# wujinzhong/seamlessCloneOptimization

Hardware: AMD Instinct MI355X
Metric: Mpix/s seamlessClone (ROI 2048^2) (higher is better)
Workload: dtype f32 (arithmetic); storage: 16-bit fixed-point field on the first two level-0 stores of a solve, float16 right-hand side and level 1

## Files before the change

include/seamlessclone_hip_testing.h:

```cpp
#ifndef SEAMLESSCLONE_HIP_TESTING_H
#define SEAMLESSCLONE_HIP_TESTING_H

#include "seamlessclone_hip.h"

#ifdef __cplusplus
extern "C" {
#endif

#define SC_FLAG_LEGACY_PATHS   (1 << 6)
#define SC_LEGACY_SEPARATE_RESTRICT 1
#define SC_LEGACY_BOTTOM_F32   2
#define SC_LEGACY_SEPARATE_TAIL 4
#define SC_LEGACY_UNPACKED_TILES 8
#define SC_LEGACY_SPLICE_LAUNCH 16
#define SC_FORCE_INTERLEAVED_OUT 32
#define SC_FLAG_KEEP_FIELD     (1 << 7)

#define SC_FLAG_POISON_ARENA   (1 << 14)


SC_API int sc_hip_mask_stage(void *instance, const uint8_t *mask, int mask_cols, int mask_rows, int mask_step,
                      int centerX, int centerY, int geo[6], uint8_t *M_out, size_t M_capacity);

SC_API int sc_hip_build_rhs(void *instance,
                     const uint8_t *face, int face_cols, int face_rows, int face_step,
                     const uint8_t *body, int body_cols, int body_rows, int body_step,
                     const uint8_t *mask, int mask_cols, int mask_rows, int mask_step,
                     int centerX, int centerY, int geo[6], float *B_out, float *lap_out, size_t plane_capacity);

SC_API int sc_hip_edit_rhs(void *instance, const sc_edit_params *p, const uint8_t *src, int cols, int rows, int src_step,
                           const uint8_t *mask, int mask_step, uint8_t *M_out, float *lap_out, size_t plane_capacity);
SC_API int sc_hip_canny(void *instance, const uint8_t *src, int cols, int rows, int src_step, float low_threshold,
                        float high_threshold, int kernel_size, uint8_t *classes_out, uint8_t *edges_out, int counts[2]);
SC_API int sc_hip_edit_counts(void *instance, int counts[2]);

SC_API int sc_hip_field_load(void *instance, int W, int H, int C, const float *U, const float *lap);
SC_API int sc_hip_field_sweep(void *instance, int method, int sweeps, float omega, int sweeps_per_launch);
SC_API int sc_hip_field_residual(void *instance, double out[2] );
SC_API int sc_hip_field_solve(void *instance);
SC_API int sc_hip_field_shape(void *instance, int whc[3]);
SC_API int sc_hip_field_store(void *instance, float *U_out, size_t capacity_floats);

SC_API int sc_hip_field_finish(void *instance, uint8_t *body, int body_cols, int body_rows, int body_step, int ltx, int lty);
SC_API int sc_hip_field_lowmode(void *instance);

SC_API int sc_hip_field_time_sweeps(void *instance, int method, int launches, int sweeps_per_launch, float omega,
                             float *ms_per_launch);

SC_API int sc_hip_time_cycle0(void *instance, int launches, float *ms_per_launch);
SC_API int sc_hip_time_cycle0_form(void *instance, int form, int launches, float *ms_per_launch);
SC_API int sc_hip_time_coarse_chain(void *instance, int reps, float *ms_eager, float *ms_graph, int *launches);
SC_API int sc_hip_time_tail_phases(void *instance, unsigned long long *cycles11);

SC_API int sc_hip_selftest_host(void);

SC_API int sc_hip_cycle0_form(const int *facts, int index, int form[3]);

SC_API int sc_hip_bytes_writer(void *instance);

SC_API int sc_hip_coarse_tile_plan(const int *facts, int *plan);

SC_API int sc_hip_pcg_plan(int cols, int rows, int kind, int frames, long long plan[10]);

#define SC_FUSED_ROW 18
SC_API int sc_hip_fused_schedule(const int *facts, const int *verdicts, int nverdicts, int *rows, int capacity);

SC_API int sc_hip_restore_spans(long long step, int rows, int ltx, int lty, int W, int H, long long *spans, int capacity);

#ifdef __cplusplus
}
#endif
#endif
```

seamlesscloneoptimization_amd/capi.py:

```python
from __future__ import annotations

import ctypes as C
import os
import re
import subprocess

import numpy as np

_PKG = os.path.dirname(os.path.abspath(__file__))
_ROOT = os.path.dirname(_PKG)
LIB_PATH = os.path.join(_PKG, "libseamlessclone_hip.so")
HEADER_PATH = os.path.join(_ROOT, "include", "seamlessclone_hip.h")
TESTING_HEADER_PATH = os.path.join(_ROOT, "include", "seamlessclone_hip_testing.h")

SC_OK = 0
SC_ERR_BAD_ARG = -1
SC_ERR_BAD_SIZE = -2
SC_ERR_EMPTY_MASK = -3
SC_ERR_ROI_OOB = -4
SC_ERR_HIP = -5
SC_ERR_NOT_CONVERGED = -6

SC_NORMAL_CLONE = 1
SC_MIXED_CLONE = 2
SC_MONOCHROME_TRANSFER = 3
CLONE_MODES = (SC_NORMAL_CLONE, SC_MIXED_CLONE, SC_MONOCHROME_TRANSFER)

SC_EDIT_COLOR_CHANGE = 1
SC_EDIT_ILLUMINATION_CHANGE = 2
SC_EDIT_TEXTURE_FLATTENING = 3
EDIT_OPS = (SC_EDIT_COLOR_CHANGE, SC_EDIT_ILLUMINATION_CHANGE, SC_EDIT_TEXTURE_FLATTENING)

SC_METHOD_JACOBI = 0
SC_METHOD_RBGS = 1
SC_METHOD_SOR = 2
SC_METHOD_MULTIGRID = 3
SC_METHOD_DST = 4
SC_METHOD_AUTO = 5
SC_METHOD_FFT = 6
SC_AUTO_DIRECT_MAX = 720
SC_AUTO_DIRECT_AREA = 450000
SC_AUTO_NARROW_MAX = 140
SC_AUTO_THIN_MAX = 4
SC_AUTO_THIN_LONG_MAX = 4096

SC_FLAG_NO_SPECULATE = 1 << 0
SC_FLAG_FLOAT_RHS = 1 << 1
SC_FLAG_FLOAT_U0 = 1 << 2
SC_FLAG_NO_COMPOSE_L1 = 1 << 3
SC_FLAG_VCYCLE_BOTTOM = 1 << 4
SC_FLAG_EXACT_TABLES = 1 << 5
SC_FLAG_LEGACY_PATHS = 1 << 6
SC_LEGACY_SEPARATE_RESTRICT, SC_LEGACY_BOTTOM_F32, SC_LEGACY_SEPARATE_TAIL, SC_LEGACY_UNPACKED_TILES = 1, 2, 4, 8
SC_LEGACY_SPLICE_LAUNCH = 16
SC_FORCE_INTERLEAVED_OUT = 32
SC_FLAG_KEEP_FIELD = 1 << 7
SC_FLAG_FFT_FP64 = 1 << 8
SC_FLAG_OPENCV_GREY_MASK = 1 << 9
SC_FLAG_FLOAT_L1 = 1 << 10
SC_FLAG_FLOAT_FIELD = 1 << 11
SC_FLAG_NO_STAGE_MARKS = 1 << 12
SC_FLAG_ROWS_RETURN = 1 << 13
SC_FLAG_POISON_ARENA = 1 << 14

def auto_takes_direct(w: int, h: int) -> bool:
    if w <= SC_AUTO_DIRECT_MAX and h <= SC_AUTO_DIRECT_MAX:
        return True
    if max(w, h) <= SC_AUTO_THIN_LONG_MAX and (w * h <= SC_AUTO_DIRECT_AREA or min(w, h) <= SC_AUTO_NARROW_MAX):
        return True
    return False


ERR_NAMES = {
    SC_ERR_BAD_ARG: "SC_ERR_BAD_ARG", SC_ERR_BAD_SIZE: "SC_ERR_BAD_SIZE", SC_ERR_EMPTY_MASK: "SC_ERR_EMPTY_MASK",
    SC_ERR_ROI_OOB: "SC_ERR_ROI_OOB", SC_ERR_HIP: "SC_ERR_HIP", SC_ERR_NOT_CONVERGED: "SC_ERR_NOT_CONVERGED",
}


class SolverOpts(C.Structure):
    _fields_ = [("method", C.c_int), ("max_sweeps", C.c_int), ("tol", C.c_float), ("check_every", C.c_int),
                ("omega", C.c_float), ("sweeps_per_launch", C.c_int), ("reference_warmup", C.c_int),
                ("mg_pre", C.c_int), ("mg_post", C.c_int), ("update_tol", C.c_float), ("flags", C.c_int), ("jacobi_tile_rows", C.c_int), ("mg_level1_sweeps", C.c_int), ("mg_direct_max", C.c_int), ("legacy_paths", C.c_int)]


class RunInfo(C.Structure):
    _fields_ = [("x0", C.c_int), ("y0", C.c_int), ("W", C.c_int), ("H", C.c_int), ("ltx", C.c_int), ("lty", C.c_int),
                ("sweeps", C.c_int), ("converged", C.c_int), ("rel_residual", C.c_double),
                ("ms_h2d", C.c_float), ("ms_mask", C.c_float), ("ms_pre", C.c_float), ("ms_solve", C.c_float),
                ("ms_post", C.c_float), ("ms_d2h", C.c_float), ("ms_device_total", C.c_float),
                ("sweep_launches", C.c_int), ("last_update", C.c_float), ("device_bytes", C.c_size_t), ("method", C.c_int),
                ("device", C.c_int), ("ms_call", C.c_float), ("field_retry", C.c_int), ("new_size", C.c_int),
                ("group_members", C.c_int), ("group_ragged", C.c_int)]


class BatchJob(C.Structure):
    _fields_ = [("face", C.c_void_p), ("face_cols", C.c_int), ("face_rows", C.c_int), ("face_step", C.c_int),
                ("body", C.c_void_p), ("body_cols", C.c_int), ("body_rows", C.c_int), ("body_step", C.c_int),
                ("mask", C.c_void_p), ("mask_cols", C.c_int), ("mask_rows", C.c_int), ("mask_step", C.c_int),
                ("centerX", C.c_int), ("centerY", C.c_int), ("body_restore", C.c_void_p), ("rc", C.c_int)]


class EditParams(C.Structure):
    _fields_ = [("op", C.c_int), ("red_mul", C.c_float), ("green_mul", C.c_float), ("blue_mul", C.c_float),
                ("alpha", C.c_float), ("beta", C.c_float), ("low_threshold", C.c_float), ("high_threshold", C.c_float),
                ("kernel_size", C.c_int)]


class EditJob(C.Structure):
# ... 204 lines not shown
    L.my_seamlessclone_api_imp_destroy.restype = None
    L.my_seamlessclone_api_imp_sync.argtypes = [C.c_void_p]
    L.my_seamlessclone_api_imp_sync.restype = None
    L.sc_hip_default_opts.argtypes = [C.POINTER(SolverOpts)]
    L.sc_hip_default_opts.restype = None
    L.sc_hip_set_solver.argtypes = [C.c_void_p, C.POINTER(SolverOpts)]
    L.sc_hip_set_solver.restype = C.c_int
    L.sc_hip_get_solver.argtypes = [C.c_void_p, C.POINTER(SolverOpts)]
    L.sc_hip_get_solver.restype = C.c_int
    L.sc_hip_get_info.argtypes = [C.c_void_p, C.POINTER(RunInfo)]
    L.sc_hip_get_info.restype = C.c_int
    L.sc_hip_last_error.argtypes = [C.c_void_p]
    L.sc_hip_last_error.restype = C.c_char_p
    L.sc_hip_set_clone_mode.argtypes = [C.c_void_p, C.c_int]
    L.sc_hip_set_clone_mode.restype = C.c_int
    L.sc_hip_get_clone_mode.argtypes = [C.c_void_p]
    L.sc_hip_get_clone_mode.restype = C.c_int
    L.sc_hip_pool_set_clone_mode.argtypes = [C.c_void_p, C.c_int]
    L.sc_hip_pool_set_clone_mode.restype = C.c_int
    L.sc_hip_run_device.argtypes = [C.c_void_p] + _IMG * 3 + [C.c_int, C.c_int, C.c_bool]
    L.sc_hip_run_device.restype = C.c_int
    L.sc_hip_malloc.argtypes = [C.c_void_p, C.c_size_t]
    L.sc_hip_malloc.restype = C.c_void_p
    L.sc_hip_free.argtypes = [C.c_void_p, C.c_void_p]
    L.sc_hip_free.restype = None
    L.sc_hip_host_alloc.argtypes = [C.c_void_p, C.c_size_t]
    L.sc_hip_host_alloc.restype = C.c_void_p
    L.sc_hip_host_free.argtypes = [C.c_void_p, C.c_void_p]
    L.sc_hip_host_free.restype = None
    L.sc_hip_memcpy_h2d.argtypes = [C.c_void_p, C.c_void_p, C.c_void_p, C.c_size_t]
    L.sc_hip_memcpy_h2d.restype = C.c_int
    L.sc_hip_memcpy_d2h.argtypes = [C.c_void_p, C.c_void_p, C.c_void_p, C.c_size_t]
    L.sc_hip_memcpy_d2h.restype = C.c_int
    L.sc_hip_memcpy_d2d_async.argtypes = [C.c_void_p, C.c_void_p, C.c_void_p, C.c_size_t]
    L.sc_hip_memcpy_d2d_async.restype = C.c_int
    L.sc_hip_device_count.argtypes = []
    L.sc_hip_device_count.restype = C.c_int
    L.sc_hip_device_pci_bus_id.argtypes = [C.c_int, C.c_char_p, C.c_int]
    L.sc_hip_device_pci_bus_id.restype = C.c_int
    L.sc_hip_mask_stage.argtypes = [C.c_void_p] + _IMG + [C.c_int, C.c_int, i32p, u8p, C.c_size_t]
    L.sc_hip_mask_stage.restype = C.c_int
    L.sc_hip_build_rhs.argtypes = [C.c_void_p] + _IMG * 3 + [C.c_int, C.c_int, i32p, f32p, f32p, C.c_size_t]
    L.sc_hip_build_rhs.restype = C.c_int
    L.sc_hip_field_load.argtypes = [C.c_void_p, C.c_int, C.c_int, C.c_int, f32p, f32p]
    L.sc_hip_field_load.restype = C.c_int
    L.sc_hip_field_sweep.argtypes = [C.c_void_p, C.c_int, C.c_int, C.c_float, C.c_int]
    L.sc_hip_field_sweep.restype = C.c_int
    L.sc_hip_field_residual.argtypes = [C.c_void_p, f64p]
    L.sc_hip_field_residual.restype = C.c_int
    L.sc_hip_field_solve.argtypes = [C.c_void_p]
    L.sc_hip_field_solve.restype = C.c_int
    L.sc_hip_bytes_writer.argtypes = [C.c_void_p]
    L.sc_hip_bytes_writer.restype = C.c_int
    L.sc_hip_field_shape.argtypes = [C.c_void_p, i32p]
    L.sc_hip_field_shape.restype = C.c_int
    L.sc_hip_field_store.argtypes = [C.c_void_p, f32p, C.c_size_t]
    L.sc_hip_field_store.restype = C.c_int
    L.sc_hip_field_finish.argtypes = [C.c_void_p, C.c_void_p, C.c_int, C.c_int, C.c_int, C.c_int, C.c_int]
    L.sc_hip_field_finish.restype = C.c_int
    L.sc_hip_field_lowmode.argtypes = [C.c_void_p]
    L.sc_hip_field_lowmode.restype = C.c_int
    L.sc_hip_field_time_sweeps.argtypes = [C.c_void_p, C.c_int, C.c_int, C.c_int, C.c_float, C.POINTER(C.c_float)]
    L.sc_hip_field_time_sweeps.restype = C.c_int
    L.sc_hip_pool_create.argtypes = [C.c_int, C.c_int]
    L.sc_hip_pool_create.restype = C.c_void_p
    L.sc_hip_pool_destroy.argtypes = [C.c_void_p]
    L.sc_hip_pool_destroy.restype = None
    L.sc_hip_pool_size.argtypes = [C.c_void_p]
    L.sc_hip_pool_size.restype = C.c_int
    L.sc_hip_pool_instance.argtypes = [C.c_void_p, C.c_int]
    L.sc_hip_pool_instance.restype = C.c_void_p
    L.sc_hip_pool_set_solver.argtypes = [C.c_void_p, C.POINTER(SolverOpts)]
    L.sc_hip_pool_set_solver.restype = C.c_int
    L.sc_hip_pool_run.argtypes = [C.c_void_p, C.POINTER(BatchJob), C.c_int, C.c_int]
    L.sc_hip_pool_run.restype = C.c_int
    L.sc_hip_pool_set_group.argtypes = [C.c_void_p, C.c_int]
    L.sc_hip_pool_set_group.restype = C.c_int
    L.sc_hip_run_device_batch.argtypes = [C.c_void_p, C.POINTER(BatchJob), C.c_int]
    L.sc_hip_run_device_batch.restype = C.c_int
    L.sc_hip_time_cycle0.argtypes = [C.c_void_p, C.c_int, C.POINTER(C.c_float)]
    L.sc_hip_time_cycle0.restype = C.c_int
    L.sc_hip_time_coarse_chain.argtypes = [C.c_void_p, C.c_int, C.POINTER(C.c_float), C.POINTER(C.c_float), C.POINTER(C.c_int)]
    L.sc_hip_time_coarse_chain.restype = C.c_int
    L.sc_hip_time_tail_phases.argtypes = [C.c_void_p, C.POINTER(C.c_ulonglong)]
    L.sc_hip_time_tail_phases.restype = C.c_int
    L.sc_hip_time_cycle0_form.argtypes = [C.c_void_p, C.c_int, C.c_int, C.POINTER(C.c_float)]
    L.sc_hip_time_cycle0_form.restype = C.c_int
    L.sc_hip_reference_tables_singular.argtypes = [C.c_int, C.c_int]
    L.sc_hip_reference_tables_singular.restype = C.c_int
    L.sc_hip_selftest_host.argtypes = []
    L.sc_hip_selftest_host.restype = C.c_int
    L.sc_hip_cycle0_form.argtypes = [i32p, C.c_int, i32p]
    L.sc_hip_cycle0_form.restype = C.c_int
    L.sc_hip_coarse_tile_plan.argtypes = [i32p, i32p]
    L.sc_hip_coarse_tile_plan.restype = C.c_int
    L.sc_hip_pcg_plan.argtypes = [C.c_int] * 4 + [C.POINTER(C.c_longlong)]
    L.sc_hip_pcg_plan.restype = C.c_int
    L.sc_hip_fused_schedule.argtypes = [i32p, i32p, C.c_int, i32p, C.c_int]
    L.sc_hip_fused_schedule.restype = C.c_int
    L.sc_hip_restore_spans.argtypes = [C.c_longlong] + [C.c_int] * 5 + [C.POINTER(C.c_longlong), C.c_int]
    L.sc_hip_restore_spans.restype = C.c_int
    L.sc_hip_plan_groups.argtypes = [i32p, C.c_int, C.c_int, C.POINTER(SolverOpts), i32p, i32p]
    L.sc_hip_plan_groups.restype = C.c_int
    L.sc_hip_plan_size.argtypes = [C.c_int, C.c_int, C.POINTER(SolverOpts), i32p]
    L.sc_hip_plan_groups_pool.argtypes = [i32p, C.c_int, C.c_int, C.c_int, C.POINTER(SolverOpts), i32p, i32p]
    L.sc_hip_plan_groups_pool.restype = C.c_int
# ... 808 lines not shown
        return p

    def from_device(self, p, shape, dtype=np.uint8):
        out = np.empty(shape, dtype)
        self._check(self.L.sc_hip_memcpy_d2h(self.h, out.ctypes.data, p, out.nbytes))
        return out

    def copy_d2d_async(self, dst, src, nbytes):
        self._check(self.L.sc_hip_memcpy_d2d_async(self.h, dst, src, nbytes))

    def run_device(self, d_face, fshape, d_body, bshape, d_mask, mshape, cx, cy, sync=True,
                   allow_not_converged=False):
        rc = self.L.sc_hip_run_device(self.h, d_face, fshape[1], fshape[0], 3 * fshape[1],
                                      d_body, bshape[1], bshape[0], 3 * bshape[1],
                                      d_mask, mshape[1], mshape[0], mshape[1], int(cx), int(cy), bool(sync))
        return self._check(rc, allow=(SC_ERR_NOT_CONVERGED,) if allow_not_converged else ())

    def run_device_batch(self, jobs, sync=True):
        rc = self.L.sc_hip_run_device_batch(self.h, jobs, len(jobs))
        if sync:
            self.sync()
        return self._check(rc, allow=(SC_ERR_NOT_CONVERGED,))

    def mask_stage(self, mask, cx, cy):
        m = _img(mask)
        geo = np.zeros(6, np.int32)
        M = np.zeros(m[1] * m[2], np.uint8)
        self._check(self.L.sc_hip_mask_stage(self.h, *m, int(cx), int(cy), geo.ctypes.data_as(i32p),
                                             M.ctypes.data_as(u8p), M.size))
        W, H = int(geo[2]), int(geo[3])
        return geo, M[:W * H].reshape(H, W).copy()

    def build_rhs(self, face, body, mask, cx, cy):
        f, b, m = _img(face), _img(body), _img(mask)
        geo = np.zeros(6, np.int32)
        cap = m[1] * m[2]
        B = np.zeros(3 * cap, np.float32)
        lap = np.zeros(3 * cap, np.float32)
        self._check(self.L.sc_hip_build_rhs(self.h, *f, *b, *m, int(cx), int(cy), geo.ctypes.data_as(i32p),
                                            B.ctypes.data_as(f32p), lap.ctypes.data_as(f32p), cap))
        W, H = int(geo[2]), int(geo[3])
        return geo, B[:3 * W * H].reshape(3, H, W).copy(), lap[:3 * W * H].reshape(3, H, W).copy()

    def field_load(self, U, lap):
        U = np.ascontiguousarray(U, np.float32)
        lap = np.ascontiguousarray(lap, np.float32)
        assert U.shape == lap.shape and U.ndim == 3
        Cc, H, W = U.shape
        self._check(self.L.sc_hip_field_load(self.h, W, H, Cc, U.ctypes.data_as(f32p), lap.ctypes.data_as(f32p)))

    def bytes_writer(self):
        return int(self.L.sc_hip_bytes_writer(self.h))

    def field_shape(self):
        whc = np.zeros(3, np.int32)
        self._check(self.L.sc_hip_field_shape(self.h, whc.ctypes.data_as(i32p)))
        return int(whc[2]), int(whc[1]), int(whc[0])

    def field_sweep(self, method, sweeps, omega=1.0, sweeps_per_launch=1):
        self._check(self.L.sc_hip_field_sweep(self.h, int(method), int(sweeps), float(omega), int(sweeps_per_launch)))

    def field_residual(self):
        out = np.zeros(2, np.float64)
        self._check(self.L.sc_hip_field_residual(self.h, out.ctypes.data_as(f64p)))
        return float(out[0]), float(out[1])

    def field_solve(self, allow_not_converged=False):
        rc = self.L.sc_hip_field_solve(self.h)
        return self._check(rc, allow=(SC_ERR_NOT_CONVERGED,) if allow_not_converged else ())

    def field_store(self):
        out = np.zeros(self.field_shape(), np.float32)
        self._check(self.L.sc_hip_field_store(self.h, out.ctypes.data_as(f32p), out.size))
        return out

    def field_finish(self, body, ltx, lty):
        b = _img(body)
        self._check(self.L.sc_hip_field_finish(self.h, *b, int(ltx), int(lty)))

    def field_lowmode(self):
        self._check(self.L.sc_hip_field_lowmode(self.h))

    def field_time_sweeps(self, method, launches, sweeps_per_launch=1, omega=1.0) -> float:
        ms = C.c_float(0)
        self._check(self.L.sc_hip_field_time_sweeps(self.h, int(method), int(launches), int(sweeps_per_launch),
                                                    float(omega), C.byref(ms)))
        return float(ms.value)

    def time_cycle0(self, launches: int = 100) -> float:
        ms = C.c_float(0)
        self._check(self.L.sc_hip_time_cycle0(self.h, int(launches), C.byref(ms)))
        return float(ms.value)

    def time_cycle0_form(self, form: int, launches: int = 100) -> float:
        ms = C.c_float(0)
        self._check(self.L.sc_hip_time_cycle0_form(self.h, int(form), int(launches), C.byref(ms)))
        return float(ms.value)

    def time_coarse_chain(self, reps: int = 50):
        a, b, n = C.c_float(0), C.c_float(0), C.c_int(0)
        self._check(self.L.sc_hip_time_coarse_chain(self.h, int(reps), C.byref(a), C.byref(b), C.byref(n)))
        return float(a.value), float(b.value), int(n.value)

    def time_tail_phases(self):
        buf = (C.c_ulonglong * 11)()
        self._check(self.L.sc_hip_time_tail_phases(self.h, buf))
# ... 93 lines not shown
        try:
            self.close()
        except Exception:
            pass


def plan_size(W: int, H: int, opts: "SolverOpts | None" = None) -> dict:
    out = np.zeros(12, np.int32)
    load().sc_hip_plan_size(int(W), int(H), C.byref(opts) if opts is not None else None, out.ctypes.data_as(i32p))
    keys = ("eligible", "levels", "tail_level", "pad_x", "pad_y", "Kxp", "Kyp", "column_tiles", "row_splits", "direct_nx_ny", "solo_differs", "conditional")
    return dict(zip(keys, out.tolist()))


def plan_groups_pool(sizes, group: int = 0, streams: int = 2, opts: "SolverOpts | None" = None):
    wh = np.ascontiguousarray(np.asarray(sizes, np.int32).reshape(-1, 2))
    n = wh.shape[0]
    g = np.zeros(n, np.int32); k = np.zeros(n, np.int32)
    rc = load().sc_hip_plan_groups_pool(wh.ctypes.data_as(i32p), n, int(group), int(streams), C.byref(opts) if opts is not None else None,
                                        g.ctypes.data_as(i32p), k.ctypes.data_as(i32p))
    if rc < 0:
        raise SeamlessCloneError(rc, "sc_hip_plan_groups_pool")
    return g.tolist(), k.tolist()


SC_POOL_GROUP_AUTO = 0


def plan_edit_groups_pool(sizes, group: int = 0, streams: int = 2):
    wh = np.ascontiguousarray(np.asarray(sizes, np.int32).reshape(-1, 2))
    n = wh.shape[0]
    g = np.zeros(n, np.int32)
    rc = load().sc_hip_plan_edit_groups_pool(wh.ctypes.data_as(i32p), n, int(group), int(streams), g.ctypes.data_as(i32p))
    if rc < 0:
        raise SeamlessCloneError(rc, "sc_hip_plan_edit_groups_pool")
    return g.tolist()


def plan_prepare(sizes, opts: "SolverOpts | None" = None) -> int:
    wh = np.ascontiguousarray(np.asarray(sizes, np.int32).reshape(-1, 2))
    return int(load().sc_hip_plan_prepare(wh.ctypes.data_as(i32p), wh.shape[0], C.byref(opts) if opts is not None else None))


def plan_cache_clear() -> None:
    load().sc_hip_plan_cache_clear()


CYCLE0_FACTS = ("sweeps", "prolong", "f_half", "u_half", "q16_in", "q16_out", "final_cycle", "out_bytes", "composed", "l1_half", "timing",
                "bands", "rag")


def cycle0_form(**facts):
    if facts.pop("out_interleaved", 0):
        facts["out_bytes"] = int(bool(facts.get("out_bytes", 0))) | 2
    f = (C.c_int * len(CYCLE0_FACTS))(*[int(facts.pop(k, 0)) for k in CYCLE0_FACTS])
    if facts:
        raise TypeError("cycle0_form: no such fact: %s" % sorted(facts))
    out = (C.c_int * 3)()
    return tuple(out) if load().sc_hip_cycle0_form(f, 0, out) == 0 else -1


def coarse_tile_plan(W, H, C_, useful, halo, rows, size_class=False, unpacked=False, lanes=False):
    f = (C.c_int * 10)(W, H, C_, useful, halo, rows, int(size_class), int(unpacked), 0, 0)
    head = np.zeros(4, np.int32)
    rc = load().sc_hip_coarse_tile_plan(f, head.ctypes.data_as(i32p))
    if rc != 0:
        raise SeamlessCloneError(rc, "coarse_tile_plan")
    if not lanes:
        return tuple(int(v) for v in head)
    n = int(head[3])
    f[9] = n
    out = np.zeros(4 + 130 * n, np.int32)
    rc = load().sc_hip_coarse_tile_plan(f, out.ctypes.data_as(i32p))
    if rc != 0:
        raise SeamlessCloneError(rc, "coarse_tile_plan")
    t = out[4:].reshape(n, 130)
    return tuple(int(v) for v in head), (t[:, 0], t[:, 1], t[:, 2::2], t[:, 3::2])


PCG_PLAN = ("nx", "ny", "x0", "y0", "cg", "bands", "rows", "eparts", "egroups", "stride")


def pcg_plan(cols, rows, kind, frames=1):
    out = (C.c_longlong * len(PCG_PLAN))()
    rc = load().sc_hip_pcg_plan(int(cols), int(rows), int(kind), int(frames), out)
    if rc != 0:
        raise SeamlessCloneError(rc, "pcg_plan")
    return dict(zip(PCG_PLAN, (int(v) for v in out)))


FUSED_FACTS = ("pre", "post", "budget", "tol", "out_wanted", "q16", "u_half", "composed", "separate_restrict", "early_kind", "bytes_form", "small")
FUSED_ROW = ("kind", "sweeps", "prolong", "final_cycle", "out_bytes", "u_half", "q16_in", "q16_out", "composed", "bands", "lm", "nodes", "judged",
             "coarse_first", "sat", "bands_asked", "early_asked", "cycle")


def fused_schedule(verdicts=(), **facts):
    d = dict(pre=2, post=2, budget=30, tol=0, out_wanted=1, q16=1, u_half=1, composed=1, separate_restrict=0, early_kind=1, bytes_form=1, small=1)
    unknown = sorted(set(facts) - set(d))
    if unknown:
        raise TypeError("fused_schedule: no such fact: %s" % unknown)
    d.update(facts)
    f = (C.c_int * len(FUSED_FACTS))(*[int(d[k]) for k in FUSED_FACTS])
    v = (C.c_int * max(1, len(verdicts)))(*[int(x) for x in verdicts])
    cap = len(FUSED_ROW) * (3 * int(d["budget"]) + 2) + 3
    out = (C.c_int * cap)()
    n = load().sc_hip_fused_schedule(f, v, len(verdicts), out, cap)
    if n < 0:
        raise SeamlessCloneError(n, "fused_schedule")
    k = len(FUSED_ROW)
    return [dict(zip(FUSED_ROW, out[k * i:k * i + k])) for i in range(n)], out[k * n], out[k * n + 1], out[k * n + 2]


# ... 48 lines not shown
```

seamlesscloneoptimization_amd/csrc/sanitize_main.cpp:

```cpp
#include "../../include/seamlessclone_hip_testing.h"
#include "sc_pcg.h"
#include <algorithm>
#include <atomic>
#include <cmath>
#include <cstdio>
#include <cstdlib>
#include <cstring>
#include <thread>
#include <vector>

namespace {
struct StubInst { int gpu; std::atomic<long> calls{ 0 }; sc_solver_opts opts; int clone_mode = SC_NORMAL_CLONE; };
std::atomic<long> g_jobs_run{ 0 };
}
extern "C" {
void *stub_create(int gpu) { StubInst *s = new StubInst(); s->gpu = gpu; sc_hip_default_opts(&s->opts); return s; }
void stub_destroy(void *p) { delete (StubInst *)p; }
void stub_sync(void *) {}
int stub_set_solver(void *p, const sc_solver_opts *o) { ((StubInst *)p)->opts = *o; return SC_OK; }
int stub_get_solver(void *p, sc_solver_opts *o) { *o = ((StubInst *)p)->opts; return SC_OK; }
int stub_set_clone_mode(void *p, int mode)
{
    if (mode < SC_NORMAL_CLONE || mode > SC_MONOCHROME_TRANSFER) return SC_ERR_BAD_ARG;
    ((StubInst *)p)->clone_mode = mode;
    return SC_OK;
}
int stub_memcpy_d2d_async(void *, void *, const void *, size_t) { return SC_OK; }
int stub_run_device(void *p, const uint8_t *, int, int, int, uint8_t *body, int, int, int, const uint8_t *, int, int, int, int, int, bool)
{
    ((StubInst *)p)->calls++;
    g_jobs_run++;
    *(volatile uint8_t *)body += 1;
    return SC_OK;
}
int stub_run(void *p, const uint8_t *f, int fc, int fr, int fs, uint8_t *body, int bc, int br, int bs, const uint8_t *m, int mc, int mr, int ms, int cx, int cy, int, bool)
{
    return stub_run_device(p, f, fc, fr, fs, body, bc, br, bs, m, mc, mr, ms, cx, cy, false);
}
std::atomic<long> g_edit_mixed{ 0 };
int stub_edit_device(void *p, const sc_edit_params *, const uint8_t *, int, int, int, const uint8_t *, int, uint8_t *dst, int, bool)
{
    ((StubInst *)p)->calls++;
    g_jobs_run++;
    *(volatile uint8_t *)dst += 1;
    return SC_OK;
}
int stub_edit(void *p, const sc_edit_params *e, const uint8_t *s, int c, int r, int ss, const uint8_t *m, int ms, uint8_t *dst, int ds)
{
    return stub_edit_device(p, e, s, c, r, ss, m, ms, dst, ds, false);
}
constexpr int FAILING_COLS = 777;
int stub_edit_device_batch(void *p, const sc_edit_params *, sc_edit_job *jobs, int n)
{
    ((StubInst *)p)->calls++;
    for (int i = 0; i < n; ++i) {
        if (jobs[i].cols != jobs[0].cols || jobs[i].rows != jobs[0].rows) g_edit_mixed++;
        g_jobs_run++; *(volatile uint8_t *)jobs[i].dst += 1; jobs[i].rc = SC_OK;
    }
    return jobs[0].cols == FAILING_COLS ? SC_ERR_HIP : SC_OK;
}
// ... 485 lines not shown
                pub[k] = sc_volume_wls_job{ fake(k, 6), fake(k, 9), fake(k, 4), nullptr, fake(k, 8), k == 1 ? nullptr : fake(k, 3), fake(k, 0),
                                            links ? fake(k, 1) : nullptr, links ? fake(k, 2) : nullptr,
                                            !links ? nullptr : k == 3 ? (const float *)((uintptr_t)fake(k, 5) + 2) : fake(k, 5), fake(k, 10),
                                            (float *)fake(k, 7), 12345 };
            }
            Instance inst;
            FloatJobs v;
            const int rc = float_intake(&inst, SC_POISSON_GUIDANCE, carries, pub, 5, arrays_of, v);
            const std::vector<int> stay = links ? std::vector<int>{ 0, 2, 4 } : std::vector<int>{ 0, 2, 3, 4 };
            if (rc != SC_ERR_BAD_ARG || inst.err != "null state pointer") return fail("float_intake: the worst code and the first reason");
            if (v.dj.size() != stay.size() || v.side.size() != stay.size() || v.rcs.size() != stay.size()) return fail("float_intake: how many jobs stay");
            if (pub[1].rc != SC_ERR_BAD_ARG || (links && pub[3].rc != SC_ERR_BAD_ARG)) return fail("float_intake: a refused job's code");
            for (size_t i = 0; i < stay.size(); ++i) {
                const int k = stay[i];
                const SideArrays &a = v.side[i];
                if (v.rcs[i] != &pub[k].rc || pub[k].rc != SC_ERR_HIP) return fail("float_intake: where a job's code goes");
                if (v.dj[i].gx != fake(k, 6) || v.dj[i].gy != fake(k, 9) || v.dj[i].b != fake(k, 10) || v.dj[i].out != (float *)fake(k, 7) || v.dj[i].d != fake(k, 8))
                    return fail("float_intake: a job's own arrays");
                if (a.w != fake(k, 0) || a.st != fake(k, 3) || a.gt != fake(k, 4)) return fail("float_intake: w, st or gt of another job");
                if (links ? (a.sx != fake(k, 1) || a.sy != fake(k, 2) || a.smt != fake(k, 5)) : (a.sx || a.sy || a.smt))
                    return fail("float_intake: sx, sy or smt of another job, or not NULL where the call carries none");
            }
        }
        {
            sc_volume_wls_job one{ fake(0, 6), fake(0, 9), fake(0, 4), nullptr, fake(0, 8), fake(0, 3), fake(0, 0), fake(0, 1), fake(0, 2), fake(0, 5), fake(0, 10),
                                   (float *)fake(0, 7), 0 };
            Instance inst;
            FloatJobs v;
            if (float_intake(&inst, SC_POISSON_GUIDANCE, FLOAT_DATA | FLOAT_STATE, &one, 1, arrays_of, v) != SC_OK || v.side.size() != 1) return fail("float_intake (a plain region call)");
            const SideArrays &a = v.side[0];
            if (a.w || a.sx || a.sy || a.gt || a.smt || a.st != fake(0, 3)) return fail("float_intake: an array the call does not carry must be NULL");
        }
    }
    {
        const int kinds[] = { SC_POISSON_LAPLACIAN, SC_POISSON_LAPLACIAN | SC_POISSON_NEUMANN, SC_POISSON_GUIDANCE | SC_POISSON_FREE_LEFT | SC_POISSON_FREE_TOP,
                              SC_POISSON_GUIDANCE | SC_POISSON_PERIODIC_X, SC_POISSON_LAPLACIAN | SC_POISSON_PERIODIC_X | SC_POISSON_PERIODIC_Y };
        for (int kind : kinds)
            for (int frames : { 1, 2, 17, 64, SC_POISSON_MAX_PLANES })
                for (int cols = 3; cols <= 2105; cols += (cols < 20 ? 1 : 83))
                    for (int rows = 3; rows <= 2205; rows += (rows < 70 ? 1 : 61)) {
                        long long p[10];
                        if (sc_hip_pcg_plan(cols, rows, kind, frames, p) != SC_OK) return fail("pcg_plan");
                        const long long nx = p[0], ny = p[1], cg = p[4], bands = p[5], rows_per = p[6], eparts = p[7], egroups = p[8], stride = p[9];
                        if (nx < 1 || nx > cols || ny < 1 || ny > (long long)rows * frames || ny % frames) return fail("pcg_plan: the unknown block");
                        if (cg != (nx + 255) / 256 || cg * bands > sc::PCG_PARTS || bands * rows_per < ny || (bands - 1) * rows_per >= ny) return fail("pcg_plan: the bands");
                        if (eparts < 1 || eparts > sc::PCG_PARTS || egroups != (nx * ny + 3) / 4 || eparts * ((egroups + eparts - 1) / eparts) < egroups) return fail("pcg_plan: the segments");
                        if (stride % 64 || stride < nx * ny) return fail("pcg_plan: the stride");
                    }
        long long p[10];
        if (sc_hip_pcg_plan(2, 7, SC_POISSON_LAPLACIAN, 1, p) != SC_ERR_BAD_SIZE || sc_hip_pcg_plan(33, 47, SC_POISSON_NEUMANN, 1, p) != SC_ERR_BAD_ARG ||
            sc_hip_pcg_plan(33, 47, SC_POISSON_LAPLACIAN, 0, p) != SC_ERR_BAD_ARG || sc_hip_pcg_plan(33, 47, SC_POISSON_LAPLACIAN, SC_POISSON_MAX_PLANES + 1, p) != SC_ERR_BAD_ARG ||
            sc_hip_pcg_plan(33, 47, SC_POISSON_LAPLACIAN, 1, nullptr) != SC_ERR_BAD_ARG) return fail("pcg_plan (refusals)");
    }
    printf("sanitize_main: clean\n");
    return 0;
}
```

seamlesscloneoptimization_amd/csrc/sc_arena.cpp:

```cpp
#include "sc_instance.h"
#include <algorithm>
#include <cstring>
#include <thread>

namespace sc {

int hip_fail(Instance *I, hipError_t e, const char *what)
{
    if (I) {
        I->err = std::string(what) + ": " + hipGetErrorString(e);
        I->scan_counter_dirty = true;
    }
    return SC_ERR_HIP;
}

int ensure(Instance *I, DevBuf &b, size_t bytes, bool zero)
{
    if (bytes <= b.cap) {
        if (!zero && bytes && (I->opts.flags & SC_FLAG_POISON_ARENA)) {
            SC_HIP(I, hipStreamSynchronize(I->stream));
            if (I->aux) SC_HIP(I, hipStreamSynchronize(I->aux));
            if (I->aux2) SC_HIP(I, hipStreamSynchronize(I->aux2));
            SC_HIP(I, hipMemsetAsync(b.p, 0xFF, bytes, I->stream));
            SC_HIP(I, hipStreamSynchronize(I->stream));
// ... 102 lines not shown
    if (rc) return rc;
    uint8_t *s = (uint8_t *)stage.p;
    size_t piece = (size_t)1 << 20;
    for (int y0 = 0; y0 < rows;) {
        const int n = std::min((int)std::max<size_t>(1, piece / dpitch), rows - y0);
        copy_rows(I, s + (size_t)y0 * dpitch, dpitch, h + (size_t)y0 * hpitch, hpitch, row_bytes, n);
        SC_HIP(I, hipMemcpyAsync((uint8_t *)d + (size_t)y0 * dpitch, s + (size_t)y0 * dpitch, dpitch * (size_t)(n - 1) + row_bytes,
                                 hipMemcpyHostToDevice, I->stream));
        y0 += n;
        piece = std::min(piece * 4, (size_t)8 << 20);
    }
    return SC_OK;
}

int download_rows(Instance *I, DevBuf &stage, uint8_t *h, size_t hpitch, const void *d, size_t dpitch,
                  size_t row_bytes, int rows)
{
    if (rows <= 0 || row_bytes == 0) return SC_OK;
    const size_t total = dpitch * (size_t)(rows - 1) + row_bytes;
    int rc = ensure_pinned(I, stage, total);
    if (rc) return rc;
    SC_HIP(I, hipMemcpyAsync(stage.p, d, total, hipMemcpyDeviceToHost, I->stream));
    SC_HIP(I, hipStreamSynchronize(I->stream));
    copy_rows(I, h, hpitch, (const uint8_t *)stage.p, dpitch, row_bytes, rows);
    return SC_OK;
}

static Field make_field(void *p, int W, int H, int C)
{
    Field f;
    f.p = (float *)p; f.W = W; f.H = H; f.C = C;
    f.pitch = round_up(W, 64);
    f.plane = (size_t)f.pitch * H;
    return f;
}

int setup_fields(Instance *I, int W, int H, int C)
{
    field_moved(I);
    I->out_direct = false;
    Field proto = make_field(nullptr, W, H, C);
    const size_t bytes = proto.bytes() + 4096;
    int rc;
    if ((rc = ensure(I, I->d_U0, bytes, false))) return rc;
    if ((rc = ensure(I, I->d_U1, bytes, false))) return rc;
    if ((rc = ensure(I, I->d_F, bytes, false))) return rc;
    const bool same = I->F.p == I->d_F.p && I->U0.p == I->d_U0.p && I->U1.p == I->d_U1.p && I->F.W == W &&
                      I->F.H == H && I->F.C == C;
    I->U0 = make_field(I->d_U0.p, W, H, C);
    I->U1 = make_field(I->d_U1.p, W, H, C);
    I->F = make_field(I->d_F.p, W, H, C);
    I->result_in_U1 = false;
    I->f_half = false;
    I->u_half = false;
    if (!same) I->mg.clear();
    return SC_OK;
}

}
```

seamlesscloneoptimization_amd/csrc/sc_batch.cpp:

```cpp
#include "sc_instance.h"
#include <algorithm>
#include <cmath>
#include <cstring>
#include <vector>

using namespace sc;

namespace sc {

FrameSpans frame_spans(size_t step, int rows, int ltx, int lty, int W, int H)
{
    FrameSpans f{};
    f.bytes = step * (size_t)rows;
    f.head_end = f.tail_begin = f.bytes;
    if (W < 3 || H < 3) return f;
    const size_t c0 = 3 * (size_t)(ltx + 1), c1 = 3 * (size_t)(ltx + W - 1), top = (size_t)(lty + 1) * step;
    f.head_end = top + c0;
    f.mid_first = top + c1; f.mid_len = step - (c1 - c0); f.stride = step; f.mids = H - 3;
    f.tail_begin = top + (size_t)(H - 3) * step + c1;
    return f;
}

}

namespace {

constexpr int GROUP_RS = 32;

struct RagScope {
    Instance *I;
    ~RagScope() { rag_end(I); }
};

int run_group_members(Instance *I, sc_batch_job *jobs, const std::vector<int> &idx, const std::vector<Geo> &geo, const int *guess, int *d_r,
                      const std::vector<SizePlan> *plans, const std::vector<char> &frame)
{
    const int n = (int)idx.size();
    Geo g0 = geo[idx[0]];
    if (plans) for (int k = 1; k < n; ++k) { g0.W = std::max(g0.W, geo[idx[k]].W); g0.H = std::max(g0.H, geo[idx[k]].H); }
    int rc;
    I->mpitch = round_up(g0.W, 64);
    const size_t mplane = (size_t)I->mpitch * g0.H;
    if ((rc = ensure(I, I->d_M, mplane * n, false))) return rc;
    if ((rc = setup_fields(I, g0.W, g0.H, 3 * n))) return rc;
    RagScope scope{ I };
    CallScope call{ I };
    std::vector<MaskJob> mj(n);
    std::vector<ImageJob> ij(n);
    for (int k = 0; k < n; ++k) {
        const int i = idx[k];
        const sc_batch_job &j = jobs[i];
        mj[k] = MaskJob{};
        mj[k].mask = j.mask; mj[k].mw = j.mask_cols; mj[k].mh = j.mask_rows; mj[k].mstep = j.mask_step;
        mj[k].rect = d_r + GROUP_RS * i;
        mj[k].g = geo[i]; mj[k].M = (uint8_t *)I->d_M.p + mplane * k; mj[k].mpitch = I->mpitch;
        ij[k].face_org = j.face + (size_t)geo[i].y0 * j.face_step + 3 * geo[i].x0; ij[k].fstep = j.face_step;
        const size_t roi = (size_t)geo[i].lty * j.body_step + 3 * geo[i].ltx;
        ij[k].body_org = j.body + roi; ij[k].body_src = frame[i] ? j.body_restore + roi : j.body + roi; ij[k].bstep = j.body_step;
        ij[k].M = (const uint8_t *)I->d_M.p + mplane * k;
        ij[k].d_rect = guess ? d_r + GROUP_RS * i : nullptr;
        if (guess) { ij[k].rx0 = guess[4 * i]; ij[k].rx1 = guess[4 * i + 1]; ij[k].ry0 = guess[4 * i + 2]; ij[k].ry1 = guess[4 * i + 3]; }
        if (plans) { ij[k].W = geo[i].W; ij[k].H = geo[i].H; }
    }
    if (plans && (rc = rag_begin_table(I, *plans))) return rc;
    bool builds_done = false;
    launch_mask_erode3_group(mj.data(), n, I->stream);
    I->erode_done = false;
    I->guard = RectGuard();
    const SolveTarget to{ nullptr, 0, &ij };
    const int solve_rc = solve_step(I, to, [&]() -> int {
        launch_preprocess_group(ij.data(), n, I->mpitch, I->U0, I->F, I->stream, I->f_half, I->u_half, I->clone_mode);
        SC_HIP(I, hipGetLastError());
        if (plans && !builds_done) {
            if ((rc = rag_begin_builds(I))) return rc;
            builds_done = true;
        }
        return SC_OK;
    });
    if (solve_rc != SC_OK && solve_rc != SC_ERR_NOT_CONVERGED) return solve_rc;
    if (!I->spec_post.done && (rc = write_output(I, to))) return rc;
    for (int k = 0; k < n; ++k) jobs[idx[k]].rc = solve_rc;
    SC_HIP(I, hipGetLastError());
    fill_info_geo(I, g0);
    I->info.group_members = n; I->info.group_ragged = plans ? 1 : 0;
    return solve_rc;
}

int report_groups(const std::vector<std::vector<int>> &groups, const std::vector<SizePlan> &plans, const int *order, int *group_of, int *kind_of)
{
    for (size_t g = 0; g < groups.size(); ++g) {
        bool uniform = true;
        for (int i : groups[g]) uniform = uniform && plans[i].W == plans[groups[g][0]].W && plans[i].H == plans[groups[g][0]].H;
        for (int i : groups[g]) {
            const int m = order ? order[i] : i;
            group_of[m] = (int)g;
            if (kind_of) kind_of[m] = groups[g].size() < 2 ? 0 : uniform ? 1 : plans[i].solo_differs ? 3 : 2;
        }
    }
    return (int)groups.size();
}

}

extern "C" {

int sc_hip_run_device_batch(void *p, sc_batch_job *jobs, int n)
{
    if (!jobs || n <= 0) return SC_ERR_BAD_ARG;
    Instance *I;
    int rc = begin_call(p, I);
    if (rc) return rc;
    auto alone = [&](int i) -> int {
        sc_batch_job &j = jobs[i];
        j.rc = sc_hip_run_device(p, j.face, j.face_cols, j.face_rows, j.face_step, j.body, j.body_cols, j.body_rows, j.body_step,
                                 j.mask, j.mask_cols, j.mask_rows, j.mask_step, j.centerX, j.centerY, false);
        return j.rc;
    };
    auto one_by_one = [&]() -> int {
        int worst = SC_OK;
        for (int i = 0; i < n; ++i) worst = worse(worst, alone(i));
        return worst;
    };
    std::vector<char> frame(n, 0);
    std::vector<Geo> geo(n);
// ... 240 lines not shown
```

seamlesscloneoptimization_amd/csrc/sc_common.h:

```cpp
#pragma once
#include <hip/hip_runtime.h>
#include <stdint.h>
#include <stddef.h>
#include <algorithm>
#include <string>
#include <vector>
#include "../../include/seamlessclone_hip_testing.h"

namespace sc {

struct Field {
    float *p = nullptr;
    int W = 0, H = 0, C = 0;
    int pitch = 0;
    size_t plane = 0;
    __host__ __device__ float *at(int c) const { return p + (size_t)c * plane; }
    size_t bytes() const { return plane * (size_t)C * sizeof(float); }
};

static inline int round_up(int v, int m) { return (v + m - 1) / m * m; }

struct Geo { int x0, y0, W, H, ltx, lty; };

struct Img8 {
// ... 69 lines not shown
    return (a - b) + (cc - d);
}
#endif
void launch_poisson_pre(const PoissonGeo &g, bool lap, const PoissonJobDev &j, Field U0, Field F, hipStream_t s, float lam = 0.f);
void launch_poisson_pre_group(const PoissonGeo &g, bool lap, const PoissonJobDev *jobs, int n, Field U0, Field F, hipStream_t s, float lam = 0.f);
void launch_poisson_out(const PoissonGeo &g, const PoissonJobDev &j, Field U, hipStream_t s);
void launch_poisson_out_group(const PoissonGeo &g, const PoissonJobDev *jobs, int n, Field U, hipStream_t s);
int poisson_mean_parts(int H);
void launch_poisson_mean(const PoissonGeo &g, const PoissonJobDev *jobs, int n, double *parts, hipStream_t s);
size_t mask_bbox_group_parts(const MaskJob *jobs, int n);
void launch_mask_bbox_group(const MaskJob *jobs, int n, hipStream_t s, int *parts);
void launch_mask_erode3_group(const MaskJob *jobs, int n, hipStream_t s);
struct BboxTask { const uint8_t *mask = nullptr; int mw = 0, mh = 0, mstep = 0; BboxFold fold; int scan_rows = 0; Geo g{}; size_t mask_bytes = 0; uint8_t *M_out = nullptr; };
void launch_preprocess(const uint8_t *body_org, int bstep, const uint8_t *face_org, int fstep,
                       const uint8_t *M, int mpitch, Field U0, Field U1, Field F, hipStream_t s, bool f_half = false, bool u_half = false, bool grey = false,
                       const BboxTask *scan = nullptr, int mode = SC_NORMAL_CLONE);
struct RectGuard { const int *d_rect = nullptr; int x0 = 0, x1 = 0, y0 = 0, y1 = 0; };
struct AbortFlag { unsigned *p = nullptr; unsigned gen = 0; unsigned *host = nullptr; };
#if defined(__HIPCC__)
__device__ __forceinline__ bool abort_set(const AbortFlag &a) { return a.p && *reinterpret_cast<const volatile unsigned *>(a.p) == a.gen; }
#endif
struct LmNodes { const float *CN = nullptr; int ny = 0, npitch = 0; };
#if defined(__HIPCC__)
__device__ __forceinline__ void lm_add4_nodes(float p00, float p01, float p10, float p11, int x, int y, float4 &v)
{
    const float ty = 0.125f * (float)(y & 7);
    const float l = __builtin_fmaf(ty, p10 - p00, p00), r = __builtin_fmaf(ty, p11 - p01, p01);
    const float dx = 0.125f * (r - l), a0 = __builtin_fmaf((float)(x & 7), dx, l);
    v.x += a0;
    v.y += a0 + dx;
    v.z += __builtin_fmaf(2.0f, dx, a0);
    v.w += __builtin_fmaf(3.0f, dx, a0);
}
__device__ __forceinline__ void lm_add4(const LmNodes &lm, int c, int x, int y, float4 &v)
{
    const float *__restrict__ p = lm.CN + ((size_t)c * lm.ny + (y >> 3)) * lm.npitch + (x >> 3);
    lm_add4_nodes(p[0], p[1], p[lm.npitch], p[lm.npitch + 1], x, y, v);
}
__device__ __forceinline__ unsigned lm_byte(float d)
{
    d = d > 255.0f ? 255.0f : d;
    d = d < 0.0f ? 0.0f : d;
    return (unsigned)(unsigned char)d;
}
__device__ __forceinline__ float lm_bilinear(const LmNodes &lm, int c, int x, int y)
{
    const float *__restrict__ p = lm.CN + ((size_t)c * lm.ny + (y >> 3)) * lm.npitch + (x >> 3);
    const float tx = 0.125f * (float)(x & 7), ty = 0.125f * (float)(y & 7);
    const float top = __builtin_fmaf(tx, p[1] - p[0], p[0]), bot = __builtin_fmaf(tx, p[lm.npitch + 1] - p[lm.npitch], p[lm.npitch]);
    return __builtin_fmaf(ty, bot - top, top);
}
#endif
void launch_postprocess(Field U, uint8_t *body_org, int bstep, hipStream_t s, RectGuard guard = RectGuard(), LmNodes lm = LmNodes(), AbortFlag ab = AbortFlag());
void launch_preprocess_group(const ImageJob *jobs, int n, int mpitch, Field U0, Field F, hipStream_t s, bool f_half, bool u_half, int mode);
void launch_postprocess_group(Field U, const ImageJob *jobs, int n, hipStream_t s, LmNodes lm = LmNodes(), AbortFlag ab = AbortFlag());
void launch_splice_planar(Field Q, uint8_t *body_org, int bstep, hipStream_t s, RectGuard guard = RectGuard(), AbortFlag ab = AbortFlag());
void launch_splice_planar_group(Field Q, const ImageJob *jobs, int n, hipStream_t s, AbortFlag ab = AbortFlag());
void launch_half_to_float(const void *src_half, float *dst, size_t n, hipStream_t s);
struct FrameSpans { size_t bytes, head_end, mid_first, mid_len, stride, tail_begin; int mids; };
FrameSpans frame_spans(size_t step, int rows, int ltx, int lty, int W, int H);
struct CopyJobs { enum { MAX = 16 }; void *dst[MAX]; const void *src[MAX]; size_t bytes[MAX]; FrameSpans frame[MAX]; };
void launch_copy_group(const CopyJobs &t, int n, hipStream_t s);

void launch_jacobi(Field Uin, Field Uout, Field F, hipStream_t s, bool tag = false, int lds_tile_rows = 0);
void launch_rb_half(Field U, Field F, int color, float omega, hipStream_t s, bool tag = false);
bool launch_jacobi_tb(Field Uin, Field Uout, Field F, int sweeps, hipStream_t s, bool tag = false);
bool launch_rb_tb(Field Uin, Field Uout, Field F, int sweeps, float omega, hipStream_t s, bool tag = false);
int  tb_max_depth(int method);
int  tb_hard_max_depth(int method);
long tb_big_side();
struct TilePlan { int nbx, nby, full, lps, lg, K, blocks; };
__host__ __device__ inline TilePlan coarse_tile_plan(int W, int H, int C, int uw, int hx, int rows, bool size_class, bool pack = true)
{
    TilePlan p;
    p.nbx = (W + uw - 1) / uw; p.nby = (H + rows - 1) / rows;
    p.full = p.nbx; p.lps = 64; p.lg = 6; p.K = 1;
    const int need = (W - (p.nbx - 1) * uw + 2 * hx + 3) / 4;
    if (pack && !size_class && need <= 32) {
        p.lg = 32 - __builtin_clz((unsigned)(need - 1));
        p.lps = 1 << p.lg; p.K = 64 >> p.lg; p.full = p.nbx - 1;
    }
    p.blocks = p.nby * (p.full * C + (p.nbx - p.full) * ((C + p.K - 1) >> (6 - p.lg)));
    return p;
}
struct TileLane { int by, c, x, sl, lps; };
__host__ __device__ inline TileLane coarse_tile_lane(const TilePlan &p, int C, int uw, int hx, int tile, int lane)
{
    TileLane t;
    const int nfull = p.full * p.nby * C;
    if (tile < nfull) {
        const int q = tile / p.full;
        t.c = q / p.nby; t.by = q - t.c * p.nby;
        t.x = (tile - q * p.full) * uw - hx + 4 * lane; t.sl = lane; t.lps = 64;
    } else {
        const int k = tile - nfull, g = k / p.nby;
        t.by = k - g * p.nby; t.lps = p.lps; t.sl = lane & (p.lps - 1);
        t.c = (g << (6 - p.lg)) + (lane >> p.lg);
        t.x = p.full * uw - hx + 4 * t.sl;
    }
    return t;
}
int  tb_gen_rows(int W, int H, int C, int hx, int hy, bool pack = false, int pack_rows = 8);
int  tb_gen_rows_deep(int W, int H, int C, int hx, int hy, bool pack = false);
struct MGGeom;
struct ComposeArgs;
struct RagMember;
constexpr int TBM_PLAIN = 0, TBM_PROLONG = 1, TBM_ZEROIN = 4;
bool launch_rb_tb_gen(Field Uin, Field Uout, Field F, int sweeps, const MGGeom &g, int mode, Field E, hipStream_t s, const RagMember *rag = nullptr, int lev = 0,
                      bool pack = true);
int  launch_rb_tb_prolong0(Field Uin, Field Uout, Field F, int sweeps, const MGGeom &g, Field E, float *partial, hipStream_t s);
int  tb_blocks_level0(int W, int H, int C, int sweeps);
void launch_max_final(const float *d_partial, int n, unsigned *d_out, hipStream_t s);
void launch_max_final2(const float *d_a, int na, const float *d_b, int nb, unsigned *d_out2, hipStream_t s, const unsigned *flag = nullptr);
void cycle0_row_geometry(int H, int sweeps, int &nby, int &step, int &hy);
int  cycle0_blocks(int W, int H, int C, int sweeps);
bool launch_cycle_coarse(Field Uout, Field F, Field Fc, const MGGeom &g, int sweeps, hipStream_t s, bool half_io = false,
                         const RagMember *rag = nullptr, int lev = 0, bool pack = true);

int  residual_max_blocks();
void launch_residual(Field U, Field F, double *d_partials, double *d_out, hipStream_t s);

struct MGDim {
    int n, nc;
    float alpha;
    float cw_last;
    float d_last;
    float tw1, tw2;
    float inv_last;
};
struct MGGeom { MGDim x, y; };
struct ComposeArgs { Field E2; MGGeom g1; };

constexpr int C0_TIMING   = 1;
constexpr int C0_F_HALF   = 2;
constexpr int C0_U_HALF   = 4;
constexpr int C0_FINAL    = 8;
constexpr int C0_COMPOSED = 16;
constexpr int C0_OUT      = 32;
constexpr int C0_BANDS    = 64;
constexpr int C0_L1_HALF  = 128;
constexpr int C0_Q16_IN   = 256;
constexpr int C0_Q16_OUT  = 512;
constexpr int C0_PACK_ROWS = 6;
constexpr int C0_PACK     = 2048;
constexpr int C0_OUT3     = 4096;
constexpr int C0_RAG      = 1024;

struct Cycle0Launch {
    Field Uin, Uout, F, Fc, E;
    MGGeom g{};
    int sweeps = 0;
    bool prolong = false;
    bool f_half = false, u_half = false, q16_in = false, q16_out = false;
    bool final_cycle = false, out_bytes = false;
    bool out_interleaved = false;
    const ImageJob *jobs = nullptr; int njobs = 0;
    bool composed = false;
    bool l1_half = false, timing = false;
    ComposeArgs comp{};
    float4 *bands = nullptr;
    float *partial = nullptr;
    LmNodes lm{};
    AbortFlag sat{};
    const RagMember *rag = nullptr;
    hipStream_t s = nullptr;
};
bool cycle0_form(const Cycle0Launch &d, int &T, bool &PRO, int &TAG);
int  cycle0_form_at(int i, int &T, bool &PRO, int &TAG);
int  launch_cycle0(const Cycle0Launch &d);

constexpr int RAG_MAX_LEVELS = 12;
struct RagMember {
    int W, H;
    int lw[RAG_MAX_LEVELS], lh[RAG_MAX_LEVELS];
    MGGeom g[RAG_MAX_LEVELS];
    const unsigned char *mm;
    int npx, npy;
    int lm_nx, lm_ny, lm_cells_y, lm_nxt, lm_nrs, lm_nparts, lm_Kx, lm_Ky;
    const float *lm_Sx, *lm_Sy, *lm_R;
    const int *lm_map[2];
};

void launch_rb_half_gen(Field U, Field F, int color, float omega, MGGeom g, hipStream_t s);
void launch_residual_restrict(Field U, Field F, Field Fc, MGGeom g, hipStream_t s);
int  prolong_blocks(int nx, int ny, int C);
void launch_prolong_add(Field Uc, Field Uf, MGGeom g, float *d_partial, unsigned *d_maxcorr, hipStream_t s);
void launch_fill_zero(Field U, hipStream_t s);

constexpr int MG_BOTTOM_MAX_LEVELS = 12;
constexpr int MG_BOTTOM_LDS_BYTES = 152 * 1024;
struct MGBottomLevel { MGGeom g; float omega; int offU, offF, pitch; };
struct MGBottomArgs {
    int nlevels, pre, post, coarse_sweeps, lds_floats;
    int fd_level, fd_nxp, fd_nyp, fd_off;
    const float *fd_mats;
    Field Ftop, Utop;
    MGBottomLevel lv[MG_BOTTOM_MAX_LEVELS];
};
__host__ __device__ static inline long fd_mat_floats(int nxp, int nyp) { return 2L * nxp * nxp + 2L * nyp * nyp + (long)nxp * nyp; }
__host__ __device__ static inline long fd_lds_floats(int nxp, int nyp) { return fd_mat_floats(nxp, nyp) + 2L * nxp * nyp; }
hipError_t mg_bottom_prepare();
void launch_fd_build(float *mats, const MGGeom &g, int nxp, int nyp, hipStream_t s, unsigned char *mm = nullptr, int NPX = 0, int NPY = 0);
void launch_fd_build_rag(const RagMember *rag, int members, int lev, hipStream_t s);
__host__ __device__ static inline long fd_mm_bytes(int NPX, int NPY) { return 4L * (2L * NPX * NPX + 2L * NPY * NPY + (long)NPX * NPY); }
struct MGBottomMM { const unsigned char *mm; Field Ftop, Utop; int nx, ny; };
bool launch_mg_bottom_mm(const MGBottomMM &a, int NPX, int NPY, int C, hipStream_t s);
struct MGTail { const unsigned char *mm; Field F, U; MGGeom g; int pre, post; unsigned long long *stamps;
                const RagMember *rag; int lev; bool rag_uniform; };
// ... 7 lines not shown
```

seamlesscloneoptimization_amd/csrc/sc_cycle0.hip:

```cpp
#include "sc_common.h"
#include <hip/hip_fp16.h>
#include "sc_wave.h"
#include "sc_mg_device.h"
#include <type_traits>

namespace sc {

constexpr int C0_HXQ = 3;
constexpr int C0_HX = 4 * C0_HXQ;

template <int R>
__device__ __forceinline__ void c0_load(const float *__restrict__ p, int P, int H, int x, int y0, float4 (&v)[R])
{
    const int xc = min(max(x, 0), P - 4);
#pragma unroll
    for (int r = 0; r < R; ++r) {
        const int yc = min(max(y0 + r, 0), H - 1);
        v[r] = *reinterpret_cast<const float4 *>(p + (size_t)yc * P + xc);
    }
}

template <int R>
__device__ __forceinline__ void c0_load_half(const __half *__restrict__ p, int P, int H, int x, int y0, float4 (&v)[R])
{
    const int xc = min(max(x, 0), P - 4);
    uint2 raw[R];
#pragma unroll
    for (int r = 0; r < R; ++r) {
        const int yc = min(max(y0 + r, 0), H - 1);
        raw[r] = *reinterpret_cast<const uint2 *>(p + (size_t)yc * P + xc);
    }
#pragma unroll
    for (int r = 0; r < R; ++r) {
        const __half2 a = *reinterpret_cast<const __half2 *>(&raw[r].x), b = *reinterpret_cast<const __half2 *>(&raw[r].y);
        const float2 fa = __half22float2(a), fb = __half22float2(b);
        v[r] = make_float4(fa.x, fa.y, fb.x, fb.y);
    }
}

template <int R>
__device__ __forceinline__ void c0_load_half_raw(const __half *__restrict__ p, int P, int H, int x, int y0, uint2 (&v)[R])
{
    const int xc = min(max(x, 0), P - 4);
#pragma unroll
    for (int r = 0; r < R; ++r) {
        const int yc = min(max(y0 + r, 0), H - 1);
        v[r] = *reinterpret_cast<const uint2 *>(p + (size_t)yc * P + xc);
    }
}
template <int R>
__device__ __forceinline__ void c0_load_q16(const uint16_t *__restrict__ p, int P, int H, int x, int y0, float4 (&v)[R])
{
    const int xc = min(max(x, 0), P - 4);
    uint2 raw[R];
#pragma unroll
    for (int r = 0; r < R; ++r) {
        const int yc = min(max(y0 + r, 0), H - 1);
        raw[r] = *reinterpret_cast<const uint2 *>(p + (size_t)yc * P + xc);
    }
#pragma unroll
    for (int r = 0; r < R; ++r) {
        v[r].x = __builtin_fmaf((float)(raw[r].x & 0xffffu), 0.015625f, -256.0f);
        v[r].y = __builtin_fmaf((float)(raw[r].x >> 16), 0.015625f, -256.0f);
        v[r].z = __builtin_fmaf((float)(raw[r].y & 0xffffu), 0.015625f, -256.0f);
        v[r].w = __builtin_fmaf((float)(raw[r].y >> 16), 0.015625f, -256.0f);
    }
}
__device__ __forceinline__ unsigned c0_q16_checked(float u, int &seen)
{
    int i;
    asm("v_cvt_i32_f32 %0, %1" : "=v"(i) : "v"(__builtin_fmaf(u, 64.0f, 16384.5f)));
    seen |= i;
    return (unsigned)min(max(i, 0), 65535);
}

__device__ __forceinline__ void c0_scale_q(uint2 &h)
{
    const __half2 k = __float2half2_rn(-0.25f);
    __half2 a = *reinterpret_cast<__half2 *>(&h.x), b = *reinterpret_cast<__half2 *>(&h.y);
    a = __hmul2(a, k); b = __hmul2(b, k);
    h.x = *reinterpret_cast<unsigned *>(&a); h.y = *reinterpret_cast<unsigned *>(&b);
}
template <int K>
__device__ __forceinline__ float c0_gs_q(float s, float quarter, const uint2 &h)
{
    const unsigned raw = (K < 2) ? h.x : h.y;
    float d;
    if (K & 1) asm("v_fma_mix_f32 %0, %1, %2, %3 op_sel:[0,0,1] op_sel_hi:[0,0,1]" : "=v"(d) : "v"(s), "s"(quarter), "v"(raw));
    else asm("v_fma_mix_f32 %0, %1, %2, %3 op_sel_hi:[0,0,1]" : "=v"(d) : "v"(s), "s"(quarter), "v"(raw));
    return d;
}
template <int K>
__device__ __forceinline__ float c0_f_minus(const uint2 &h, float s)
{
    const unsigned raw = (K < 2) ? h.x : h.y;
    float d;
    if (K & 1) asm("v_fma_mix_f32 %0, %1, -4.0, -%2 op_sel:[1,0,0] op_sel_hi:[1,0,0]" : "=v"(d) : "v"(raw), "v"(s));
    else asm("v_fma_mix_f32 %0, %1, -4.0, -%2 op_sel_hi:[1,0,0]" : "=v"(d) : "v"(raw), "v"(s));
    return d;
}
__device__ __forceinline__ float c0_comp(const float4 &v, int k) { return k == 0 ? v.x : k == 1 ? v.y : k == 2 ? v.z : v.w; }


constexpr int C0_OUT3_ROWS = 52, C0_OUT3_WORDS = (256 - 2 * C0_HX) / 4;
__device__ __forceinline__ int c0_lane_again() { int z = 0; asm volatile("" : "+v"(z)); return (int)__builtin_amdgcn_mbcnt_hi(~0u, __builtin_amdgcn_mbcnt_lo(~0u, (unsigned)z)); }
template <bool ON> __device__ __forceinline__ float c0_opaque_s(float v) { if constexpr (ON) asm volatile("" : "+s"(v)); return v; }
template <bool ON> __device__ __forceinline__ int c0_opaque_s(int v) { if constexpr (ON) asm volatile("" : "+s"(v)); return v; }
template <int N> __device__ __forceinline__ unsigned *c0_out3_stage() { __shared__ unsigned stage[N]; return stage; }
__device__ __forceinline__ void c0_out3_write(const unsigned *__restrict__ stage, uint8_t *__restrict__ body, int bstep, int W, int H, int x0t, int y0t,
                                              int wv, int lane, int nw)
{
    const int lo = 3 * (max(x0t, 1) - x0t), hi = 3 * (min(x0t + 4 * C0_OUT3_WORDS, W - 1) - x0t);
    for (int rr = wv; rr < C0_OUT3_ROWS; rr += nw) {
        const int y = y0t + rr;
        if (y < 1 || y > H - 2) continue;
        uint8_t *d = body + (size_t)y * bstep + 3 * (size_t)x0t;
        const int a = (int)((uintptr_t)d & 3);
        const int o0 = 12 * lane - a;
        if (o0 >= hi || o0 + 12 <= lo) continue;
        const int jc = min(lane, C0_OUT3_WORDS - 1), jp = max(min(lane - 1, C0_OUT3_WORDS - 1), 0);
        unsigned pc[3], pp[3];
#pragma unroll
        for (int c = 0; c < 3; ++c) {
            const unsigned *row = stage + (c * C0_OUT3_ROWS + rr) * C0_OUT3_WORDS;
            pc[c] = row[jc]; pp[c] = row[jp];
        }
        unsigned w[4];
        w[0] = ((pp[2] >> 16) & 255u) | ((pp[0] >> 24) << 8) | ((pp[1] >> 24) << 16) | ((pp[2] >> 24) << 24);
        w[1] = (pc[0] & 255u) | ((pc[1] & 255u) << 8) | ((pc[2] & 255u) << 16) | (((pc[0] >> 8) & 255u) << 24);
        w[2] = ((pc[1] >> 8) & 255u) | (((pc[2] >> 8) & 255u) << 8) | (((pc[0] >> 16) & 255u) << 16) | (((pc[1] >> 16) & 255u) << 24);
        w[3] = ((pc[2] >> 16) & 255u) | ((pc[0] >> 24) << 8) | ((pc[1] >> 24) << 16) | ((pc[2] >> 24) << 24);
#pragma unroll
        for (int k = 0; k < 3; ++k) {
            const unsigned v = (unsigned)(((((unsigned long long)w[k + 1]) << 32) | w[k]) >> (8 * (4 - a)));
            const int o = o0 + 4 * k;
            if (o >= lo && o + 4 <= hi) *reinterpret_cast<unsigned *>(d + o) = v;
            else {
#pragma unroll
                for (int b = 0; b < 4; ++b)
                    if (o + b >= lo && o + b < hi) d[o + b] = (uint8_t)(v >> (8 * b));
            }
        }
    }
}

template <int T, int NW, int R, bool PRO, bool GEN, bool ZEROIN, int TAG = 0, class... X3>
__global__ __launch_bounds__(NW * 64) __attribute__((amdgpu_waves_per_eu(4))) void k_cycle0(Field Uin, Field Uout, Field F, Field Fc, Field E, MGGeom g,
                                                    float *__restrict__ partial, ComposeArgs comp, float4 *__restrict__ bands, LmNodes lm, AbortFlag sat,
                                                    const RagMember *__restrict__ rag, int lev, X3... x3)
{
    constexpr int HY = 2 * T + 2, RH = NW * R;
    constexpr bool OUT3 = (TAG & C0_OUT3) != 0;
    static_assert(sizeof...(X3) == (OUT3 ? 1 : 0), "the members' jobs travel with the three-channel bytes form only");
    constexpr bool RAG = (TAG & C0_RAG) != 0;
    constexpr bool COMP = (TAG & C0_COMPOSED) != 0;
    static_assert(!COMP || (PRO && !GEN && R % 2 == 0), "composition of two prolongations exists on level 0 only");
    constexpr bool FINAL = (TAG & C0_FINAL) != 0;
    constexpr bool OUT = (TAG & C0_OUT) != 0, BANDS = ((TAG & C0_BANDS) != 0 || FINAL) && !OUT;
    static_assert(!OUT || (FINAL && !GEN), "bytes leave from the last level-0 launch only");
    static_assert(!OUT3 || (OUT && !RAG && T == 2 && RH - 2 * HY == C0_OUT3_ROWS), "interleaved bytes: the judged two-sweep form of a same-size group");
    static_assert(!(TAG & C0_BANDS) || !GEN, "cell shares exist on level 0 only");
    constexpr bool HF = (TAG & C0_F_HALF) != 0, HU = (TAG & C0_U_HALF) != 0;
    static_assert(!(HF && GEN), "float16 right-hand sides exist on level 0 only");
    constexpr bool L1H = (TAG & C0_L1_HALF) != 0;
    constexpr bool UQI = (TAG & C0_Q16_IN) != 0, UQO = (TAG & C0_Q16_OUT) != 0;
    static_assert(!((UQI || UQO) && (GEN || (HU && UQI) || (OUT && UQO))), "16-bit fields: level 0, between its launches");
    static_assert(!L1H || !GEN || ZEROIN, "float16 level-1 fields: the level-1 launch starts from a zero correction");
    static_assert(!(PRO && GEN), "the in-kernel prolongation relies on level 0's regular last interval");
    static_assert(2 * T + 2 <= C0_HX, "column halo too small");
    static_assert(R % 2 == 0, "bands must hold whole coarse-row pairs");
    __shared__ float4 edge[2][NW][2][64];
    __shared__ float2 hedge[2][NW][64];
    const int lane = threadIdx.x & 63;
    const int wv = __builtin_amdgcn_readfirstlane(threadIdx.x >> 6);
    int W = Uin.W, H = Uin.H;
    const int P = Uin.pitch;
    const int nbx = (W + (256 - 2 * C0_HX) - 1) / (256 - 2 * C0_HX), nby = (H + (RH - 2 * HY) - 1) / (RH - 2 * HY);
    const int tile = xcd_tile(blockIdx.x, gridDim.x);
    constexpr bool PACK = (TAG & C0_PACK) != 0;
    static_assert(!PACK || (GEN && ZEROIN && !PRO && !RAG), "packed column tiles: the coarse forms of one size");
    TileLane tl{};
    if constexpr (PACK) tl = coarse_tile_lane(coarse_tile_plan(W, H, Uin.C, 256 - 2 * C0_HX, C0_HX, RH - 2 * HY, false), Uin.C, 256 - 2 * C0_HX, C0_HX, tile, lane);
    const int bx = tile % nbx, by = PACK ? tl.by : (tile / nbx) % nby;
    const int c_first = PACK ? min(tl.c, Uin.C - 1) : OUT3 ? 3 * (tile / (nbx * nby)) : tile / (nbx * nby);
    const int sl = PACK ? tl.sl : lane, lps = PACK ? tl.lps : 64;
    const bool live = !PACK || tl.c < Uin.C;
    if constexpr (RAG) {
        const RagMember &m = rag[c_first / 3];
        W = m.lw[lev]; H = m.lh[lev];
        if (bx * (256 - 2 * C0_HX) >= W || by * (RH - 2 * HY) >= H) {
            if (PRO && threadIdx.x == 0) partial[tile] = 0.f;
            return;
        }
        g = m.g[lev];
        if (PRO) E.H = m.lh[lev + 1];
        if ((TAG & C0_COMPOSED) != 0) { comp.g1 = m.g[lev + 1]; comp.E2.H = m.lh[lev + 2]; }
    }
    const int lane_wg = lane, wv_wg = wv, bx_wg = bx, by_wg = by;
    const MGGeom &g_wg = g;
    const ComposeArgs &comp_wg = comp;
    int ci = 0, c_run = c_first, pt_run = OUT3 ? tile + 2 * (c_first / 3) * (nbx * nby) : tile;
    const int pt_step = nbx * nby;
    _Pragma("nounroll") do {
    const int lane = OUT3 ? c0_lane_again() : lane_wg, wv = c0_opaque_s<OUT3>(wv_wg), bx = c0_opaque_s<OUT3>(bx_wg), by = c0_opaque_s<OUT3>(by_wg);
    std::conditional_t<OUT3, MGGeom, const MGGeom &> g = g_wg;
    std::conditional_t<OUT3, ComposeArgs, const ComposeArgs &> comp = comp_wg;
    if constexpr (OUT3) {
        g.x.tw1 = c0_opaque_s<OUT3>(g.x.tw1); g.y.tw1 = c0_opaque_s<OUT3>(g.y.tw1);
        comp.g1.x.tw1 = c0_opaque_s<OUT3>(comp.g1.x.tw1); comp.g1.y.tw1 = c0_opaque_s<OUT3>(comp.g1.y.tw1);
    }
    const int x = PACK ? tl.x : bx * (256 - 2 * C0_HX) - C0_HX + 4 * lane;
    const int y0 = by * (RH - 2 * HY) - HY + wv * R;
    const int c = OUT3 ? c_run : c_first, ptile = OUT3 ? pt_run : tile;
    float4 u[R], f[HF ? 1 : R];
    uint2 fh[HF ? R : 1];
    if (ZEROIN) {
#pragma unroll
        for (int r = 0; r < R; ++r) u[r] = make_float4(0.f, 0.f, 0.f, 0.f);
    } else if (HU) {
        c0_load_half<R>(reinterpret_cast<const __half *>(Uin.p) + (size_t)c * Uin.plane, P, H, x, y0, u);
    } else if (UQI) {
        c0_load_q16<R>(reinterpret_cast<const uint16_t *>(Uin.p) + (size_t)c * Uin.plane, P, H, x, y0, u);
    } else {
        c0_load<R>(Uin.at(c), P, H, x, y0, u);
    }
    constexpr int NE = R / 2 + 2, NQ = R / 4 + 3;
    float2 eab[PRO ? NE : 1];
    float ecc[PRO ? NE : 1];
    float2 e2r[COMP ? NQ : 1];
    float e2l[COMP ? NQ : 1];
    static_assert(!PRO || GEN || 2 * T + 3 <= C0_HX, "column halo too small for the shared prolongation loads");
    float e2b63[COMP ? NQ : 1];
    if (PRO) {
        const int cx = min(max(x >> 1, 0), E.pitch - 4), J = (y0 >> 1) - 1;
        if constexpr (L1H) {
            const __half *__restrict__ e = reinterpret_cast<const __half *>(E.p) + (size_t)c * E.plane;
#pragma unroll
            for (int j = 0; j < NE; ++j) {
                const __half *er = e + (size_t)min(max(J + j, 0), E.H - 1) * E.pitch + cx;
                eab[j] = __half22float2(*reinterpret_cast<const __half2 *>(er));
            }
        } else {
        const float *__restrict__ e = E.at(c);
#pragma unroll
        for (int j = 0; j < NE; ++j) {
            const float *er = e + (size_t)min(max(J + j, 0), E.H - 1) * E.pitch + cx;
            eab[j] = *reinterpret_cast<const float2 *>(er);
        }
        }
    }
    if (COMP) {
        const float *__restrict__ e2 = comp.E2.at(c);
        const int qx = min(max(x >> 2, 0), comp.E2.pitch - 2), Q = ((y0 >> 1) - 1) >> 1;
#pragma unroll
        for (int q = 0; q < NQ; ++q) {
            const float *er = e2 + (size_t)min(max(Q + q, 0), comp.E2.H - 1) * comp.E2.pitch + qx;
            e2r[q].x = er[0];
            e2b63[q] = 0.f;
            if (lane == 63) e2b63[q] = er[1];
        }
    }
    if (!PRO) {
        if constexpr (HF) c0_load_half_raw<R>(reinterpret_cast<const __half *>(F.p) + (size_t)c * F.plane, P, H, x, y0, fh);
        else if constexpr (GEN && L1H) c0_load_half<R>(reinterpret_cast<const __half *>(F.p) + (size_t)c * F.plane, P, H, x, y0, f);
        else c0_load<R>(F.at(c), P, H, x, y0, f);
    }
    const bool x0ok = (x + 0 >= 1) && (x + 0 <= W - 2), x1ok = (x + 1 >= 1) && (x + 1 <= W - 2);
    const bool x2ok = (x + 2 >= 1) && (x + 2 <= W - 2), x3ok = (x + 3 >= 1) && (x + 3 <= W - 2);

    const int xw = bx * (256 - 2 * C0_HX) - C0_HX;
    bool inner = !GEN && (xw >= 4) && (xw + 255 <= W - 2) && (y0 >= 1) && (y0 + R - 1 <= H - 2);
// ... 256 lines not shown
#undef SC_C0_RES
#undef SC_C0_F
            float rl = wave_from_left(res.w);
            if (GEN) {
                float rn = wave_from_right(res.x);
                h0[r] = ((0.5f * rl + res.x) + wxa0 * res.y) + wxb0 * res.z;
                h1[r] = ((0.5f * res.y + res.z) + wxa1 * res.w) + wxb1 * rn;
            } else {
                h0[r] = __builtin_fmaf(res.y, 0.5f, __builtin_fmaf(rl, 0.5f, res.x));
                h1[r] = __builtin_fmaf(res.w, 0.5f, __builtin_fmaf(res.y, 0.5f, res.z));
            }
        }
        };
        if (inner) residual_rows(std::false_type{}); else residual_rows(std::true_type{});
        hedge[0][wv][lane] = make_float2(h0[R - 1], h1[R - 1]);
        if (GEN) hedge[1][wv][lane] = make_float2(h0[0], h1[0]);
        __syncthreads();
        const float2 hup = (wv > 0) ? hedge[0][wv - 1][lane] : make_float2(0.f, 0.f);
        const float2 hdn = (GEN && wv < NW - 1) ? hedge[1][wv + 1][lane] : make_float2(0.f, 0.f);
        const bool lane_out = (sl >= C0_HXQ) && (sl < lps - C0_HXQ) && live;
        float *__restrict__ fc = Fc.at(c);
        const float fx0 = (I == g.x.nc) ? 2.0f * g.x.inv_last : 1.0f;
        const float fx1 = (I + 1 == g.x.nc) ? 2.0f * g.x.inv_last : 1.0f;
#pragma unroll
        for (int r = 0; r < R; r += 2) {
            const int yr = wv * R + r, y = y0 + r;
            const int J = y >> 1;
            if (!lane_out || yr < HY || yr >= RH - HY || J < 1 || J > g.y.nc) continue;
            const float m0 = (r == 0) ? hup.x : h0[r - 1], m1 = (r == 0) ? hup.y : h1[r - 1];
            float v0, v1;
            if (GEN) {
                const float wya = (J == g.y.nc) ? g.y.tw1 : 0.5f, wyb = (J == g.y.nc) ? g.y.tw2 : 0.0f;
                const float p0 = (r + 2 < R) ? h0[(r + 2 < R) ? r + 2 : 0] : hdn.x;
                const float p1 = (r + 2 < R) ? h1[(r + 2 < R) ? r + 2 : 0] : hdn.y;
                v0 = ((0.5f * m0 + h0[r]) + wya * h0[r + 1]) + wyb * p0;
                v1 = ((0.5f * m1 + h1[r]) + wya * h1[r + 1]) + wyb * p1;
            } else {
                v0 = __builtin_fmaf(h0[r + 1], 0.5f, __builtin_fmaf(m0, 0.5f, h0[r]));
                v1 = __builtin_fmaf(h1[r + 1], 0.5f, __builtin_fmaf(m1, 0.5f, h1[r]));
            }
            const float fy = (J == g.y.nc) ? 2.0f * g.y.inv_last : 1.0f;
            if constexpr (L1H && !GEN) {
                __half *o = reinterpret_cast<__half *>(Fc.p) + (size_t)c * Fc.plane + (size_t)J * Fc.pitch + I;
                if (I >= 1 && I <= g.x.nc) o[0] = __float2half_rn(v0 * (fx0 * fy));
                if (I + 1 >= 1 && I + 1 <= g.x.nc) o[1] = __float2half_rn(v1 * (fx1 * fy));
            } else {
            float *o = fc + (size_t)J * Fc.pitch + I;
            if (I >= 1 && I <= g.x.nc) o[0] = v0 * (fx0 * fy);
            if (I + 1 >= 1 && I + 1 <= g.x.nc) o[1] = v1 * (fx1 * fy);
            }
        }
    }

    if constexpr (OUT3) {
        if (lane < C0_HXQ || lane >= 64 - C0_HXQ || x >= P || x >= W) continue;
    } else if (sl < C0_HXQ || sl >= lps - C0_HXQ || !live || x >= P || x >= W) return;
    if constexpr (OUT) {
        uint8_t *__restrict__ q = reinterpret_cast<uint8_t *>(Uout.p) + (size_t)c * Uout.plane;
        const bool corr = lm.CN && x <= W - 2;
        const int Yc0 = max(y0, 0) >> 3;
        float nd[3][2] = { { 0.f, 0.f }, { 0.f, 0.f }, { 0.f, 0.f } };
        if (corr) {
            const float *__restrict__ pn = lm.CN + (size_t)c * lm.ny * lm.npitch + (x >> 3);
#pragma unroll
            for (int k = 0; k < 3; ++k) {
                const float *row = pn + (size_t)min(Yc0 + k, lm.ny - 1) * lm.npitch;
                nd[k][0] = row[0]; nd[k][1] = row[1];
            }
        }
#pragma unroll
        for (int r = 0; r < R; ++r) {
            const int yr = wv * R + r, y = y0 + r;
            if (!(yr >= HY && yr < RH - HY && y >= 1 && y <= H - 2)) continue;
            float4 v = u[r];
            if (corr) {
                const bool second = (y >> 3) != Yc0;
                lm_add4_nodes(second ? nd[1][0] : nd[0][0], second ? nd[1][1] : nd[0][1], second ? nd[2][0] : nd[1][0], second ? nd[2][1] : nd[1][1], x, y, v);
            }
            const unsigned px4 = lm_byte(v.x) | (lm_byte(v.y) << 8) | (lm_byte(v.z) << 16) | (lm_byte(v.w) << 24);
            if constexpr (OUT3) c0_out3_stage<3 * C0_OUT3_ROWS * C0_OUT3_WORDS>()[(ci * C0_OUT3_ROWS + (yr - HY)) * C0_OUT3_WORDS + (lane - C0_HXQ)] = px4;
            else *reinterpret_cast<unsigned *>(q + (size_t)y * P + x) = px4;
        }
        if constexpr (OUT3) continue; else return;
    }
    if constexpr (GEN && L1H) {
        __half *__restrict__ outh = reinterpret_cast<__half *>(Uout.p) + (size_t)c * Uout.plane;
#pragma unroll
        for (int r = 0; r < R; ++r) {
            const int yr = wv * R + r, y = y0 + r;
            if (!(yr >= HY && yr < RH - HY && y >= 0 && y < H)) continue;
            const __half2 a = __floats2half2_rn(u[r].x, u[r].y), b2 = __floats2half2_rn(u[r].z, u[r].w);
            uint2 pk; pk.x = *reinterpret_cast<const unsigned *>(&a); pk.y = *reinterpret_cast<const unsigned *>(&b2);
            *reinterpret_cast<uint2 *>(outh + (size_t)y * P + x) = pk;
        }
        return;
    }
    if constexpr (UQO) {
        uint16_t *__restrict__ outq = reinterpret_cast<uint16_t *>(Uout.p) + (size_t)c * Uout.plane;
        int s0 = 0, s1 = 0, s2 = 0, s3 = 0;
#pragma unroll
        for (int r = 0; r < R; ++r) {
            const int yr = wv * R + r, y = y0 + r;
            if (!(yr >= HY && yr < RH - HY && y >= 0 && y < H)) continue;
            uint2 pk;
            pk.x = c0_q16_checked(u[r].x, s0) | (c0_q16_checked(u[r].y, s1) << 16);
            pk.y = c0_q16_checked(u[r].z, s2) | (c0_q16_checked(u[r].w, s3) << 16);
            *reinterpret_cast<uint2 *>(outq + (size_t)y * P + x) = pk;
        }
        const int seen = s0 | (x + 1 < W ? s1 : 0) | (x + 2 < W ? s2 : 0) | (x + 3 < W ? s3 : 0);
        if ((seen & ~0xffff) && sat.p) { *sat.p = sat.gen; if (sat.host) *sat.host = sat.gen; }
        return;
    }
    float *__restrict__ out = Uout.at(c);
#pragma unroll
    for (int r = 0; r < R; ++r) {
        const int yr = wv * R + r, y = y0 + r;
        if (yr >= HY && yr < RH - HY && y >= 0 && y < H) *reinterpret_cast<float4 *>(out + (size_t)y * P + x) = u[r];
    }
    } while (OUT3 && (c_run += 1, pt_run += pt_step, ++ci < 3));
    if constexpr (OUT3) {
        const ImageJobs &t = (x3, ...);
        const ImageJob &j = t.j[c_first / 3];
        __syncthreads();
        if (abort_set(sat)) return;
        if (j.d_rect && (j.d_rect[0] != j.rx0 || j.d_rect[1] != j.rx1 || j.d_rect[2] != j.ry0 || j.d_rect[3] != j.ry1)) return;
        c0_out3_write(c0_out3_stage<3 * C0_OUT3_ROWS * C0_OUT3_WORDS>(), j.body_org, j.bstep, W, H, bx * (256 - 2 * C0_HX), by * (RH - 2 * HY), wv, c0_lane_again(), NW);
    }
}

constexpr int C0_NW = 8, C0_R = 8;


using Cycle0Kernel = void (*)(Field, Field, Field, Field, Field, MGGeom, float *, ComposeArgs, float4 *, LmNodes, AbortFlag, const RagMember *, int);
struct Cycle0Form { int T; bool PRO; int TAG; Cycle0Kernel k; };
#define C0_FORM(T_, PRO_, TAG_) { T_, PRO_, TAG_, k_cycle0<T_, C0_NW, C0_R, PRO_, false, false, TAG_> }
#define C0_FORM_RAG(T_, PRO_, TAG_) C0_FORM(T_, PRO_, TAG_), C0_FORM(T_, PRO_, TAG_ | C0_RAG)
#define C0_FORM_TWIN(T_, PRO_, TAG_) C0_FORM(T_, PRO_, TAG_), C0_FORM(T_, PRO_, TAG_ | C0_TIMING)
constexpr int C0_FAST = C0_F_HALF | C0_L1_HALF, C0_FAST_CYCLE = C0_FAST | C0_COMPOSED, C0_Q16 = C0_Q16_IN | C0_Q16_OUT;
static constexpr Cycle0Form c0_forms[] = {
    C0_FORM_RAG(2, false, C0_FAST | C0_U_HALF | C0_Q16_OUT), C0_FORM(2, false, C0_FAST | C0_U_HALF | C0_Q16_OUT | C0_TIMING),
    C0_FORM_RAG(2, false, C0_FAST | C0_U_HALF), C0_FORM_RAG(2, false, C0_FAST),
    C0_FORM_RAG(4, true, C0_FAST_CYCLE | C0_Q16), C0_FORM(4, true, C0_FAST_CYCLE | C0_Q16 | C0_TIMING), C0_FORM(4, true, C0_FAST_CYCLE | C0_Q16 | C0_BANDS),
    C0_FORM_RAG(4, true, C0_FAST_CYCLE | C0_Q16_IN | C0_BANDS), C0_FORM(4, true, C0_FAST_CYCLE | C0_Q16_IN | C0_BANDS | C0_TIMING),
    C0_FORM(4, true, C0_FAST_CYCLE | C0_Q16_IN),
    C0_FORM_RAG(2, true, C0_FAST_CYCLE | C0_FINAL | C0_OUT), C0_FORM(2, true, C0_FAST_CYCLE | C0_FINAL | C0_OUT | C0_TIMING),
    C0_FORM_RAG(2, true, C0_FAST_CYCLE | C0_FINAL),
    C0_FORM_RAG(4, true, C0_FAST_CYCLE), C0_FORM(4, true, C0_FAST_CYCLE | C0_TIMING), C0_FORM_RAG(4, true, C0_FAST_CYCLE | C0_BANDS),
    C0_FORM_TWIN(4, true, C0_COMPOSED | C0_F_HALF), C0_FORM(4, true, C0_COMPOSED | C0_F_HALF | C0_BANDS),
    C0_FORM(2, true, C0_COMPOSED | C0_F_HALF | C0_FINAL), C0_FORM(2, true, C0_COMPOSED | C0_F_HALF | C0_FINAL | C0_OUT),
    C0_FORM_TWIN(4, true, C0_COMPOSED), C0_FORM(4, true, C0_COMPOSED | C0_BANDS),
    C0_FORM(2, true, C0_COMPOSED | C0_FINAL), C0_FORM(2, true, C0_COMPOSED | C0_FINAL | C0_OUT),
    C0_FORM(1, false, C0_F_HALF | C0_U_HALF), C0_FORM(2, false, C0_F_HALF | C0_U_HALF),
    C0_FORM_TWIN(1, false, C0_F_HALF), C0_FORM_TWIN(2, false, C0_F_HALF), C0_FORM_TWIN(1, false, 0), C0_FORM_TWIN(2, false, 0),
    C0_FORM_TWIN(2, true, C0_F_HALF), C0_FORM_TWIN(3, true, C0_F_HALF), C0_FORM_TWIN(4, true, C0_F_HALF), C0_FORM(4, true, C0_F_HALF | C0_BANDS),
    C0_FORM_TWIN(2, true, 0), C0_FORM_TWIN(3, true, 0), C0_FORM_TWIN(4, true, 0), C0_FORM(4, true, C0_BANDS),
    C0_FORM(1, true, C0_F_HALF | C0_FINAL), C0_FORM(2, true, C0_F_HALF | C0_FINAL), C0_FORM(2, true, C0_F_HALF | C0_FINAL | C0_OUT),
    C0_FORM(1, true, C0_FINAL), C0_FORM(2, true, C0_FINAL), C0_FORM(2, true, C0_FINAL | C0_OUT),
};
#undef C0_FORM_TWIN
#undef C0_FORM_RAG
#undef C0_FORM

constexpr int C0_OUT3_TAG = C0_FAST_CYCLE | C0_FINAL | C0_OUT | C0_OUT3;
static bool c0_is_out3(const Cycle0Launch &d)
{
    return d.out_interleaved && d.out_bytes && d.final_cycle && d.prolong && d.composed && d.sweeps == 2 && d.f_half && d.l1_half && !d.u_half && !d.q16_in &&
           !d.q16_out && !d.timing && !d.rag;
}

static const Cycle0Form *c0_find(const Cycle0Launch &d)
{
    if (d.out_interleaved) return nullptr;
    const bool shares = d.bands && d.prolong && !d.final_cycle && d.sweeps == 4;
    const int TAG = (d.timing ? C0_TIMING : 0) | (d.f_half ? C0_F_HALF : 0) | (d.u_half ? C0_U_HALF : 0) | (d.final_cycle ? C0_FINAL : 0) |
                    (d.composed ? C0_COMPOSED : 0) | (d.out_bytes ? C0_OUT : 0) | (shares ? C0_BANDS : 0) | (d.l1_half ? C0_L1_HALF : 0) |
                    (d.q16_in ? C0_Q16_IN : 0) | (d.q16_out ? C0_Q16_OUT : 0) | (d.rag ? C0_RAG : 0);
    for (const Cycle0Form &f : c0_forms)
        if (f.TAG == TAG && f.T == d.sweeps && f.PRO == d.prolong) return &f;
    return nullptr;
}

bool cycle0_form(const Cycle0Launch &d, int &T, bool &PRO, int &TAG)
{
    if (c0_is_out3(d)) { T = 2; PRO = true; TAG = C0_OUT3_TAG; return true; }
    const Cycle0Form *f = c0_find(d);
    if (f) { T = f->T; PRO = f->PRO; TAG = f->TAG; }
    return f != nullptr;
}
int cycle0_form_at(int i, int &T, bool &PRO, int &TAG)
{
    const int n = (int)(sizeof(c0_forms) / sizeof(c0_forms[0]));
    if (i >= 0 && i < n) { T = c0_forms[i].T; PRO = c0_forms[i].PRO; TAG = c0_forms[i].TAG; }
    return n;
}

int launch_cycle0(const Cycle0Launch &d)
{
    if (d.out_interleaved) {
        if (!c0_is_out3(d) || !d.jobs || d.njobs < 1 || d.njobs > (int)ImageJobs::MAX || d.Uin.C != 3 * d.njobs) return -1;
        ImageJobs t{};
        for (int i = 0; i < d.njobs; ++i) t.j[i] = d.jobs[i];
        const int blocks = cycle0_blocks(d.Uin.W, d.Uin.H, d.njobs, 2);
        hipLaunchKernelGGL((k_cycle0<2, C0_NW, C0_R, true, false, false, C0_OUT3_TAG, ImageJobs>), dim3(blocks), dim3(C0_NW * 64), 0, d.s, d.Uin, d.Uout, d.F, d.Fc,
                           d.E, d.g, d.partial, d.comp, d.bands, d.lm, d.sat, d.rag, 0, t);
        return 3 * blocks;
    }
    const Cycle0Form *f = c0_find(d);
    if (!f) return -1;
    const int blocks = cycle0_blocks(d.Uin.W, d.Uin.H, d.Uin.C, f->T);
    hipLaunchKernelGGL(f->k, dim3(blocks), dim3(C0_NW * 64), 0, d.s, d.Uin, d.Uout, d.F, d.Fc, d.E, d.g, d.partial, d.comp, d.bands, d.lm, d.sat, d.rag, 0);
    return f->PRO ? blocks : 0;
}

void cycle0_row_geometry(int H, int sweeps, int &nby, int &step, int &hy)
{
    const int RH = C0_NW * C0_R;
    hy = 2 * sweeps + 2; step = RH - 2 * hy; nby = (H + step - 1) / step;
}

int cycle0_blocks(int W, int H, int C, int sweeps)
{
    const int RH = C0_NW * C0_R, HY = 2 * sweeps + 2;
    return ((W + (256 - 2 * C0_HX) - 1) / (256 - 2 * C0_HX)) * ((H + (RH - 2 * HY) - 1) / (RH - 2 * HY)) * C;
}

template <int T, int R, int TAG = 0, int NW = C0_NW>
static bool launch_cn(Field Uout, Field F, Field Fc, const MGGeom &g, hipStream_t s, const RagMember *rag, int lev, bool pack)
{
    constexpr int RH = NW * R, HY = 2 * T + 2;
    Field none{};
    const TilePlan tp = coarse_tile_plan(F.W, F.H, F.C, 256 - 2 * C0_HX, C0_HX, RH - 2 * HY, rag != nullptr, pack && R <= C0_PACK_ROWS);
    const int blocks = tp.blocks;
    if constexpr (R <= C0_PACK_ROWS) if (tp.K >= 2) {
        hipLaunchKernelGGL((k_cycle0<T, NW, R, false, true, true, TAG | C0_PACK>), dim3(blocks), dim3(NW * 64), 0, s, F ,
                           Uout, F, Fc, none, g, (float *)nullptr, ComposeArgs(), (float4 *)nullptr, LmNodes(), AbortFlag(), (const RagMember *)nullptr, 0);
        return true;
    }
    if (rag) {
        if constexpr ((T == 4 && TAG == C0_L1_HALF && R != 8) || (T == 2 && TAG == 0 && NW == C0_NW))
            hipLaunchKernelGGL((k_cycle0<T, NW, R, false, true, true, TAG | C0_RAG>), dim3(blocks), dim3(NW * 64), 0, s, F, Uout, F, Fc, none, g,
                               (float *)nullptr, ComposeArgs(), (float4 *)nullptr, LmNodes(), AbortFlag(), rag, lev);
        else return false;
        return true;
    }
    hipLaunchKernelGGL((k_cycle0<T, NW, R, false, true, true, TAG>), dim3(blocks), dim3(NW * 64), 0, s, F ,
                       Uout, F, Fc, none, g, (float *)nullptr, ComposeArgs(), (float4 *)nullptr, LmNodes(), AbortFlag(), (const RagMember *)nullptr, 0);
    return true;
}

static int cn_blocks(const Field &F, int T, int R, int NW, bool size_class, bool pack)
{
    const int RH = NW * R, HY = 2 * T + 2;
    return coarse_tile_plan(F.W, F.H, F.C, 256 - 2 * C0_HX, C0_HX, RH - 2 * HY, size_class, pack).blocks;
}

bool launch_cycle_coarse(Field Uout, Field F, Field Fc, const MGGeom &g, int sweeps, hipStream_t s, bool half_io, const RagMember *rag, int lev, bool pack)
{
    pack = pack && !rag;
    if (half_io) {
// ... 18 lines not shown
```

seamlesscloneoptimization_amd/csrc/sc_hooks.cpp:

```cpp
#include "sc_pcg.h"
#include <algorithm>
#include <cmath>
#include <cstring>
#include <vector>

using namespace sc;

static int float_rhs(Instance *I)
{
    if (!I->f_half) return SC_OK;
    SC_HIP(I, hipSetDevice(I->gpu));
    Field scratch = I->result_in_U1 ? I->U0 : I->U1;
    const size_t n = I->F.plane * (size_t)I->F.C;
    launch_half_to_float(I->F.p, scratch.p, n, I->stream);
    SC_HIP(I, hipGetLastError());
    SC_HIP(I, hipMemcpyAsync(I->F.p, scratch.p, n * sizeof(float), hipMemcpyDeviceToDevice, I->stream));
    I->f_half = false;
    return SC_OK;
}

static int mg_time_coarse_chain(Instance *I, int reps, float *ms_eager, float *ms_graph, int *launches)
{
    if (I->mg.size() < 4 || I->mg_bottom < 3 || !mg_composes_level1(I)) { I->err = "time_coarse_chain: run a multigrid clone of at least ~500^2 first"; return SC_ERR_BAD_ARG; }
    const int pre = mg_params(I->opts).pre, post = mg_params(I->opts).post;
    int rc;
    if ((rc = fd_wait(I))) return rc;
    *launches = (int)(2 * (I->mg_bottom - 2) + 1) - (tail_serves(I, I->mg_bottom - 1) ? 2 : 0);
    if ((rc = vcycle(I, 2, pre, post))) return rc;
    SC_HIP(I, hipEventRecord(I->ev_k0, I->stream));
    for (int i = 0; i < reps; ++i) if ((rc = vcycle(I, 2, pre, post))) return rc;
    SC_HIP(I, hipEventRecord(I->ev_k1, I->stream));
    SC_HIP(I, hipStreamSynchronize(I->stream));
    float ms = 0.f;
    SC_HIP(I, hipEventElapsedTime(&ms, I->ev_k0, I->ev_k1));
    *ms_eager = ms / (float)reps;
    hipGraph_t graph = nullptr;
    hipGraphExec_t exec = nullptr;
    SC_HIP(I, hipStreamBeginCapture(I->stream, hipStreamCaptureModeThreadLocal));
    rc = vcycle(I, 2, pre, post);
    hipError_t e = hipStreamEndCapture(I->stream, &graph);
    if (rc || e != hipSuccess || !graph) { if (graph) (void)hipGraphDestroy(graph); return rc ? rc : hip_fail(I, e, "hipStreamEndCapture"); }
    e = hipGraphInstantiate(&exec, graph, nullptr, nullptr, 0);
    if (e != hipSuccess) { (void)hipGraphDestroy(graph); return hip_fail(I, e, "hipGraphInstantiate"); }
    (void)hipGraphLaunch(exec, I->stream);
    SC_HIP(I, hipEventRecord(I->ev_k0, I->stream));
    for (int i = 0; i < reps; ++i) (void)hipGraphLaunch(exec, I->stream);
    SC_HIP(I, hipEventRecord(I->ev_k1, I->stream));
    e = hipStreamSynchronize(I->stream);
    (void)hipGraphExecDestroy(exec);
    (void)hipGraphDestroy(graph);
    if (e != hipSuccess) return hip_fail(I, e, "hipStreamSynchronize");
    SC_HIP(I, hipEventElapsedTime(&ms, I->ev_k0, I->ev_k1));
    *ms_graph = ms / (float)reps;
// ... 162 lines not shown
    if (rc) return rc;
    if (plane_capacity < (size_t)cols * rows) return SC_ERR_BAD_SIZE;
    int dps, dms;
    if ((rc = edit_upload(I, src, cols, rows, ss, mask, ms, dps, dms))) return rc;
    if ((rc = setup_fields(I, cols, rows, 3))) return rc;
    if ((rc = edit_stage(I, ep, (const uint8_t *)I->d_face.p, cols, rows, dps, (const uint8_t *)I->d_mask.p, dms))) return rc;
    edit_preprocess(I, ep, (const uint8_t *)I->d_face.p, dps);
    SC_HIP(I, hipGetLastError());
    if (M_out && (rc = download_rows(I, I->h_out, M_out, cols, I->d_M.p, I->mpitch, cols, rows))) return rc;
    if (lap_out && (rc = download_field(I, I->F, lap_out))) return rc;
    SC_HIP(I, hipStreamSynchronize(I->stream));
    return SC_OK;
}

int sc_hip_canny(void *p, const uint8_t *src, int cols, int rows, int ss, float low, float high, int aperture, uint8_t *classes_out,
                 uint8_t *edges_out, int counts[2])
{
    Instance *I = get(p);
    if (!I || !src) return SC_ERR_BAD_ARG;
    I->err.clear();
    SC_HIP(I, hipSetDevice(I->gpu));
    if (!std::isfinite(low) || !std::isfinite(high) || (aperture != 3 && aperture != 5 && aperture != 7)) return SC_ERR_BAD_ARG;
    if (cols < 1 || rows < 1 || ss < 3 * cols) return SC_ERR_BAD_SIZE;
    int rc, dps, dms;
    if ((rc = edit_upload(I, src, cols, rows, ss, nullptr, 0, dps, dms))) return rc;
    I->mpitch = round_up(cols, 64);
    if ((rc = canny_stage(I, (const uint8_t *)I->d_face.p, cols, rows, dps, low, high, aperture, classes_out))) return rc;
    if (edges_out) {
        if ((rc = download_rows(I, I->h_out, edges_out, cols, I->d_edge.p, I->mpitch, cols, rows))) return rc;
        for (size_t i = 0; i < (size_t)cols * rows; ++i) edges_out[i] = edges_out[i] == 2 ? 255 : 0;
    }
    if (counts) { counts[0] = I->hyst_launches; counts[1] = I->hyst_reads; }
    SC_HIP(I, hipStreamSynchronize(I->stream));
    return SC_OK;
}

int sc_hip_edit_counts(void *p, int counts[2])
{
    Instance *I = get(p);
    if (!I || !counts) return SC_ERR_BAD_ARG;
    counts[0] = I->hyst_launches; counts[1] = I->hyst_reads;
    return SC_OK;
}

int sc_hip_bytes_writer(void *p)
{
    Instance *I = get(p);
    if (!I) return SC_ERR_BAD_ARG;
    const int w = I->bytes_writer;
    I->bytes_writer = 0;
    return w;
}

int sc_hip_field_load(void *p, int W, int H, int C, const float *U, const float *lap)
{
    Instance *I = get(p);
    if (I) field_moved(I);
    if (I) I->out_direct = false;
    if (!I || !U || !lap) return SC_ERR_BAD_ARG;
    I->err.clear();
    SC_HIP(I, hipSetDevice(I->gpu));
    if (W < 1 || H < 1 || C < 1 || C > 16) return SC_ERR_BAD_SIZE;
    int rc;
    if ((rc = setup_fields(I, W, H, C))) return rc;
    SC_HIP(I, hipMemsetAsync(I->d_U0.p, 0, I->U0.bytes(), I->stream));
    SC_HIP(I, hipMemsetAsync(I->d_U1.p, 0, I->U1.bytes(), I->stream));
    SC_HIP(I, hipMemsetAsync(I->d_F.p, 0, I->F.bytes(), I->stream));
    const size_t wb = (size_t)W * sizeof(float), pb = (size_t)I->U0.pitch * sizeof(float);
    if ((rc = upload_rows(I, I->h_face, I->U0.p, pb, (const uint8_t *)U, wb, wb, C * H))) return rc;
    if ((rc = upload_rows(I, I->h_body, I->F.p, pb, (const uint8_t *)lap, wb, wb, C * H))) return rc;
    SC_HIP(I, hipMemcpyAsync(I->U1.p, I->U0.p, pb * (size_t)(C * H - 1) + wb, hipMemcpyDeviceToDevice, I->stream));
    SC_HIP(I, hipStreamSynchronize(I->stream));
    return SC_OK;
}

int sc_hip_field_sweep(void *p, int method, int sweeps, float omega, int spl)
{
    Instance *I = get(p);
    if (I && I->out_direct) { I->err = "the last clone kept no solution field (set SC_FLAG_KEEP_FIELD to keep it)"; return SC_ERR_BAD_ARG; }
    if (I && I->f_half) { int frc = float_rhs(I); if (frc) return frc; }
    if (!I || !I->F.p) return SC_ERR_BAD_ARG;
    SC_HIP(I, hipSetDevice(I->gpu));
    I->info.sweep_launches = 0;
    int rc = run_sweeps(I, method, sweeps, omega, spl);
    if (rc) return rc;
    SC_HIP(I, hipStreamSynchronize(I->stream));
    return SC_OK;
}

int sc_hip_field_residual(void *p, double out[2])
{
    Instance *I = get(p);
    if (I && I->out_direct) { I->err = "the last clone kept no solution field (set SC_FLAG_KEEP_FIELD to keep it)"; return SC_ERR_BAD_ARG; }
    if (I && I->f_half) { int frc = float_rhs(I); if (frc) return frc; }
    if (!I || !I->F.p || !out) return SC_ERR_BAD_ARG;
    SC_HIP(I, hipSetDevice(I->gpu));
    return eval_residual(I, out);
}

int sc_hip_field_solve(void *p)
{
    Instance *I = get(p);
    if (I && I->f_half) { int frc = float_rhs(I); if (frc) return frc; }
    if (!I || !I->F.p) return SC_ERR_BAD_ARG;
    SC_HIP(I, hipSetDevice(I->gpu));
    I->info.sweep_launches = 0;
// ... 137 lines not shown
    auto once = [&]() { return launch_cycle0(d); };
    if (once() < 0) { I->err = "time_cycle0_form: form not instantiated"; return SC_ERR_BAD_ARG; }
    SC_HIP(I, hipEventRecord(I->ev_k0, I->stream));
    for (int i = 0; i < launches; ++i) once();
    SC_HIP(I, hipEventRecord(I->ev_k1, I->stream));
    SC_HIP(I, hipGetLastError());
    SC_HIP(I, hipStreamSynchronize(I->stream));
    lowmode_bands_written(I, nullptr);
    *ms_per_launch = ev_ms(I->ev_k0, I->ev_k1) / (float)launches;
    return SC_OK;
}

int sc_hip_coarse_tile_plan(const int *facts, int *plan)
{
    if (!facts || !plan) return SC_ERR_BAD_ARG;
    const int W = facts[0], H = facts[1], C = facts[2], uw = facts[3], hx = facts[4], rows = facts[5], first = facts[8], n = facts[9];
    if (W < 1 || H < 1 || C < 1 || hx < 4 || hx % 4 || uw != 256 - 2 * hx || rows < 1 || first < 0 || n < 0) return SC_ERR_BAD_ARG;
    const TilePlan tp = coarse_tile_plan(W, H, C, uw, hx, rows, facts[6] != 0, facts[7] == 0);
    if ((long)first + n > tp.blocks) return SC_ERR_BAD_ARG;
    plan[0] = tp.full; plan[1] = tp.lps; plan[2] = tp.K; plan[3] = tp.blocks;
    for (int k = 0; k < n; ++k) {
        int *o = plan + 4 + 130 * (size_t)k;
        for (int lane = 0; lane < 64; ++lane) {
            const TileLane tl = coarse_tile_lane(tp, C, uw, hx, first + k, lane);
            o[0] = tl.by; o[1] = tl.lps; o[2 + 2 * lane] = tl.c; o[3 + 2 * lane] = tl.x;
        }
    }
    return SC_OK;
}

int sc_hip_pcg_plan(int cols, int rows, int kind, int frames, long long plan[10])
{
    if (!plan || frames < 1 || frames > SC_POISSON_MAX_PLANES) return SC_ERR_BAD_ARG;
    const sc_poisson_layout l{ cols, rows, 1, 1, (long long)cols, (long long)cols * rows };
    const int rc = family_validate(&kind, &l, nullptr, "at most 8192 unknowns (pixels - 2) per side", nullptr);
    if (rc) return rc;
    const int k = poisson_norm_kind(kind);
    const MixedGeo mg = poisson_mixed_geo(poisson_free_sides(k), cols, rows, poisson_periodic(k));
    const PcgGeo wg = frames > 1 ? volume_work_geo(mg, frames) : pcg_geo(mg);
    const long long out[10] = { wg.nx, wg.ny, wg.x0, wg.y0, wg.cg, wg.bands, wg.rows, wg.eparts, wg.egroups, wg.stride };
    std::copy(out, out + 10, plan);
    return SC_OK;
}

int sc_hip_cycle0_form(const int *facts, int index, int form[3])
{
    if (!form) return SC_ERR_BAD_ARG;
    int T = 0, TAG = 0, rc;
    bool PRO = false;
    if (facts) {
        static float4 some_bands;
        static const RagMember some_class{};
        Cycle0Launch d;
        d.sweeps = facts[0]; d.prolong = facts[1]; d.f_half = facts[2]; d.u_half = facts[3]; d.q16_in = facts[4]; d.q16_out = facts[5];
        d.final_cycle = facts[6]; d.out_bytes = (facts[7] & 1) != 0; d.out_interleaved = (facts[7] & 2) != 0; d.composed = facts[8]; d.l1_half = facts[9]; d.timing = facts[10];
        d.bands = facts[11] ? &some_bands : nullptr; d.rag = facts[12] ? &some_class : nullptr;
        rc = cycle0_form(d, T, PRO, TAG) ? 0 : -1;
    } else if ((rc = cycle0_form_at(index, T, PRO, TAG)) <= index || index < 0) {
        return rc;
    }
    if (rc >= 0) { form[0] = T; form[1] = PRO; form[2] = TAG; }
    return rc;
}

int sc_hip_fused_schedule(const int *facts, const int *verdicts, int nverdicts, int *rows, int capacity)
{
    if (!facts || !rows || nverdicts < 0 || (nverdicts > 0 && !verdicts)) return SC_ERR_BAD_ARG;
    const int pre = facts[0], post = facts[1], budget = facts[2], early_kind = facts[9];
    if (pre < 1 || pre > 2 || post < 1 || post > 2 || budget < 1 || budget > 64 || early_kind < 0 || early_kind > 3) return SC_ERR_BAD_ARG;
    const bool bytes_form = facts[10] != 0;
    FusedSchedule S{ FusedFacts{ pre, post, budget, facts[3] != 0, facts[4] != 0, facts[5] != 0, facts[6] != 0, facts[7] != 0, facts[8] != 0, facts[11] != 0 } };
    int n = 0, used = 0, verdict = VERDICT_NONE;
    for (;;) {
        FusedStep s = fused_next(S, verdict);
        if (s.kind == FUSED_DONE) break;
        if (s.ask_early) fused_early(S, s, early_kind);
        if (capacity < SC_FUSED_ROW * (n + 1) + 3) return SC_ERR_BAD_ARG;
        const int row[SC_FUSED_ROW] = { s.kind, s.sweeps, s.prolong, s.final_cycle, s.out_bytes, s.u_half, s.q16_in, s.q16_out, s.composed, s.bands, s.lm,
                                        s.nodes, s.judged, s.coarse_first, s.sat, s.bands_sweeps, s.ask_early, S.cyc };
        std::memcpy(rows + SC_FUSED_ROW * n++, row, sizeof(row));
        verdict = VERDICT_NONE;
        if (!s.judged) continue;
        if (s.out_bytes && !bytes_form) { verdict = VERDICT_NO_FORM; continue; }
        verdict = nverdicts ? verdicts[std::min(used++, nverdicts - 1)] : VERDICT_ACCEPT;
        if (verdict < VERDICT_ACCEPT || verdict > VERDICT_SATURATED) return SC_ERR_BAD_ARG;
        if (verdict == VERDICT_REJECT_EARLY && !(s.out_bytes && S.early_cond)) verdict = VERDICT_ACCEPT;
        if (verdict == VERDICT_SATURATED && !S.f.q16) verdict = VERDICT_ACCEPT;
    }
    if (capacity < SC_FUSED_ROW * n + 3) return SC_ERR_BAD_ARG;
    rows[SC_FUSED_ROW * n] = S.cyc; rows[SC_FUSED_ROW * n + 1] = S.sweep_launches; rows[SC_FUSED_ROW * n + 2] = S.result;
    return n;
}

int sc_hip_time_coarse_chain(void *p, int reps, float *ms_eager, float *ms_graph, int *launches)
{
    Instance *I = get(p);
    if (!I || reps < 1 || !ms_eager || !ms_graph || !launches) return SC_ERR_BAD_ARG;
    SC_HIP(I, hipSetDevice(I->gpu));
    return mg_time_coarse_chain(I, reps, ms_eager, ms_graph, launches);
}

int sc_hip_time_tail_phases(void *p, unsigned long long *cycles11)
{
    Instance *I = get(p);
    if (!I || !cycles11) return SC_ERR_BAD_ARG;
    SC_HIP(I, hipSetDevice(I->gpu));
    return mg_time_tail_phases(I, cycles11);
// ... 4 lines not shown
```

seamlesscloneoptimization_amd/csrc/sc_instance.h:

```cpp
#pragma once
#include "sc_common.h"
#include "sc_hostcopy.h"
#include <algorithm>
#include <memory>
#include <cmath>

namespace sc {

struct DevBuf {
    void *p = nullptr;
    size_t cap = 0;
    bool own = true;
};
inline void dev_release(DevBuf &b) { if (b.p && b.own) (void)hipFree(b.p); b.p = nullptr; b.cap = 0; }

struct FD1 {
    int n = 0;
    float cw_last = 0.f, d_last = 0.f;
    std::vector<double> lam, q, ee;
};

struct LowMode {
    int w = 0, h = 0, C = 0;
    int Kx = 0, Ky = 0, Kxp = 0, Kyp = 0;
// ... 74 lines not shown
    int nl = 0, tail = 0, npx = 0, npy = 0, Kxp = 0, Kyp = 0;
    int max_nx = 0, max_ny = 0, max_nxt = 0, max_nrs = 0, max_cells_y = 0;
    double max_ratio = 0.0;
    DevBuf d_aux, h_stage;
    bool pad_uniform = false;
    bool levels_built = false;
    hipEvent_t ev = nullptr;
    hipEvent_t ev_ready = nullptr;
    bool ready_pending = false;
};

struct SolveTarget {
    uint8_t *org = nullptr; int step = 0;
    const std::vector<ImageJob> *group = nullptr;
    bool writes() const { return org || group; }
};

struct Instance {
    uint32_t magic = 0x5C10E001u;
    int gpu = 0;
    hipStream_t stream = nullptr;
    hipStream_t aux = nullptr;
    hipStream_t aux2 = nullptr;
    hipEvent_t ev_fork = nullptr, ev_join = nullptr;
    bool aux_pending = false;
    sc_solver_opts opts{};
    int clone_mode = SC_NORMAL_CLONE;
    bool edit_call = false;
    sc_run_info info{};
    std::string err;

    DevBuf d_in, h_in;
    DevBuf d_face, d_body_roi, d_mask, d_out;
    DevBuf h_face, h_body, h_mask, h_out;
    DevBuf h_sx, h_sy;
    DevBuf h_state;
    DevBuf h_gt, h_smt;
    std::unique_ptr<RowCopier> copier;
    hipEvent_t ev_chunk[8]{};
    DevBuf d_M;
    int mpitch = 0;
    DevBuf d_edge, h_hyst;
    int hyst_launches = 0, hyst_reads = 0;
    DevBuf d_pois;
    bool auto_as_single = false;
    float screen_lambda = 0.f;
    DevBuf d_U0, d_U1, d_F;
    Field U0, U1, F;
    bool result_in_U1 = false;
    int bytes_writer = 0;
    bool out_direct = false;
    bool f_half = false;
    bool u_half = false;
    bool u_q16 = false;
    bool mg_q16_last = false;
    AbortFlag sat;
    unsigned sat_counter = 0;
    bool force_float_field = false;
    struct SpecPost { SolveTarget to; bool armed = false, done = false; } spec_post;
    RectGuard guard;
    int last_mc = -1, last_mr = -1, last_rect[4] = { 0, 0, 0, 0 };
    int spec_cooldown = 0;
    bool erode_done = false;
    BboxTask pending_scan;
    bool scan_pending = false;
    bool scan_counter_dirty = false;
    hipEvent_t ev_scan = nullptr, scan_fence = nullptr;
    bool bench_tag = false;
    std::vector<DevBuf> mg_bufs;
    DevBuf mg_partial;
    DevBuf h_partial;
    std::vector<MGLevel> mg;
    size_t mg_bottom = 0;
    bool mg_l1_half = false;
    int fd_level = -1, fd_nxp = 0, fd_nyp = 0;
    DevBuf mg_fd;
    bool fd_mm = false;
    int fd_npx = 0, fd_npy = 0;
    size_t fd_mm_off = 0;
    hipEvent_t ev_fd_fork = nullptr, ev_fd = nullptr;
    bool fd_pending = false;
    LowMode lm;
    RagState rag;
    DstState dst;
    FftState fft;
    PcgState *pcg = nullptr;
    bool fft_lds_float = false, fft_lds_double = false;
    DevBuf d_rects, h_rects;
    DevBuf d_bbox_parts;
    hipEvent_t ev_rects = nullptr;
    int group_spec_cooldown = 0;
    int *d_rect = nullptr;
    int *h_rect = nullptr;
    double *d_partials = nullptr;
    double *d_red = nullptr;
    double *h_red = nullptr;
    unsigned *d_maxcorr = nullptr;
    unsigned *h_maxcorr = nullptr;
    hipEvent_t ev[8]{};
    bool stage_marks = true;
    bool marks_ends_only = false;
    hipEvent_t tm[8]{};
    hipEvent_t ev_k0 = nullptr, ev_k1 = nullptr;
    size_t arena_bytes = 0;
    std::vector<DevBuf> retired;
    size_t retired_bytes = 0;
    struct Slab { uint8_t *base = nullptr; size_t cap = 0, used = 0; };
    std::vector<Slab> slabs;

    bool ok() const { return magic == 0x5C10E001u; }
};

struct CallScope {
    Instance *I;
    ~CallScope()
    {
        I->edit_call = false;
        I->force_float_field = false;
        I->spec_post = Instance::SpecPost();
        I->auto_as_single = false;
        I->screen_lambda = 0.f;
    }
};

inline bool legacy_path(const sc_solver_opts &o, int which) { return (o.flags & SC_FLAG_LEGACY_PATHS) && (o.legacy_paths & which); }
constexpr long SC_OUT3_MIN_TILES = 200;

constexpr int SC_RETRY_FLOAT_FIELD = 1;

int hip_fail(Instance *I, hipError_t e, const char *what);
#define SC_HIP(I, call)                                                   \
    do {                                                                  \
        hipError_t e_ = (call);                                           \
        if (e_ != hipSuccess) return hip_fail((I), e_, #call);            \
    } while (0)

int ensure(Instance *I, DevBuf &b, size_t bytes, bool zero = true);
int ensure_pinned(Instance *I, DevBuf &b, size_t bytes);
double fd_selftest_error();
double fd_closed_selftest_error();
int setup_fields(Instance *I, int W, int H, int C);

Instance *get(void *p);
int begin_call(void *p, Instance *&I);
int validate_images(Instance *I, const void *face, int fc, int fr, int fs, const void *body, int bc, int br,
                    int bs, const void *mask, int mc, int mr, int ms);
int geo_from_rect(Instance *I, const int r[4], int cx, int cy, Geo &g);
int check_roi(Instance *I, const Geo &g, int bc, int br);
int device_bbox(Instance *I, const uint8_t *d_mask, int mc, int mr, int ms, int cx, int cy, Geo &g);
void erode_mask(Instance *I, const uint8_t *d_mask, int ms, int mr, const Geo &g);
void fill_info_geo(Instance *I, const Geo &g);
float ev_ms(hipEvent_t a, hipEvent_t b);
inline void stage_mark(Instance *I, int k)
{
    if (I->stage_marks) (void)hipEventRecord(I->ev[k], I->stream);
}
inline int worse(int worst, int rc) { return (rc != SC_OK && (worst == SC_OK || worst == SC_ERR_NOT_CONVERGED)) ? rc : worst; }
int edit_validate(Instance *I, const sc_edit_params *p, const void *src, int cols, int rows, int ss, const void *mask, int ms,
                  const void *dst, int ds);
int canny_stage(Instance *I, const uint8_t *d_src, int W, int H, int ss, float low, float high, int aperture, uint8_t *C_out);
int edit_stage(Instance *I, const sc_edit_params *p, const uint8_t *d_src, int W, int H, int ss, const uint8_t *d_mask, int ms);
void edit_preprocess(Instance *I, const sc_edit_params *p, const uint8_t *d_src, int ss);
int canny_stage_group(Instance *I, const EditJob *jobs, int n, int W, int H, size_t mplane, float low, float high, int aperture);
void edit_preprocess_group(Instance *I, const sc_edit_params *p, const EditJob *jobs, int n, size_t mplane);
int poisson_validate(const sc_poisson_params *p, const sc_poisson_layout *l, const char **why);
constexpr int SC_POISSON_FREE_ALL = SC_POISSON_FREE_LEFT | SC_POISSON_FREE_RIGHT | SC_POISSON_FREE_TOP | SC_POISSON_FREE_BOTTOM;
constexpr int SC_POISSON_PERIODIC_ALL = SC_POISSON_PERIODIC_X | SC_POISSON_PERIODIC_Y;
inline int poisson_free_sides(int kind) { return (kind & SC_POISSON_NEUMANN) ? 15 : (kind & SC_POISSON_FREE_ALL) >> 12; }
inline int poisson_periodic(int kind) { return (kind & SC_POISSON_PERIODIC_ALL) >> 17; }
inline int poisson_base(int kind) { return kind & ~(SC_POISSON_NEUMANN | SC_POISSON_FREE_ALL | SC_POISSON_PERIODIC_ALL); }
inline int poisson_norm_kind(int kind)
{
    const int f = poisson_free_sides(kind);
    return poisson_base(kind) | (f == 15 ? SC_POISSON_NEUMANN : f << 12) | (kind & SC_POISSON_PERIODIC_ALL);
}
inline bool poisson_direct(int kind) { return poisson_free_sides(kind) || poisson_periodic(kind); }
inline MixedGeo poisson_mixed_geo(int f, int cols, int rows, int per)
{
    auto axis = [](bool lo, bool hi) { return lo ? (hi ? 1 : 3) : (hi ? 2 : 0); };
// ... 28 lines not shown
template <class Job, class ArraysOf> int float_intake(Instance *I, int kind, int carries, Job *jobs, int n, ArraysOf arrays_of, FloatJobs &v,
                                                      size_t span = 0, size_t tspan = 0)
{
    if (!jobs || n <= 0) { I->err = "no jobs"; return SC_ERR_BAD_ARG; }
    int worst = SC_OK;
    const char *why = "";
    for (int i = 0; i < n; ++i) {
        Job &j = jobs[i];
        const FloatArrays a = arrays_of(j);
        const int vrc = float_job_validate(kind, carries, a, &why, span, tspan);
        if (vrc != SC_OK) {
            j.rc = vrc;
            if (worst == SC_OK) { worst = vrc; I->err = why; }
            continue;
        }
        j.rc = SC_ERR_HIP;
        v.dj.push_back(float_dev_job(kind, carries, a));
        const bool smooth = (carries & FLOAT_SMOOTH) != 0;
        v.side.push_back(SideArrays{ carries & FLOAT_WEIGHT ? a.weight : nullptr, smooth ? a.smooth_x : nullptr, smooth ? a.smooth_y : nullptr,
                                     carries & FLOAT_STATE ? a.state : nullptr, carries & FLOAT_GT ? a.gt : nullptr,
                                     carries & FLOAT_SMOOTH_T ? a.smooth_t : nullptr });
        v.rcs.push_back(&j.rc);
    }
    return worst;
}
struct FloatStaged { PoissonJobDev job; SideArrays side; };
int float_stage(Instance *I, const sc_poisson_layout *l, int kind, int carries, const FloatArrays &a, FloatStaged &s, int frames = 1,
                long long frame_stride = 0, int tframes = 0);
template <class Chunk> int run_chunks(Instance *I, int C, int *const *rcs, int nv, Chunk chunk)
{
    const int per = std::max(1, SC_POISSON_MAX_PLANES / C);
    int worst = SC_OK;
    for (int i0 = 0; i0 < nv; i0 += per) {
        const int m = std::min(per, nv - i0);
        const int rc = chunk(i0, m);
        if (rc != SC_OK && rc != SC_ERR_NOT_CONVERGED) {
            for (int k = rc == SC_ERR_HIP ? 0 : i0; k < nv; ++k) *rcs[k] = rc;
            return rc;
        }
        worst = worse(worst, rc);
        I->info.group_members = m > 1 ? m : 0;
    }
    return worst;
}
int poisson_run(Instance *I, const PoissonCall &p, const sc_poisson_layout *l, const PoissonJobDev *dj, int *const *rcs, int nv, bool timed, float t[4]);
void poisson_set_timing(Instance *I, const float t[4]);
int poisson_download(Instance *I, const sc_poisson_layout *l, const float *d_out, float *out, const float t[4], int rc_solve, int frames = 1,
                     long long frame_stride = 0);
void copy_rows(Instance *I, uint8_t *dst, size_t dpitch, const uint8_t *src, size_t spitch, size_t row_bytes, int rows);
int upload_rows(Instance *I, DevBuf &stage, void *d, size_t dpitch, const uint8_t *h, size_t hpitch, size_t row_bytes, int rows);
int download_rows(Instance *I, DevBuf &stage, uint8_t *h, size_t hpitch, const void *d, size_t dpitch, size_t row_bytes, int rows);

int solve(Instance *I);
void solve_prepare(Instance *I);
int solve_attempt(Instance *I, const SolveTarget &t);
template <class Pre> int solve_step(Instance *I, const SolveTarget &t, Pre &&pre)
{
    int rc;
    do {
        solve_prepare(I);
        if ((rc = pre())) return rc;
    } while ((rc = solve_attempt(I, t)) == SC_RETRY_FLOAT_FIELD);
    return rc;
}
int write_output(Instance *I, const SolveTarget &t, AbortFlag sat = AbortFlag());
bool mg_reads_half_rhs(const Instance *I);
bool mg_level1_half(const Instance *I);
bool mg_composes_level1(const Instance *I);
struct MGParams { int pre, post, budget; float utol; };
inline MGParams mg_params(const sc_solver_opts &o)
{
    return { o.mg_pre > 0 ? o.mg_pre : 2, o.mg_post > 0 ? o.mg_post : 2, o.max_sweeps > 0 ? o.max_sweeps : 30, o.update_tol > 0.f ? o.update_tol : 0.25f };
}
inline int fd_wait(Instance *I)
{
    if (I->fd_pending) {
        SC_HIP(I, hipStreamWaitEvent(I->stream, I->ev_fd, 0));
        I->fd_pending = false;
    }
    return SC_OK;
}
int vcycle(Instance *I, size_t l, int pre, int post, unsigned no_post = 0);
int run_tail(Instance *I, size_t l, int pre, int post, bool &done, unsigned long long *stamps = nullptr);
bool tail_serves(const Instance *I, size_t l);

enum { FUSED_DONE = 0, FUSED_FIRST, FUSED_FULL, FUSED_BEFORE_JUDGED, FUSED_JUDGED_BYTES, FUSED_JUDGED_FIELD, FUSED_CATCH_UP };
enum { VERDICT_NONE = -1, VERDICT_ACCEPT = 0, VERDICT_REJECT, VERDICT_REJECT_EARLY, VERDICT_SATURATED, VERDICT_NO_FORM };
enum { NODES_NONE = 0, NODES_MAIN, NODES_SECOND, NODES_NOTHING };
struct FusedFacts {
    int pre, post, budget;
    bool tol;
    bool out_wanted, q16;
    bool u_half, composed;
    bool separate_restrict;
    bool small;
};
struct FusedStep {
    int kind = FUSED_DONE, sweeps = 0;
    bool prolong = false, final_cycle = false, out_bytes = false, u_half = false, q16_in = false, q16_out = false, composed = false;
    bool coarse_first = false;
    int bands_sweeps = 0;
    int bands = 0;
    bool ask_early = false;
    bool lm = false;
    int nodes = NODES_NONE;
    bool judged = false;
    bool sat = false;
};
struct FusedSchedule {
    FusedFacts f;
    int last = -1, cyc = 0;
    int sweep_launches = 0;
    int result = SC_OK;
// ... 46 lines not shown
```

seamlesscloneoptimization_amd/csrc/sc_kernels.hip:

```cpp
#include "sc_common.h"
#include <hip/hip_fp16.h>
#include "sc_wave.h"
#include <limits.h>
#include <algorithm>
#include <stdlib.h>

namespace sc {

__device__ __forceinline__ int wave_min_i(int v)
{
#pragma unroll
    for (int o = 32; o > 0; o >>= 1) v = min(v, __shfl_xor(v, o, 64));
    return v;
}
__device__ __forceinline__ int wave_max_i(int v)
{
#pragma unroll
    for (int o = 32; o > 0; o >>= 1) v = max(v, __shfl_xor(v, o, 64));
    return v;
}
__device__ __forceinline__ double wave_sum_d(double v)
{
#pragma unroll
    for (int o = 32; o > 0; o >>= 1) v += __shfl_down(v, o, 64);
// ... 305 lines not shown
            gx = std::max(gx, ((t.j[i].g.W + 3) / 4 + 63) / 64);
            gy = std::max(gy, (t.j[i].g.H + 4 * ER_STRIP_GROUP - 1) / (4 * ER_STRIP_GROUP));
        }
        hipLaunchKernelGGL(k_mask_erode3_group<ER_STRIP_GROUP>, dim3(gx, gy, cnt), dim3(256), 0, s, t);
    }
}

constexpr int P4_TW = 128, P4_RPT = 2, P4_TH = 8 * P4_RPT;
constexpr int P4_ROWQ = (3 * (P4_TW + 2) + 15 + 4 + 15) / 16;
constexpr int P4_ROWD = 4 * P4_ROWQ;

__device__ __forceinline__ void p4_stage(const uint8_t *__restrict__ img, int step, int W, int H, int tx0, int ty0,
                                         unsigned (*sm)[P4_ROWD], int *org)
{
    for (int i = threadIdx.x; i < (P4_TH + 2) * P4_ROWQ; i += 256) {
        const int ry = i / P4_ROWQ, q = i - ry * P4_ROWQ;
        const int y = ty0 - 1 + ry;
        uint4 v = make_uint4(0u, 0u, 0u, 0u);
        int a = 0;
        if (y >= 0 && y < H) {
            const uint8_t *row = img + (size_t)y * step;
            const uint8_t *first = row + 3 * (tx0 - 1);
            a = (int)((uintptr_t)first & 15);
            const uint8_t *p = first - a + 16 * q;
            if (p >= row && p + 16 <= row + 3 * W) {
                v = *reinterpret_cast<const uint4 *>(p);
            } else {
                unsigned w[4] = { 0u, 0u, 0u, 0u };
#pragma unroll
                for (int k = 0; k < 4; ++k) {
                    const uint8_t *pk = p + 4 * k;
                    if (pk + 3 >= row && pk < row + 3 * W) w[k] = *reinterpret_cast<const unsigned *>(pk);
                }
                v = make_uint4(w[0], w[1], w[2], w[3]);
            }
        }
        if (q == 0) org[ry] = a;
        *reinterpret_cast<uint4 *>(&sm[ry][4 * q]) = v;
    }
}

template <int N>
__device__ __forceinline__ void p4_window(const unsigned *row, int word0, int shift, unsigned (&w)[N])
{
    unsigned d[N + 1];
#pragma unroll
    for (int k = 0; k <= N; ++k) d[k] = row[word0 + k];
#pragma unroll
    for (int k = 0; k < N; ++k) w[k] = __builtin_amdgcn_alignbyte(d[k + 1], d[k], shift);
}

#define P4_BYTE(w, b) ((float)(((w)[(b) >> 2] >> (8 * ((b) & 3))) & 0xffu))

template <bool HF, bool HU, bool GREY = false, bool ER = false, int MODE = SC_NORMAL_CLONE>
__device__ __forceinline__ void preprocess_block(const uint8_t *__restrict__ body, int bstep,
                                                 const uint8_t *__restrict__ face, int fstep,
                                                 const uint8_t *__restrict__ M, int mpitch,
                                                 const Field &U0, const Field &F, int c0, int by, const BboxTask *er = nullptr)
{
    __shared__ __attribute__((aligned(16))) unsigned sb[P4_TH + 2][P4_ROWD], sp[P4_TH + 2][P4_ROWD];
    __shared__ int ob[P4_TH + 2], op[P4_TH + 2];
    __shared__ unsigned hw[ER ? P4_TH + 7 : 1][ER ? 34 : 1], ew[ER ? P4_TH + 1 : 1][ER ? 34 : 1];
    const int W = U0.W, H = U0.H;
    const int tx0 = blockIdx.x * P4_TW, ty0 = by * P4_TH;
    p4_stage(body, bstep, W, H, tx0, ty0, sb, ob);
    p4_stage(face, fstep, W, H, tx0, ty0, sp, op);
    if (ER) {
        const uint8_t *mask = er->mask;
        const int mstep = er->mstep, gx0 = er->g.x0, gy0 = er->g.y0;
        const uintptr_t lo = (uintptr_t)mask & ~(uintptr_t)3, hi = ((uintptr_t)mask + er->mask_bytes - 1) & ~(uintptr_t)3;
        for (int i = threadIdx.x; i < (P4_TH + 7) * 33; i += 256) {
            const int r = i / 33, wq = i - r * 33;
            const int y = ty0 - 4 + r, x = tx0 - 4 + 4 * wq;
            unsigned h = 0u;
            if (y >= 0 && y < H && x >= 0 && x < W) {
                const uint8_t *s = mask + (size_t)(y + gy0) * mstep + (gx0 + x - 3);
                const int a = (int)((uintptr_t)s & 3);
                const unsigned *p = reinterpret_cast<const unsigned *>(s - a);
                unsigned d[4];
#pragma unroll
                for (int k = 0; k < 4; ++k) {
                    const uintptr_t q = (uintptr_t)(p + k);
                    d[k] = (q >= lo && q <= hi) ? p[k] : 0u;
                }
                const unsigned fa = is255_flags(__builtin_amdgcn_alignbyte(d[1], d[0], a));
                const unsigned fb = is255_flags(__builtin_amdgcn_alignbyte(d[2], d[1], a));
                const unsigned fc = is255_flags(__builtin_amdgcn_alignbyte(d[3], d[2], a));
                h = fa & __builtin_amdgcn_alignbyte(fb, fa, 1) & __builtin_amdgcn_alignbyte(fb, fa, 2) &
                    __builtin_amdgcn_alignbyte(fb, fa, 3) & fb & __builtin_amdgcn_alignbyte(fc, fb, 1) &
                    __builtin_amdgcn_alignbyte(fc, fb, 2);
            }
            hw[r][wq] = h;
        }
        __syncthreads();
        for (int i = threadIdx.x; i < (P4_TH + 1) * 33; i += 256) {
            const int r = i / 33, wq = i - r * 33;
            const int y = ty0 - 1 + r, x = tx0 - 4 + 4 * wq;
            unsigned v = hw[r][wq] & hw[r + 1][wq] & hw[r + 2][wq] & hw[r + 3][wq] & hw[r + 4][wq] & hw[r + 5][wq] & hw[r + 6][wq];
            unsigned xring = 0u;
#pragma unroll
            for (int j = 0; j < 4; ++j)
                if (x + j >= 3 && x + j <= W - 4) xring |= 0x80u << (8 * j);
            v &= xring;
            if (y < 3 || y > H - 4 || x < 0 || x >= W) v = 0u;
            v = (v >> 7) * 255u;
            ew[r][wq] = v;
            if (r >= 1 && wq >= 1 && y < H && x < W) *reinterpret_cast<unsigned *>(er->M_out + (size_t)y * mpitch + x) = v;
// ... 32 lines not shown
    }
    const bool yin = (y >= 1) && (y <= H - 2);
    unsigned mw = 0, muw = 0, mlb = 0;
    if (ER) {
        if (yin) { mw = ew[ly + 1][lx + 1]; muw = ew[ly][lx + 1]; mlb = ew[ly + 1][lx] >> 24; }
    } else if (yin) {
        mw = *reinterpret_cast<const unsigned *>(M + (size_t)y * mpitch + x);
        muw = *reinterpret_cast<const unsigned *>(M + (size_t)(y - 1) * mpitch + x);
        mlb = x > 0 ? M[(size_t)y * mpitch + x - 1] : 0u;
    }
    const size_t o = (size_t)y * U0.pitch + x;
#pragma unroll
    for (int c = 0; c < 3; ++c) {
        float uv[4], lv[4];
#pragma unroll
        for (int j = 0; j < 4; ++j) {
            const int b = 3 * (j + 1) + c;
            const float bcc = P4_BYTE(bc, b);
            uv[j] = (x + j < W) ? bcc : 0.f;
            float lap = 0.0f;
            if (yin && x + j >= 1 && x + j <= W - 2) {
                const float bl = P4_BYTE(bc, b - 3), br = P4_BYTE(bc, b + 3), bup = P4_BYTE(bu, b), bdn = P4_BYTE(bd, b);
                const float pcc = MONO ? yc[j + 1] : P4_BYTE(pc, b), pl = MONO ? yc[j] : P4_BYTE(pc, b - 3), pr = MONO ? yc[j + 2] : P4_BYTE(pc, b + 3),
                            pup = MONO ? yu[j] : P4_BYTE(pu, b), pdn = MONO ? yd[j] : P4_BYTE(pd, b);
                const unsigned mb = (mw >> (8 * j)) & 0xffu, mlbyte = (j == 0 ? mlb : ((mw >> (8 * (j - 1))) & 0xffu)), mub = (muw >> (8 * j)) & 0xffu;
                if (GREY) {
                    const float k = 1.0f / 255.0f;
                    const float wm = (float)mb * k, wi = (float)(255u - mb) * k, wlm = (float)mlbyte * k, wli = (float)(255u - mlbyte) * k;
                    const float wum = (float)mub * k, wui = (float)(255u - mub) * k;
                    const float gx = (br - bcc) * wi + (pr - pcc) * wm;
                    const float gxl = (bcc - bl) * wli + (pcc - pl) * wlm;
                    const float gy = (bdn - bcc) * wi + (pdn - pcc) * wm;
                    const float gyu = (bcc - bup) * wui + (pcc - pup) * wum;
                    lap = (gx - gxl) + (gy - gyu);
                } else {
                bool m = mb != 0u;
                bool ml = mlbyte != 0u;
                bool mu = mub != 0u;
                if constexpr (MIXED) {
                    const float pdl = P4_BYTE(pd, b - 3), bdl = P4_BYTE(bd, b - 3), pur = P4_BYTE(pu, b + 3), bur = P4_BYTE(bu, b + 3);
                    m = m && fabsf(pr - pdn) > fabsf(br - bdn);
                    ml = ml && fabsf(pcc - pdl) > fabsf(bcc - bdl);
                    mu = mu && fabsf(pur - pcc) > fabsf(bur - bcc);
                }
                const float gx = m ? (pr - pcc) : (br - bcc);
                const float gxl = ml ? (pcc - pl) : (bcc - bl);
                const float gy = m ? (pdn - pcc) : (bdn - bcc);
                const float gyu = mu ? (pcc - pup) : (bcc - bup);
                lap = (gx - gxl) + (gy - gyu);
                }
            }
            lv[j] = lap;
        }
        if (HU) {
            const __half2 a = __floats2half2_rn(uv[0], uv[1]), b2 = __floats2half2_rn(uv[2], uv[3]);
            uint2 pk; pk.x = *reinterpret_cast<const unsigned *>(&a); pk.y = *reinterpret_cast<const unsigned *>(&b2);
            *reinterpret_cast<uint2 *>(reinterpret_cast<__half *>(U0.p) + (size_t)(c0 + c) * U0.plane + o) = pk;
        } else {
            *reinterpret_cast<float4 *>(U0.at(c0 + c) + o) = make_float4(uv[0], uv[1], uv[2], uv[3]);
        }
        if (HF) {
            const __half2 a = __floats2half2_rn(lv[0], lv[1]), b2 = __floats2half2_rn(lv[2], lv[3]);
            uint2 pk; pk.x = *reinterpret_cast<const unsigned *>(&a); pk.y = *reinterpret_cast<const unsigned *>(&b2);
            *reinterpret_cast<uint2 *>(reinterpret_cast<__half *>(F.p) + (size_t)(c0 + c) * F.plane + o) = pk;
        } else {
            *reinterpret_cast<float4 *>(F.at(c0 + c) + o) = make_float4(lv[0], lv[1], lv[2], lv[3]);
        }
    }
    }
}
#undef P4_BYTE

template <bool HF, bool HU, bool GREY = false, bool BB = false, int MODE = SC_NORMAL_CLONE>
__global__ __launch_bounds__(256) void k_preprocess(const uint8_t *__restrict__ body, int bstep,
                                                     const uint8_t *__restrict__ face, int fstep,
                                                     const uint8_t *__restrict__ M, int mpitch,
                                                     Field U0, Field U1, Field F, BboxTask bb)
{
    if (BB && (int)blockIdx.y < bb.scan_rows) {
        const int b = (int)blockIdx.y * (int)gridDim.x + (int)blockIdx.x;
        if (b < bb.fold.nblocks) mask_bbox_block(bb.mask, bb.mw, bb.mh, bb.mstep, bb.fold, b % bb.fold.nbx, b / bb.fold.nbx);
        return;
    }
    if constexpr (BB) preprocess_block<HF, HU, GREY, true, MODE>(body, bstep, face, fstep, M, mpitch, U0, F, 0, (int)blockIdx.y - bb.scan_rows, &bb);
    else preprocess_block<HF, HU, GREY, false, MODE>(body, bstep, face, fstep, M, mpitch, U0, F, 0, (int)blockIdx.y);
}

template <bool HF, bool HU, int MODE = SC_NORMAL_CLONE>
__global__ __launch_bounds__(256) void k_preprocess_group(ImageJobs t, int mpitch, Field U0, Field F)
{
    const ImageJob &j = t.j[blockIdx.z];
    if (j.W > 0) {
        if ((int)blockIdx.x * P4_TW >= j.W || (int)blockIdx.y * P4_TH >= j.H) return;
        U0.W = F.W = j.W; U0.H = F.H = j.H;
    }
    preprocess_block<HF, HU, false, false, MODE>(j.body_src, j.bstep, j.face_org, j.fstep, j.M, mpitch, U0, F, 3 * blockIdx.z, (int)blockIdx.y);
}

template <int MODE>
static void launch_preprocess_group_mode(const ImageJob *jobs, int n, int mpitch, Field U0, Field F, hipStream_t s, bool f_half, bool u_half)
{
    for (int i0 = 0; i0 < n; i0 += ImageJobs::MAX) {
        ImageJobs t{};
        const int cnt = std::min(n - i0, (int)ImageJobs::MAX);
        for (int i = 0; i < cnt; ++i) t.j[i] = jobs[i0 + i];
        Field u = U0, f = F;
        u.p = u_half ? reinterpret_cast<float *>(reinterpret_cast<uint16_t *>(U0.p) + (size_t)3 * i0 * U0.plane) : U0.p + (size_t)3 * i0 * U0.plane;
        f.p = f_half ? reinterpret_cast<float *>(reinterpret_cast<uint16_t *>(F.p) + (size_t)3 * i0 * F.plane) : F.p + (size_t)3 * i0 * F.plane;
        dim3 g4((U0.W + P4_TW - 1) / P4_TW, (U0.H + P4_TH - 1) / P4_TH, cnt);
        if (f_half && u_half) hipLaunchKernelGGL((k_preprocess_group<true, true, MODE>), g4, dim3(256), 0, s, t, mpitch, u, f);
        else if (f_half) hipLaunchKernelGGL((k_preprocess_group<true, false, MODE>), g4, dim3(256), 0, s, t, mpitch, u, f);
        else hipLaunchKernelGGL((k_preprocess_group<false, false, MODE>), g4, dim3(256), 0, s, t, mpitch, u, f);
    }
}

void launch_preprocess_group(const ImageJob *jobs, int n, int mpitch, Field U0, Field F, hipStream_t s, bool f_half, bool u_half, int mode)
{
    if (mode == SC_MIXED_CLONE) launch_preprocess_group_mode<SC_MIXED_CLONE>(jobs, n, mpitch, U0, F, s, f_half, u_half);
    else if (mode == SC_MONOCHROME_TRANSFER) launch_preprocess_group_mode<SC_MONOCHROME_TRANSFER>(jobs, n, mpitch, U0, F, s, f_half, u_half);
    else launch_preprocess_group_mode<SC_NORMAL_CLONE>(jobs, n, mpitch, U0, F, s, f_half, u_half);
}

template <int MODE>
static void launch_preprocess_mode(dim3 g4, const uint8_t *body_org, int bstep, const uint8_t *face_org, int fstep, const uint8_t *M, int mpitch,
                                   Field U0, Field U1, Field F, hipStream_t s, bool f_half, bool u_half, const BboxTask &bb)
{
    if (bb.scan_rows > 0) {
        if (f_half && u_half) hipLaunchKernelGGL((k_preprocess<true, true, false, true, MODE>), g4, dim3(256), 0, s, body_org, bstep, face_org, fstep, M, mpitch, U0, U1, F, bb);
        else if (f_half) hipLaunchKernelGGL((k_preprocess<true, false, false, true, MODE>), g4, dim3(256), 0, s, body_org, bstep, face_org, fstep, M, mpitch, U0, U1, F, bb);
        else hipLaunchKernelGGL((k_preprocess<false, false, false, true, MODE>), g4, dim3(256), 0, s, body_org, bstep, face_org, fstep, M, mpitch, U0, U1, F, bb);
        return;
    }
    if (f_half && u_half) hipLaunchKernelGGL((k_preprocess<true, true, false, false, MODE>), g4, dim3(256), 0, s, body_org, bstep, face_org, fstep, M, mpitch, U0, U1, F, bb);
    else if (f_half) hipLaunchKernelGGL((k_preprocess<true, false, false, false, MODE>), g4, dim3(256), 0, s, body_org, bstep, face_org, fstep, M, mpitch, U0, U1, F, bb);
    else hipLaunchKernelGGL((k_preprocess<false, false, false, false, MODE>), g4, dim3(256), 0, s, body_org, bstep, face_org, fstep, M, mpitch, U0, U1, F, bb);
}

void launch_preprocess(const uint8_t *body_org, int bstep, const uint8_t *face_org, int fstep,
                       const uint8_t *M, int mpitch, Field U0, Field U1, Field F, hipStream_t s, bool f_half, bool u_half, bool grey,
                       const BboxTask *scan, int mode)
{
    dim3 g4((U0.W + P4_TW - 1) / P4_TW, (U0.H + P4_TH - 1) / P4_TH);
    BboxTask bb{};
    if (scan && !grey) {
        bb = *scan;
        const int chunks = (bb.mw + 15 + 15) / 16;
        bb.fold.nbx = (chunks + 63) / 64;
        bb.fold.nblocks = bb.fold.nbx * ((bb.mh + 4 * BB_ROWS - 1) / (4 * BB_ROWS));
        bb.scan_rows = (bb.fold.nblocks + (int)g4.x - 1) / (int)g4.x;
        g4.y += (unsigned)bb.scan_rows;
    }
    if (grey) hipLaunchKernelGGL((k_preprocess<false, false, true>), g4, dim3(256), 0, s, body_org, bstep, face_org, fstep, M, mpitch, U0, U1, F, bb);
    else if (mode == SC_MIXED_CLONE) launch_preprocess_mode<SC_MIXED_CLONE>(g4, body_org, bstep, face_org, fstep, M, mpitch, U0, U1, F, s, f_half, u_half, bb);
    else if (mode == SC_MONOCHROME_TRANSFER) launch_preprocess_mode<SC_MONOCHROME_TRANSFER>(g4, body_org, bstep, face_org, fstep, M, mpitch, U0, U1, F, s, f_half, u_half, bb);
    else launch_preprocess_mode<SC_NORMAL_CLONE>(g4, body_org, bstep, face_org, fstep, M, mpitch, U0, U1, F, s, f_half, u_half, bb);
}

__device__ __forceinline__ void copy_run(const uint8_t *__restrict__ s, uint8_t *__restrict__ d, size_t a, size_t b, size_t lane, size_t lanes)
{
    if (a >= b) return;
    size_t a16 = (a + 15) & ~(size_t)15;
    if (a16 > b) a16 = b;
    const size_t b16 = a16 + ((b - a16) & ~(size_t)15);
    if (lane < 16) {
        if (a + lane < a16) d[a + lane] = s[a + lane];
        if (b16 + lane < b) d[b16 + lane] = s[b16 + lane];
    }
    for (size_t o = a16 + 16 * lane; o < b16; o += 16 * lanes) *reinterpret_cast<uint4 *>(d + o) = *reinterpret_cast<const uint4 *>(s + o);
}

__global__ __launch_bounds__(256) void k_copy_group(CopyJobs t)
{
    const int m = blockIdx.y;
// ... 482 lines not shown
```

seamlesscloneoptimization_amd/csrc/sc_multigrid.cpp:

```cpp
#include "sc_instance.h"
#include <algorithm>
#include <cmath>
#include <cstring>
#include <cstdlib>

namespace sc {

static int run_bottom(Instance *I, size_t l0, int pre, int post)
{
    MGBottomArgs a;
    a.nlevels = (int)(I->mg.size() - l0);
    a.pre = pre; a.post = post;
    const MGLevel &last = I->mg.back();
    a.coarse_sweeps = std::max(8, std::min(64, 2 * std::max(last.g.x.n, last.g.y.n)));
    int off = 0;
    for (int i = 0; i < a.nlevels; ++i) {
        const MGLevel &L = I->mg[l0 + i];
        a.lv[i].g = L.g; a.lv[i].omega = L.omega;
        a.lv[i].pitch = bottom_pitch(L);
        const int plane = a.lv[i].pitch * (L.g.y.n + 2);
        a.lv[i].offU = off; a.lv[i].offF = off + plane;
        off += 2 * plane;
    }
    a.fd_level = I->fd_level; a.fd_nxp = I->fd_nxp; a.fd_nyp = I->fd_nyp;
// ... 307 lines not shown
    int rc;
    const bool out_wanted = I->spec_post.armed && o.tol <= 0.f && !(o.flags & SC_FLAG_KEEP_FIELD) && pre == 2 && post == 2;
    const bool q16 = I->mg_l1_half && mg_field_q16(I, out_wanted) && budget > 1;
    const int nb_cap = cycle0_blocks(I->F.W, I->F.H, I->F.C, 4);
    const bool host_fold = nb_cap <= 16384;
    if (host_fold && (rc = ensure_pinned(I, I->h_partial, sizeof(float) * (2 * (size_t)nb_cap + 64)))) return rc;
    float *const part_base = host_fold ? (float *)I->h_partial.p : (float *)I->mg_partial.p;
    AbortFlag sat;
    if (q16) {
        sat.p = (unsigned *)((float *)I->mg_partial.p + 2 * (size_t)nb_cap);
        sat.host = host_fold ? (unsigned *)((float *)I->h_partial.p + 2 * (size_t)nb_cap) : nullptr;
        sat.gen = 0x7fc00000u | (++I->sat_counter & 0x3fffffu);
    }
    I->sat = sat;
    const Level0Maxima maxima{ host_fold, nb_cap, part_base, sat };
    FusedSchedule S{ FusedFacts{ pre, post, budget, o.tol > 0.f, out_wanted, q16, I->u_half, mg_composes_level1(I), legacy_path(o, SC_LEGACY_SEPARATE_RESTRICT),
                                 I->F.C > 3 || (size_t)I->F.W * I->F.H < (size_t)3 << 18 } };
    const int launches_before = I->info.sweep_launches;
    int nb_last = 0;
    float4 *bands = nullptr;
    LmNodes early_lm;
    int verdict = VERDICT_NONE;
    for (;;) {
        FusedStep s = fused_next(S, verdict);
        I->info.sweep_launches = launches_before + S.sweep_launches;
        if (s.kind == FUSED_DONE) break;
        verdict = VERDICT_NONE;
        if (s.coarse_first && (rc = vcycle(I, 1, pre, post, s.composed ? (1u << 1) : 0u))) return rc;
        if (s.ask_early) fused_early(S, s, lowmode_early_kind(I, utol));
        if (s.coarse_first) bands = s.bands_sweeps ? lowmode_bands_buffer(I, s.bands_sweeps) : nullptr;
        if (s.lm && I->aux_pending) {
            SC_HIP(I, hipStreamWaitEvent(I->stream, I->ev_join, 0));
            I->aux_pending = false;
        }
        float *const part_now = part_base + (size_t)((S.cyc + 1) & 1) * nb_cap;
        Cycle0Launch d = step_launch(level0_launch(I, s.composed), s);
        if (s.prolong) d.partial = part_now;
        if (s.bands) d.bands = bands;
        if (s.lm) d.lm = early_lm;
        if (s.sat) d.sat = sat;
        bool interleaved = false;
        if (s.out_bytes) {
            const SolveTarget &to = I->spec_post.to;
            if (to.group && !d.rag && to.group->size() <= (size_t)ImageJobs::MAX && to.group->size() * 3 == (size_t)I->F.C && (*to.group)[0].W == 0 &&
                !legacy_path(o, SC_LEGACY_SPLICE_LAUNCH)) {
                const long tiles = (long)cycle0_blocks(I->F.W, I->F.H, (int)to.group->size(), s.sweeps);
                Cycle0Launch d3 = d;
                d3.out_interleaved = true; d3.jobs = to.group->data(); d3.njobs = (int)to.group->size(); d3.sat = sat;
                int T3, TAG3;
                bool PRO3;
                if ((tiles >= SC_OUT3_MIN_TILES || legacy_path(o, SC_FORCE_INTERLEAVED_OUT)) && cycle0_form(d3, T3, PRO3, TAG3)) { d = d3; interleaved = true; }
            }
        }
        const int nb = launch_cycle0(d);
        if (s.out_bytes && nb <= 0) { verdict = VERDICT_NO_FORM; continue; }
        if (s.prolong ? nb <= 0 : nb < 0) { I->err = "cycle0: unsupported depth"; return SC_ERR_BAD_ARG; }
        const Field Q = I->result_in_U1 ? I->U0 : I->U1;
        if (s.out_bytes) I->bytes_writer |= interleaved ? 2 : 1;
        if (!s.out_bytes) I->result_in_U1 = !I->result_in_U1;
        if (s.kind == FUSED_FIRST) {
            if (I->rag.dev && I->rag.ready_pending) {
                SC_HIP(I, hipStreamWaitEvent(I->stream, I->rag.ev_ready, 0));
                I->rag.ready_pending = false;
            }
            I->u_half = false;
            I->mg_q16_last = q16;
        } else if (!s.out_bytes) {
            lowmode_bands_written(I, d.bands ? result(I).p : nullptr);
        }
        I->u_q16 = s.q16_out;
        if (s.nodes != NODES_NONE) {
            early_lm = LmNodes();
            if (s.nodes == NODES_MAIN) {
                if ((rc = lowmode_nodes(I, result(I), early_lm))) return rc;
            } else if (s.nodes == NODES_SECOND) {
                SC_HIP(I, hipEventRecord(I->ev_fork, I->stream));
                SC_HIP(I, hipStreamWaitEvent(I->aux, I->ev_fork, 0));
                if ((rc = lowmode_nodes(I, result(I), early_lm, I->aux))) return rc;
                SC_HIP(I, hipEventRecord(I->ev_join, I->aux));
                I->aux_pending = true;
            }
        }
        if (!s.prolong) continue;
        SC_HIP(I, hipGetLastError());
        const int nb_prev = nb_last;
        if (!s.out_bytes) nb_last = nb;
        if (!s.judged) continue;
        float m, m_prev;
        bool saturated = false;
        if (s.out_bytes)
            rc = correction_maxima(I, maxima, S.cyc + 1, nb, nb_prev, part_now, [&]() -> int {
                    const SolveTarget &to = I->spec_post.to;
                    if (interleaved) return SC_OK;
                    if (!to.group) launch_splice_planar(Q, to.org, to.step, I->stream, I->guard, sat);
                    else launch_splice_planar_group(Q, to.group->data(), (int)to.group->size(), I->stream, sat);
                    return SC_OK;
                }, m, m_prev, saturated);
        else
            rc = correction_maxima(I, maxima, S.cyc + 1, nb, nb_prev, part_now, [&]() -> int {
                    if (!(I->spec_post.armed && o.tol <= 0.f)) return SC_OK;
                    const int lrc = write_output(I, I->spec_post.to, sat);
                    if (lrc) return lrc;
                    I->spec_post.done = true;
                    return SC_OK;
                }, m, m_prev, saturated);
        if (rc) return rc;
        I->info.last_update = m;
        bool stop = false;
        if (saturated) {
            if (!s.out_bytes) I->spec_post.done = false;
            verdict = VERDICT_SATURATED;
        } else if (s.out_bytes) {
            const bool early_ok = !(S.early_cond && I->lm.max_ratio * (double)m > 0.049);
            if (stop_rule(utol, m, m_prev) && early_ok) { I->spec_post.done = true; I->out_direct = true; verdict = VERDICT_ACCEPT; }
            else verdict = early_ok ? VERDICT_REJECT : VERDICT_REJECT_EARLY;
        } else {
            if (o.tol > 0.f && (rc = residual_stop(I, stop))) return rc;
            if (stop || stop_rule(utol, m, m_prev)) verdict = VERDICT_ACCEPT;
// ... 58 lines not shown
```

seamlesscloneoptimization_amd/csrc/sc_solver.cpp:

```cpp
#include "sc_instance.h"
#include <algorithm>

namespace sc {

Field &result(Instance *I) { return I->result_in_U1 ? I->U1 : I->U0; }
static Field &other(Instance *I) { return I->result_in_U1 ? I->U0 : I->U1; }

int effective_method(const Instance *I)
{
    const sc_solver_opts &o = I->opts;
    if (o.method != SC_METHOD_AUTO) return o.method;
    const int w = I->F.W - 2, h = I->F.H - 2;
    if (o.tol > 0.f || w < 1 || h < 1) return SC_METHOD_MULTIGRID;
    if (I->F.C > 3 && !I->auto_as_single) return SC_METHOD_MULTIGRID;
    if (w <= SC_AUTO_DIRECT_MAX && h <= SC_AUTO_DIRECT_MAX) return SC_METHOD_FFT;
    if (std::max(w, h) <= SC_AUTO_THIN_LONG_MAX &&
        ((long)w * h <= SC_AUTO_DIRECT_AREA || std::min(w, h) <= SC_AUTO_NARROW_MAX)) return SC_METHOD_FFT;
    if (std::min(w, h) <= SC_AUTO_THIN_MAX && std::max(w, h) <= SC_AUTO_THIN_LONG_MAX) return SC_METHOD_FFT;
    return SC_METHOD_MULTIGRID;
}

bool fft_in_double(const Instance *I)
{
    return (I->opts.flags & SC_FLAG_FFT_FP64) || I->opts.method == SC_METHOD_AUTO;
// ... 74 lines not shown
        left -= T;
    }
    SC_HIP(I, hipGetLastError());
    return SC_OK;
}

int mg_solve(Instance *I);

int solve(Instance *I)
{
    const sc_solver_opts &o = I->opts;
    field_moved(I);
    if (I->aux_pending) {
        SC_HIP(I, hipStreamWaitEvent(I->stream, I->ev_join, 0));
        I->aux_pending = false;
    }
    I->out_direct = false;
    I->info.sweeps = 0;
    I->info.converged = 0;
    I->info.rel_residual = NAN;
    I->info.method = o.method;
    if (I->F.W < 3 || I->F.H < 3) { I->info.converged = 1; return SC_OK; }
    const int method = effective_method(I);
    I->info.method = method;
    if (method == SC_METHOD_MULTIGRID) return mg_solve(I);
    if (method == SC_METHOD_DST) return dst_solve(I);
    if (method == SC_METHOD_FFT) return fft_solve(I, fft_in_double(I));
    if (o.tol <= 0.f) {
        int rc = run_sweeps(I, o.method, o.max_sweeps, o.omega, o.sweeps_per_launch);
        if (rc) return rc;
        I->info.sweeps = o.max_sweeps;
        I->info.converged = 1;
        return SC_OK;
    }
    const int every = std::max(1, o.check_every);
    int done = 0;
    while (done < o.max_sweeps) {
        const int n = std::min(every, o.max_sweeps - done);
        int rc = run_sweeps(I, o.method, n, o.omega, o.sweeps_per_launch);
        if (rc) return rc;
        done += n;
        double r[2];
        rc = eval_residual(I, r);
        if (rc) return rc;
        const double rel = (r[1] > 0.0) ? std::sqrt(r[0] / r[1]) : std::sqrt(r[0]);
        I->info.rel_residual = rel;
        I->info.sweeps = done;
        if (rel <= (double)o.tol) { I->info.converged = 1; return SC_OK; }
    }
    I->info.sweeps = done;
    return SC_ERR_NOT_CONVERGED;
}

void solve_prepare(Instance *I)
{
    I->result_in_U1 = false;
    I->f_half = mg_reads_half_rhs(I);
    I->u_half = I->f_half && !(I->opts.flags & SC_FLAG_FLOAT_U0);
}

int solve_attempt(Instance *I, const SolveTarget &t)
{
    I->info.sweep_launches = 0;
    if (t.writes()) {
        I->spec_post.to = t;
        I->spec_post.armed = true; I->spec_post.done = false;
    }
    const int rc = solve(I);
    I->spec_post.armed = false;
    const bool forced = I->force_float_field || (I->opts.flags & SC_FLAG_FLOAT_FIELD);
    I->force_float_field = false;
    if (rc != SC_RETRY_FLOAT_FIELD) return rc;
    if (forced) { I->err = "internal: a 16-bit field on the float32 path"; return SC_ERR_HIP; }
    I->force_float_field = true;
    I->info.field_retry = 1;
    return rc;
}

int write_output(Instance *I, const SolveTarget &t, AbortFlag sat)
{
    LmNodes lm;
    const int rc = output_nodes(I, lm);
    if (rc) return rc;
    if (t.group) launch_postprocess_group(result(I), t.group->data(), (int)t.group->size(), I->stream, lm, sat);
    else launch_postprocess(result(I), t.org, t.step, I->stream, I->guard, lm, sat);
    return SC_OK;
}

}
```

Before: 24110.

## Read initial field directly from destination bytes in first fused cycle

Adds a member-major cycle-0 kernel form that loads the initial guess straight from the interleaved 8-bit destination image, de-interleaving channels with alignbyte. Preprocessing then skips storing the half-precision U0 planes, which removes a write and a read of a full field. A fallback kernel fills the U0 planes when the form is unavailable. This adds byte-unpacking ALU work and guarded loads at row edges, and only applies to same-size groups above a tile threshold.

Measured after the change: 24520, median of 6. +1.7%, better.

```diff
diff --git a/include/seamlessclone_hip_testing.h b/include/seamlessclone_hip_testing.h
--- a/include/seamlessclone_hip_testing.h
+++ b/include/seamlessclone_hip_testing.h
@@ -14,6 +14,8 @@
 #define SC_LEGACY_UNPACKED_TILES 8
 #define SC_LEGACY_SPLICE_LAUNCH 16
 #define SC_FORCE_INTERLEAVED_OUT 32
+#define SC_LEGACY_U0_PLANES     64
+#define SC_FORCE_U0_BYTES       128
 #define SC_FLAG_KEEP_FIELD     (1 << 7)
 
 #define SC_FLAG_POISON_ARENA   (1 << 14)
@@ -57,6 +59,8 @@
 SC_API int sc_hip_cycle0_form(const int *facts, int index, int form[3]);
 
 SC_API int sc_hip_bytes_writer(void *instance);
+SC_API int sc_hip_u0_reader(void *instance);
+SC_API int sc_hip_u0_bytes_fetch(const uint8_t *row, int W, int xw, int *out);
 
 SC_API int sc_hip_coarse_tile_plan(const int *facts, int *plan);
 
diff --git a/seamlesscloneoptimization_amd/capi.py b/seamlesscloneoptimization_amd/capi.py
--- a/seamlesscloneoptimization_amd/capi.py
+++ b/seamlesscloneoptimization_amd/capi.py
@@ -54,6 +54,8 @@
 SC_LEGACY_SEPARATE_RESTRICT, SC_LEGACY_BOTTOM_F32, SC_LEGACY_SEPARATE_TAIL, SC_LEGACY_UNPACKED_TILES = 1, 2, 4, 8
 SC_LEGACY_SPLICE_LAUNCH = 16
 SC_FORCE_INTERLEAVED_OUT = 32
+SC_LEGACY_U0_PLANES = 64
+SC_FORCE_U0_BYTES = 128
 SC_FLAG_KEEP_FIELD = 1 << 7
 SC_FLAG_FFT_FP64 = 1 << 8
 SC_FLAG_OPENCV_GREY_MASK = 1 << 9
@@ -364,6 +366,10 @@
     L.sc_hip_field_solve.restype = C.c_int
     L.sc_hip_bytes_writer.argtypes = [C.c_void_p]
     L.sc_hip_bytes_writer.restype = C.c_int
+    L.sc_hip_u0_reader.argtypes = [C.c_void_p]
+    L.sc_hip_u0_reader.restype = C.c_int
+    L.sc_hip_u0_bytes_fetch.argtypes = [C.c_void_p, C.c_int, C.c_int, i32p]
+    L.sc_hip_u0_bytes_fetch.restype = C.c_int
     L.sc_hip_field_shape.argtypes = [C.c_void_p, i32p]
     L.sc_hip_field_shape.restype = C.c_int
     L.sc_hip_field_store.argtypes = [C.c_void_p, f32p, C.c_size_t]
@@ -1278,6 +1284,9 @@
     def bytes_writer(self):
         return int(self.L.sc_hip_bytes_writer(self.h))
 
+    def u0_reader(self):
+        return int(self.L.sc_hip_u0_reader(self.h))
+
     def field_shape(self):
         whc = np.zeros(3, np.int32)
         self._check(self.L.sc_hip_field_shape(self.h, whc.ctypes.data_as(i32p)))
@@ -1477,11 +1486,21 @@
 def cycle0_form(**facts):
     if facts.pop("out_interleaved", 0):
         facts["out_bytes"] = int(bool(facts.get("out_bytes", 0))) | 2
+    if facts.pop("in_bytes", 0):
+        facts["u_half"] = int(bool(facts.get("u_half", 0))) | 2
     f = (C.c_int * len(CYCLE0_FACTS))(*[int(facts.pop(k, 0)) for k in CYCLE0_FACTS])
     if facts:
         raise TypeError("cycle0_form: no such fact: %s" % sorted(facts))
     out = (C.c_int * 3)()
     return tuple(out) if load().sc_hip_cycle0_form(f, 0, out) == 0 else -1
+
+
+def u0_bytes_fetch(buf, offset, W, xw):
+    out = np.empty((64, 16), np.int32)
+    rc = load().sc_hip_u0_bytes_fetch(C.c_void_p(buf.ctypes.data + offset), W, xw, out.ctypes.data_as(i32p))
+    if rc:
+        raise ValueError("sc_hip_u0_bytes_fetch: %d" % rc)
+    return out
 
 
 def coarse_tile_plan(W, H, C_, useful, halo, rows, size_class=False, unpacked=False, lanes=False):
diff --git a/seamlesscloneoptimization_amd/csrc/sanitize_main.cpp b/seamlesscloneoptimization_amd/csrc/sanitize_main.cpp
--- a/seamlesscloneoptimization_amd/csrc/sanitize_main.cpp
+++ b/seamlesscloneoptimization_amd/csrc/sanitize_main.cpp
@@ -6,6 +6,7 @@
 #include <cstdio>
 #include <cstdlib>
 #include <cstring>
+#include <memory>
 #include <thread>
 #include <vector>
 
@@ -597,6 +598,32 @@
             sc_hip_pcg_plan(33, 47, SC_POISSON_LAPLACIAN, 0, p) != SC_ERR_BAD_ARG || sc_hip_pcg_plan(33, 47, SC_POISSON_LAPLACIAN, SC_POISSON_MAX_PLANES + 1, p) != SC_ERR_BAD_ARG ||
             sc_hip_pcg_plan(33, 47, SC_POISSON_LAPLACIAN, 1, nullptr) != SC_ERR_BAD_ARG) return fail("pcg_plan (refusals)");
     }
+    {
+        std::vector<int> out(64 * 16);
+        for (int W = 3; W <= 600; ++W)
+            for (int al = 0; al < 4; ++al) {
+                const size_t lead = 4 + (size_t)al;
+                std::unique_ptr<uint8_t[]> buf(new uint8_t[lead + 3 * (size_t)W + 3]);
+                uint8_t *base = buf.get();
+                if (((uintptr_t)base & 3) != 0) return fail("u0_bytes: allocation alignment");
+                uint8_t *row = base + lead;
+                for (size_t i = 0; i < lead + 3 * (size_t)W + 3; ++i) base[i] = (uint8_t)(i * 37u + (unsigned)W);
+                const int nbx = (W + 231) / 232;
+                for (int bx : { 0, nbx / 2, nbx - 1 }) {
+                    const int xw = bx * 232 - 12;
+                    if (sc_hip_u0_bytes_fetch(row, W, xw, out.data()) != SC_OK) return fail("u0_bytes_fetch");
+                    for (int lane = 0; lane < 64; ++lane) {
+                        const int *o = &out[16 * lane];
+                        const int x = std::min(std::max(xw + 4 * lane, 0), W);
+                        for (int k = 0; k < 4; ++k) {
+                            if ((o[2] >> k & 1) && !(o[0] + 4 * k + 3 >= 0 && o[0] + 4 * k < 3 * W)) return fail("u0_bytes: a dword outside the row was read");
+                            for (int ci = 0; ci < 3; ++ci)
+                                if (o[4 + 4 * ci + k] != (x + k < W ? (int)row[3 * (x + k) + ci] : 0)) return fail("u0_bytes: value");
+                        }
+                    }
+                }
+            }
+    }
     printf("sanitize_main: clean\n");
     return 0;
 }
diff --git a/seamlesscloneoptimization_amd/csrc/sc_arena.cpp b/seamlesscloneoptimization_amd/csrc/sc_arena.cpp
--- a/seamlesscloneoptimization_amd/csrc/sc_arena.cpp
+++ b/seamlesscloneoptimization_amd/csrc/sc_arena.cpp
@@ -178,7 +178,7 @@
     I->F = make_field(I->d_F.p, W, H, C);
     I->result_in_U1 = false;
     I->f_half = false;
-    I->u_half = false;
+    I->u_half = I->u0_bytes = false;
     if (!same) I->mg.clear();
     return SC_OK;
 }
diff --git a/seamlesscloneoptimization_amd/csrc/sc_batch.cpp b/seamlesscloneoptimization_amd/csrc/sc_batch.cpp
--- a/seamlesscloneoptimization_amd/csrc/sc_batch.cpp
+++ b/seamlesscloneoptimization_amd/csrc/sc_batch.cpp
@@ -69,7 +69,7 @@
     I->guard = RectGuard();
     const SolveTarget to{ nullptr, 0, &ij };
     const int solve_rc = solve_step(I, to, [&]() -> int {
-        launch_preprocess_group(ij.data(), n, I->mpitch, I->U0, I->F, I->stream, I->f_half, I->u_half, I->clone_mode);
+        launch_preprocess_group(ij.data(), n, I->mpitch, I->U0, I->F, I->stream, I->f_half, I->u_half, I->clone_mode, !I->u0_bytes);
         SC_HIP(I, hipGetLastError());
         if (plans && !builds_done) {
             if ((rc = rag_begin_builds(I))) return rc;
diff --git a/seamlesscloneoptimization_amd/csrc/sc_common.h b/seamlesscloneoptimization_amd/csrc/sc_common.h
--- a/seamlesscloneoptimization_amd/csrc/sc_common.h
+++ b/seamlesscloneoptimization_amd/csrc/sc_common.h
@@ -145,7 +145,8 @@
 }
 #endif
 void launch_postprocess(Field U, uint8_t *body_org, int bstep, hipStream_t s, RectGuard guard = RectGuard(), LmNodes lm = LmNodes(), AbortFlag ab = AbortFlag());
-void launch_preprocess_group(const ImageJob *jobs, int n, int mpitch, Field U0, Field F, hipStream_t s, bool f_half, bool u_half, int mode);
+void launch_preprocess_group(const ImageJob *jobs, int n, int mpitch, Field U0, Field F, hipStream_t s, bool f_half, bool u_half, int mode, bool store_u0 = true);
+void launch_u0_half_group(const ImageJob *jobs, int n, Field U0, hipStream_t s);
 void launch_postprocess_group(Field U, const ImageJob *jobs, int n, hipStream_t s, LmNodes lm = LmNodes(), AbortFlag ab = AbortFlag());
 void launch_splice_planar(Field Q, uint8_t *body_org, int bstep, hipStream_t s, RectGuard guard = RectGuard(), AbortFlag ab = AbortFlag());
 void launch_splice_planar_group(Field Q, const ImageJob *jobs, int n, hipStream_t s, AbortFlag ab = AbortFlag());
@@ -237,6 +238,7 @@
 constexpr int C0_PACK_ROWS = 6;
 constexpr int C0_PACK     = 2048;
 constexpr int C0_OUT3     = 4096;
+constexpr int C0_IN3      = 8192;
 constexpr int C0_RAG      = 1024;
 
 struct Cycle0Launch {
@@ -247,6 +249,7 @@
     bool f_half = false, u_half = false, q16_in = false, q16_out = false;
     bool final_cycle = false, out_bytes = false;
     bool out_interleaved = false;
+    bool in_bytes = false;
     const ImageJob *jobs = nullptr; int njobs = 0;
     bool composed = false;
     bool l1_half = false, timing = false;
diff --git a/seamlesscloneoptimization_amd/csrc/sc_cycle0.hip b/seamlesscloneoptimization_amd/csrc/sc_cycle0.hip
--- a/seamlesscloneoptimization_amd/csrc/sc_cycle0.hip
+++ b/seamlesscloneoptimization_amd/csrc/sc_cycle0.hip
@@ -2,6 +2,7 @@
 #include <hip/hip_fp16.h>
 #include "sc_wave.h"
 #include "sc_mg_device.h"
+#include "sc_u0_bytes.h"
 #include <type_traits>
 
 namespace sc {
@@ -72,6 +73,29 @@
     asm("v_cvt_i32_f32 %0, %1" : "=v"(i) : "v"(__builtin_fmaf(u, 64.0f, 16384.5f)));
     seen |= i;
     return (unsigned)min(max(i, 0), 65535);
+}
+
+template <int R>
+__device__ __forceinline__ void c0_load_bytes(const uint8_t *__restrict__ body, int bstep, int W, int H, int xc, int y0, bool unguarded, unsigned (&ch)[R][3])
+{
+    U0Quad raw[R];
+    int sh[R];
+    if (unguarded) {
+#pragma unroll
+        for (int r = 0; r < R; ++r) {
+            const uint8_t *row = body + (size_t)min(max(y0 + r, 0), H - 1) * bstep;
+            raw[r] = u0_fetch_unguarded(row, u0_first_dword(row, xc, sh[r]));
+        }
+    } else {
+#pragma unroll
+        for (int r = 0; r < R; ++r) {
+            const uint8_t *row = body + (size_t)min(max(y0 + r, 0), H - 1) * bstep;
+            unsigned fetched;
+            raw[r] = u0_fetch_guarded(row, W, u0_first_dword(row, xc, sh[r]), fetched);
+        }
+    }
+#pragma unroll
+    for (int r = 0; r < R; ++r) u0_channels(raw[r], sh[r], ch[r]);
 }
 
 __device__ __forceinline__ void c0_scale_q(uint2 &h)
@@ -150,8 +174,9 @@
                                                     const RagMember *__restrict__ rag, int lev, X3... x3)
 {
     constexpr int HY = 2 * T + 2, RH = NW * R;
-    constexpr bool OUT3 = (TAG & C0_OUT3) != 0;
-    static_assert(sizeof...(X3) == (OUT3 ? 1 : 0), "the members' jobs travel with the three-channel bytes form only");
+    constexpr bool OUT3 = (TAG & C0_OUT3) != 0, IN3 = (TAG & C0_IN3) != 0, MM = OUT3 || IN3;
+    static_assert(sizeof...(X3) == (MM ? 1 : 0), "the members' jobs travel with the member-major forms only");
+    static_assert(!IN3 || (!OUT3 && !PRO && !GEN && !ZEROIN && T == 2 && !(TAG & (C0_RAG | C0_U_HALF | C0_Q16_IN | C0_FINAL))), "destination bytes in: the first two-sweep launch of a same-size group");
     constexpr bool RAG = (TAG & C0_RAG) != 0;
     constexpr bool COMP = (TAG & C0_COMPOSED) != 0;
     static_assert(!COMP || (PRO && !GEN && R % 2 == 0), "composition of two prolongations exists on level 0 only");
@@ -182,7 +207,7 @@
     TileLane tl{};
     if constexpr (PACK) tl = coarse_tile_lane(coarse_tile_plan(W, H, Uin.C, 256 - 2 * C0_HX, C0_HX, RH - 2 * HY, false), Uin.C, 256 - 2 * C0_HX, C0_HX, tile, lane);
     const int bx = tile % nbx, by = PACK ? tl.by : (tile / nbx) % nby;
-    const int c_first = PACK ? min(tl.c, Uin.C - 1) : OUT3 ? 3 * (tile / (nbx * nby)) : tile / (nbx * nby);
+    const int c_first = PACK ? min(tl.c, Uin.C - 1) : MM ? 3 * (tile / (nbx * nby)) : tile / (nbx * nby);
     const int sl = PACK ? tl.sl : lane, lps = PACK ? tl.lps : 64;
     const bool live = !PACK || tl.c < Uin.C;
     if constexpr (RAG) {
@@ -201,22 +226,46 @@
     const ComposeArgs &comp_wg = comp;
     int ci = 0, c_run = c_first, pt_run = OUT3 ? tile + 2 * (c_first / 3) * (nbx * nby) : tile;
     const int pt_step = nbx * nby;
+    unsigned held[IN3 ? R : 1][2];
+    (void)held;
     _Pragma("nounroll") do {
-    const int lane = OUT3 ? c0_lane_again() : lane_wg, wv = c0_opaque_s<OUT3>(wv_wg), bx = c0_opaque_s<OUT3>(bx_wg), by = c0_opaque_s<OUT3>(by_wg);
-    std::conditional_t<OUT3, MGGeom, const MGGeom &> g = g_wg;
-    std::conditional_t<OUT3, ComposeArgs, const ComposeArgs &> comp = comp_wg;
-    if constexpr (OUT3) {
-        g.x.tw1 = c0_opaque_s<OUT3>(g.x.tw1); g.y.tw1 = c0_opaque_s<OUT3>(g.y.tw1);
-        comp.g1.x.tw1 = c0_opaque_s<OUT3>(comp.g1.x.tw1); comp.g1.y.tw1 = c0_opaque_s<OUT3>(comp.g1.y.tw1);
+    const int lane = MM ? c0_lane_again() : lane_wg, wv = c0_opaque_s<MM>(wv_wg), bx = c0_opaque_s<MM>(bx_wg), by = c0_opaque_s<MM>(by_wg);
+    std::conditional_t<MM, MGGeom, const MGGeom &> g = g_wg;
+    std::conditional_t<MM, ComposeArgs, const ComposeArgs &> comp = comp_wg;
+    if constexpr (MM) {
+        g.x.tw1 = c0_opaque_s<MM>(g.x.tw1); g.y.tw1 = c0_opaque_s<MM>(g.y.tw1);
+        comp.g1.x.tw1 = c0_opaque_s<MM>(comp.g1.x.tw1); comp.g1.y.tw1 = c0_opaque_s<MM>(comp.g1.y.tw1);
     }
     const int x = PACK ? tl.x : bx * (256 - 2 * C0_HX) - C0_HX + 4 * lane;
     const int y0 = by * (RH - 2 * HY) - HY + wv * R;
-    const int c = OUT3 ? c_run : c_first, ptile = OUT3 ? pt_run : tile;
+    const int c = MM ? c_run : c_first, ptile = OUT3 ? pt_run : tile;
     float4 u[R], f[HF ? 1 : R];
     uint2 fh[HF ? R : 1];
     if (ZEROIN) {
 #pragma unroll
         for (int r = 0; r < R; ++r) u[r] = make_float4(0.f, 0.f, 0.f, 0.f);
+    } else if constexpr (IN3) {
+        const int xc = u0_clamp_x(x, W);
+        unsigned word[R];
+        if (ci == 0) {
+            const ImageJobs &t = (x3, ...);
+            const ImageJob &j = t.j[c_first / 3];
+            const int xw0 = bx * (256 - 2 * C0_HX) - C0_HX;
+            const bool whole = u0_wave_unguarded(xw0, W) && (y0 >= 1) && (y0 + R - 1 <= H - 2);
+            unsigned ch[R][3];
+            c0_load_bytes<R>(j.body_src, j.bstep, W, H, xc, y0, whole, ch);
+#pragma unroll
+            for (int r = 0; r < R; ++r) { word[r] = ch[r][0]; held[r][0] = ch[r][1]; held[r][1] = ch[r][2]; }
+        } else {
+#pragma unroll
+            for (int r = 0; r < R; ++r) word[r] = ci == 1 ? held[r][0] : held[r][1];
+        }
+#pragma unroll
+        for (int r = 0; r < R; ++r) {
+            float o[4];
+            u0_values(word[r], xc, W, o);
+            u[r] = make_float4(o[0], o[1], o[2], o[3]);
+        }
     } else if (HU) {
         c0_load_half<R>(reinterpret_cast<const __half *>(Uin.p) + (size_t)c * Uin.plane, P, H, x, y0, u);
     } else if (UQI) {
@@ -579,7 +628,7 @@
         }
     }
 
-    if constexpr (OUT3) {
+    if constexpr (MM) {
         if (lane < C0_HXQ || lane >= 64 - C0_HXQ || x >= P || x >= W) continue;
     } else if (sl < C0_HXQ || sl >= lps - C0_HXQ || !live || x >= P || x >= W) return;
     if constexpr (OUT) {
@@ -636,7 +685,7 @@
         }
         const int seen = s0 | (x + 1 < W ? s1 : 0) | (x + 2 < W ? s2 : 0) | (x + 3 < W ? s3 : 0);
         if ((seen & ~0xffff) && sat.p) { *sat.p = sat.gen; if (sat.host) *sat.host = sat.gen; }
-        return;
+        if constexpr (MM) continue; else return;
     }
     float *__restrict__ out = Uout.at(c);
 #pragma unroll
@@ -644,7 +693,7 @@
         const int yr = wv * R + r, y = y0 + r;
         if (yr >= HY && yr < RH - HY && y >= 0 && y < H) *reinterpret_cast<float4 *>(out + (size_t)y * P + x) = u[r];
     }
-    } while (OUT3 && (c_run += 1, pt_run += pt_step, ++ci < 3));
+    } while (MM && (c_run += 1, pt_run += pt_step, ++ci < 3));
     if constexpr (OUT3) {
         const ImageJobs &t = (x3, ...);
         const ImageJob &j = t.j[c_first / 3];
@@ -695,9 +744,16 @@
            !d.q16_out && !d.timing && !d.rag;
 }
 
+constexpr int C0_IN3_TAG = C0_FAST | C0_IN3;
+static bool c0_is_in3(const Cycle0Launch &d)
+{
+    return d.in_bytes && !d.out_interleaved && !d.out_bytes && !d.final_cycle && !d.prolong && !d.composed && d.sweeps == 2 && d.f_half && d.l1_half && !d.u_half &&
+           !d.q16_in && !d.timing && !d.rag;
+}
+
 static const Cycle0Form *c0_find(const Cycle0Launch &d)
 {
-    if (d.out_interleaved) return nullptr;
+    if (d.out_interleaved || d.in_bytes) return nullptr;
     const bool shares = d.bands && d.prolong && !d.final_cycle && d.sweeps == 4;
     const int TAG = (d.timing ? C0_TIMING : 0) | (d.f_half ? C0_F_HALF : 0) | (d.u_half ? C0_U_HALF : 0) | (d.final_cycle ? C0_FINAL : 0) |
                     (d.composed ? C0_COMPOSED : 0) | (d.out_bytes ? C0_OUT : 0) | (shares ? C0_BANDS : 0) | (d.l1_half ? C0_L1_HALF : 0) |
@@ -710,6 +766,7 @@
 bool cycle0_form(const Cycle0Launch &d, int &T, bool &PRO, int &TAG)
 {
     if (c0_is_out3(d)) { T = 2; PRO = true; TAG = C0_OUT3_TAG; return true; }
+    if (c0_is_in3(d)) { T = 2; PRO = false; TAG = C0_IN3_TAG | (d.q16_out ? C0_Q16_OUT : 0); return true; }
     const Cycle0Form *f = c0_find(d);
     if (f) { T = f->T; PRO = f->PRO; TAG = f->TAG; }
     return f != nullptr;
@@ -732,6 +789,19 @@
                            d.E, d.g, d.partial, d.comp, d.bands, d.lm, d.sat, d.rag, 0, t);
         return 3 * blocks;
     }
+    if (d.in_bytes) {
+        if (!c0_is_in3(d) || !d.jobs || d.njobs < 1 || d.njobs > (int)ImageJobs::MAX || d.Uin.C != 3 * d.njobs) return -1;
+        ImageJobs t{};
+        for (int i = 0; i < d.njobs; ++i) t.j[i] = d.jobs[i];
+        const int blocks = cycle0_blocks(d.Uin.W, d.Uin.H, d.njobs, 2);
+        if (d.q16_out)
+            hipLaunchKernelGGL((k_cycle0<2, C0_NW, C0_R, false, false, false, C0_IN3_TAG | C0_Q16_OUT, ImageJobs>), dim3(blocks), dim3(C0_NW * 64), 0, d.s, d.Uin, d.Uout,
+                               d.F, d.Fc, d.E, d.g, d.partial, d.comp, d.bands, d.lm, d.sat, d.rag, 0, t);
+        else
+            hipLaunchKernelGGL((k_cycle0<2, C0_NW, C0_R, false, false, false, C0_IN3_TAG, ImageJobs>), dim3(blocks), dim3(C0_NW * 64), 0, d.s, d.Uin, d.Uout,
+                               d.F, d.Fc, d.E, d.g, d.partial, d.comp, d.bands, d.lm, d.sat, d.rag, 0, t);
+        return 0;
+    }
     const Cycle0Form *f = c0_find(d);
     if (!f) return -1;
     const int blocks = cycle0_blocks(d.Uin.W, d.Uin.H, d.Uin.C, f->T);
diff --git a/seamlesscloneoptimization_amd/csrc/sc_hooks.cpp b/seamlesscloneoptimization_amd/csrc/sc_hooks.cpp
--- a/seamlesscloneoptimization_amd/csrc/sc_hooks.cpp
+++ b/seamlesscloneoptimization_amd/csrc/sc_hooks.cpp
@@ -1,4 +1,5 @@
 #include "sc_pcg.h"
+#include "sc_u0_bytes.h"
 #include <algorithm>
 #include <cmath>
 #include <cstring>
@@ -267,6 +268,36 @@
     return w;
 }
 
+int sc_hip_u0_reader(void *p)
+{
+    Instance *I = get(p);
+    if (!I) return SC_ERR_BAD_ARG;
+    const int w = I->u0_reader;
+    I->u0_reader = 0;
+    return w;
+}
+
+int sc_hip_u0_bytes_fetch(const uint8_t *row, int W, int xw, int *out)
+{
+    if (!row || !out || W < 1) return SC_ERR_BAD_ARG;
+    const bool whole = u0_wave_unguarded(xw, W);
+    for (int lane = 0; lane < 64; ++lane, out += 16) {
+        const int xc = u0_clamp_x(xw + 4 * lane, W);
+        int shift;
+        const int q = u0_first_dword(row, xc, shift);
+        unsigned fetched = 15u, ch[3];
+        const U0Quad v = whole ? u0_fetch_unguarded(row, q) : u0_fetch_guarded(row, W, q, fetched);
+        u0_channels(v, shift, ch);
+        out[0] = q; out[1] = shift; out[2] = (int)fetched; out[3] = whole ? 1 : 0;
+        for (int c = 0; c < 3; ++c) {
+            float f[4];
+            u0_values(ch[c], xc, W, f);
+            for (int k = 0; k < 4; ++k) out[4 + 4 * c + k] = (int)f[k];
+        }
+    }
+    return SC_OK;
+}
+
 int sc_hip_field_load(void *p, int W, int H, int C, const float *U, const float *lap)
 {
     Instance *I = get(p);
@@ -510,7 +541,7 @@
         static float4 some_bands;
         static const RagMember some_class{};
         Cycle0Launch d;
-        d.sweeps = facts[0]; d.prolong = facts[1]; d.f_half = facts[2]; d.u_half = facts[3]; d.q16_in = facts[4]; d.q16_out = facts[5];
+        d.sweeps = facts[0]; d.prolong = facts[1]; d.f_half = facts[2]; d.u_half = (facts[3] & 1) != 0; d.in_bytes = (facts[3] & 2) != 0; d.q16_in = facts[4]; d.q16_out = facts[5];
         d.final_cycle = facts[6]; d.out_bytes = (facts[7] & 1) != 0; d.out_interleaved = (facts[7] & 2) != 0; d.composed = facts[8]; d.l1_half = facts[9]; d.timing = facts[10];
         d.bands = facts[11] ? &some_bands : nullptr; d.rag = facts[12] ? &some_class : nullptr;
         rc = cycle0_form(d, T, PRO, TAG) ? 0 : -1;
diff --git a/seamlesscloneoptimization_amd/csrc/sc_instance.h b/seamlesscloneoptimization_amd/csrc/sc_instance.h
--- a/seamlesscloneoptimization_amd/csrc/sc_instance.h
+++ b/seamlesscloneoptimization_amd/csrc/sc_instance.h
@@ -150,6 +150,8 @@
     bool out_direct = false;
     bool f_half = false;
     bool u_half = false;
+    bool u0_bytes = false;
+    int u0_reader = 0;
     bool u_q16 = false;
     bool mg_q16_last = false;
     AbortFlag sat;
@@ -223,6 +225,7 @@
 
 inline bool legacy_path(const sc_solver_opts &o, int which) { return (o.flags & SC_FLAG_LEGACY_PATHS) && (o.legacy_paths & which); }
 constexpr long SC_OUT3_MIN_TILES = 200;
+constexpr long SC_IN3_MIN_TILES = 200;
 
 constexpr int SC_RETRY_FLOAT_FIELD = 1;
 
@@ -357,13 +360,13 @@
 int download_rows(Instance *I, DevBuf &stage, uint8_t *h, size_t hpitch, const void *d, size_t dpitch, size_t row_bytes, int rows);
 
 int solve(Instance *I);
-void solve_prepare(Instance *I);
+void solve_prepare(Instance *I, const SolveTarget &t = SolveTarget());
 int solve_attempt(Instance *I, const SolveTarget &t);
 template <class Pre> int solve_step(Instance *I, const SolveTarget &t, Pre &&pre)
 {
     int rc;
     do {
-        solve_prepare(I);
+        solve_prepare(I, t);
         if ((rc = pre())) return rc;
     } while ((rc = solve_attempt(I, t)) == SC_RETRY_FLOAT_FIELD);
     return rc;
diff --git a/seamlesscloneoptimization_amd/csrc/sc_kernels.hip b/seamlesscloneoptimization_amd/csrc/sc_kernels.hip
--- a/seamlesscloneoptimization_amd/csrc/sc_kernels.hip
+++ b/seamlesscloneoptimization_amd/csrc/sc_kernels.hip
@@ -381,7 +381,7 @@
 
 #define P4_BYTE(w, b) ((float)(((w)[(b) >> 2] >> (8 * ((b) & 3))) & 0xffu))
 
-template <bool HF, bool HU, bool GREY = false, bool ER = false, int MODE = SC_NORMAL_CLONE>
+template <bool HF, bool HU, bool GREY = false, bool ER = false, int MODE = SC_NORMAL_CLONE, bool SU = true>
 __device__ __forceinline__ void preprocess_block(const uint8_t *__restrict__ body, int bstep,
                                                  const uint8_t *__restrict__ face, int fstep,
                                                  const uint8_t *__restrict__ M, int mpitch,
@@ -520,7 +520,8 @@
             }
             lv[j] = lap;
         }
-        if (HU) {
+        if (!SU) {
+        } else if (HU) {
             const __half2 a = __floats2half2_rn(uv[0], uv[1]), b2 = __floats2half2_rn(uv[2], uv[3]);
             uint2 pk; pk.x = *reinterpret_cast<const unsigned *>(&a); pk.y = *reinterpret_cast<const unsigned *>(&b2);
             *reinterpret_cast<uint2 *>(reinterpret_cast<__half *>(U0.p) + (size_t)(c0 + c) * U0.plane + o) = pk;
@@ -554,7 +555,7 @@
     else preprocess_block<HF, HU, GREY, false, MODE>(body, bstep, face, fstep, M, mpitch, U0, F, 0, (int)blockIdx.y);
 }
 
-template <bool HF, bool HU, int MODE = SC_NORMAL_CLONE>
+template <bool HF, bool HU, int MODE = SC_NORMAL_CLONE, bool SU = true>
 __global__ __launch_bounds__(256) void k_preprocess_group(ImageJobs t, int mpitch, Field U0, Field F)
 {
     const ImageJob &j = t.j[blockIdx.z];
@@ -562,11 +563,11 @@
         if ((int)blockIdx.x * P4_TW >= j.W || (int)blockIdx.y * P4_TH >= j.H) return;
         U0.W = F.W = j.W; U0.H = F.H = j.H;
     }
-    preprocess_block<HF, HU, false, false, MODE>(j.body_src, j.bstep, j.face_org, j.fstep, j.M, mpitch, U0, F, 3 * blockIdx.z, (int)blockIdx.y);
+    preprocess_block<HF, HU, false, false, MODE, SU>(j.body_src, j.bstep, j.face_org, j.fstep, j.M, mpitch, U0, F, 3 * blockIdx.z, (int)blockIdx.y);
 }
 
 template <int MODE>
-static void launch_preprocess_group_mode(const ImageJob *jobs, int n, int mpitch, Field U0, Field F, hipStream_t s, bool f_half, bool u_half)
+static void launch_preprocess_group_mode(const ImageJob *jobs, int n, int mpitch, Field U0, Field F, hipStream_t s, bool f_half, bool u_half, bool store_u0)
 {
     for (int i0 = 0; i0 < n; i0 += ImageJobs::MAX) {
         ImageJobs t{};
@@ -576,17 +577,47 @@
         u.p = u_half ? reinterpret_cast<float *>(reinterpret_cast<uint16_t *>(U0.p) + (size_t)3 * i0 * U0.plane) : U0.p + (size_t)3 * i0 * U0.plane;
         f.p = f_half ? reinterpret_cast<float *>(reinterpret_cast<uint16_t *>(F.p) + (size_t)3 * i0 * F.plane) : F.p + (size_t)3 * i0 * F.plane;
         dim3 g4((U0.W + P4_TW - 1) / P4_TW, (U0.H + P4_TH - 1) / P4_TH, cnt);
-        if (f_half && u_half) hipLaunchKernelGGL((k_preprocess_group<true, true, MODE>), g4, dim3(256), 0, s, t, mpitch, u, f);
+        if (f_half && u_half && !store_u0) hipLaunchKernelGGL((k_preprocess_group<true, true, MODE, false>), g4, dim3(256), 0, s, t, mpitch, u, f);
+        else if (f_half && u_half) hipLaunchKernelGGL((k_preprocess_group<true, true, MODE>), g4, dim3(256), 0, s, t, mpitch, u, f);
         else if (f_half) hipLaunchKernelGGL((k_preprocess_group<true, false, MODE>), g4, dim3(256), 0, s, t, mpitch, u, f);
         else hipLaunchKernelGGL((k_preprocess_group<false, false, MODE>), g4, dim3(256), 0, s, t, mpitch, u, f);
     }
 }
 
-void launch_preprocess_group(const ImageJob *jobs, int n, int mpitch, Field U0, Field F, hipStream_t s, bool f_half, bool u_half, int mode)
-{
-    if (mode == SC_MIXED_CLONE) launch_preprocess_group_mode<SC_MIXED_CLONE>(jobs, n, mpitch, U0, F, s, f_half, u_half);
-    else if (mode == SC_MONOCHROME_TRANSFER) launch_preprocess_group_mode<SC_MONOCHROME_TRANSFER>(jobs, n, mpitch, U0, F, s, f_half, u_half);
-    else launch_preprocess_group_mode<SC_NORMAL_CLONE>(jobs, n, mpitch, U0, F, s, f_half, u_half);
+void launch_preprocess_group(const ImageJob *jobs, int n, int mpitch, Field U0, Field F, hipStream_t s, bool f_half, bool u_half, int mode, bool store_u0)
+{
+    if (mode == SC_MIXED_CLONE) launch_preprocess_group_mode<SC_MIXED_CLONE>(jobs, n, mpitch, U0, F, s, f_half, u_half, store_u0);
+    else if (mode == SC_MONOCHROME_TRANSFER) launch_preprocess_group_mode<SC_MONOCHROME_TRANSFER>(jobs, n, mpitch, U0, F, s, f_half, u_half, store_u0);
+    else launch_preprocess_group_mode<SC_NORMAL_CLONE>(jobs, n, mpitch, U0, F, s, f_half, u_half, store_u0);
+}
+
+__global__ __launch_bounds__(256) void k_u0_half_group(ImageJobs t, Field U0)
+{
+    const ImageJob &j = t.j[blockIdx.z];
+    const int x = 4 * (int)(blockIdx.x * 64 + (threadIdx.x & 63)), y = (int)(blockIdx.y * 4 + (threadIdx.x >> 6));
+    if (x >= U0.W || y >= U0.H) return;
+    const uint8_t *row = j.body_src + (size_t)y * j.bstep;
+#pragma unroll
+    for (int c = 0; c < 3; ++c) {
+        float uv[4];
+#pragma unroll
+        for (int k = 0; k < 4; ++k) uv[k] = (x + k < U0.W) ? (float)row[3 * (min(x + k, U0.W - 1)) + c] : 0.f;
+        const __half2 a = __floats2half2_rn(uv[0], uv[1]), b2 = __floats2half2_rn(uv[2], uv[3]);
+        uint2 pk; pk.x = *reinterpret_cast<const unsigned *>(&a); pk.y = *reinterpret_cast<const unsigned *>(&b2);
+        *reinterpret_cast<uint2 *>(reinterpret_cast<__half *>(U0.p) + (size_t)(3 * blockIdx.z + c) * U0.plane + (size_t)y * U0.pitch + x) = pk;
+    }
+}
+
+void launch_u0_half_group(const ImageJob *jobs, int n, Field U0, hipStream_t s)
+{
+    for (int i0 = 0; i0 < n; i0 += ImageJobs::MAX) {
+        ImageJobs t{};
+        const int cnt = std::min(n - i0, (int)ImageJobs::MAX);
+        for (int i = 0; i < cnt; ++i) t.j[i] = jobs[i0 + i];
+        Field u = U0;
+        u.p = reinterpret_cast<float *>(reinterpret_cast<uint16_t *>(U0.p) + (size_t)3 * i0 * U0.plane);
+        hipLaunchKernelGGL(k_u0_half_group, dim3((U0.W + 255) / 256, (U0.H + 3) / 4, cnt), dim3(256), 0, s, t, u);
+    }
 }
 
 template <int MODE>
diff --git a/seamlesscloneoptimization_amd/csrc/sc_multigrid.cpp b/seamlesscloneoptimization_amd/csrc/sc_multigrid.cpp
--- a/seamlesscloneoptimization_amd/csrc/sc_multigrid.cpp
+++ b/seamlesscloneoptimization_amd/csrc/sc_multigrid.cpp
@@ -383,6 +383,20 @@
                 if ((tiles >= SC_OUT3_MIN_TILES || legacy_path(o, SC_FORCE_INTERLEAVED_OUT)) && cycle0_form(d3, T3, PRO3, TAG3)) { d = d3; interleaved = true; }
             }
         }
+        if (s.kind == FUSED_FIRST && s.u_half) {
+            int reader = 1;
+            if (I->u0_bytes) {
+                const SolveTarget &to = I->spec_post.to;
+                Cycle0Launch d3 = d;
+                d3.u_half = false; d3.in_bytes = true; d3.jobs = to.group ? to.group->data() : nullptr; d3.njobs = to.group ? (int)to.group->size() : 0;
+                int T3, TAG3;
+                bool PRO3;
+                if (d3.jobs && cycle0_form(d3, T3, PRO3, TAG3)) { d = d3; reader = 2; }
+                else if (!to.group) { I->err = "internal: no initial field stored for a solve without members"; return SC_ERR_BAD_ARG; }
+                else { launch_u0_half_group(to.group->data(), (int)to.group->size(), I->U0, I->stream); reader = 4; }
+            }
+            I->u0_reader |= reader;
+        }
         const int nb = launch_cycle0(d);
         if (s.out_bytes && nb <= 0) { verdict = VERDICT_NO_FORM; continue; }
         if (s.prolong ? nb <= 0 : nb < 0) { I->err = "cycle0: unsupported depth"; return SC_ERR_BAD_ARG; }
@@ -394,7 +408,7 @@
                 SC_HIP(I, hipStreamWaitEvent(I->stream, I->rag.ev_ready, 0));
                 I->rag.ready_pending = false;
             }
-            I->u_half = false;
+            I->u_half = I->u0_bytes = false;
             I->mg_q16_last = q16;
         } else if (!s.out_bytes) {
             lowmode_bands_written(I, d.bands ? result(I).p : nullptr);
diff --git a/seamlesscloneoptimization_amd/csrc/sc_solver.cpp b/seamlesscloneoptimization_amd/csrc/sc_solver.cpp
--- a/seamlesscloneoptimization_amd/csrc/sc_solver.cpp
+++ b/seamlesscloneoptimization_amd/csrc/sc_solver.cpp
@@ -150,11 +150,19 @@
     return SC_ERR_NOT_CONVERGED;
 }
 
-void solve_prepare(Instance *I)
+void solve_prepare(Instance *I, const SolveTarget &t)
 {
     I->result_in_U1 = false;
     I->f_half = mg_reads_half_rhs(I);
     I->u_half = I->f_half && !(I->opts.flags & SC_FLAG_FLOAT_U0);
+    I->u0_bytes = false;
+    if (I->u_half && t.group && !t.group->empty() && t.group->size() <= (size_t)ImageJobs::MAX && t.group->size() * 3 == (size_t)I->F.C &&
+        !legacy_path(I->opts, SC_LEGACY_U0_PLANES)) {
+        bool one_size = true;
+        for (const ImageJob &j : *t.group) one_size = one_size && j.W == 0;
+        const long tiles = (long)cycle0_blocks(I->F.W, I->F.H, (int)t.group->size(), 2);
+        I->u0_bytes = one_size && (tiles >= SC_IN3_MIN_TILES || legacy_path(I->opts, SC_FORCE_U0_BYTES));
+    }
 }
 
 int solve_attempt(Instance *I, const SolveTarget &t)
diff --git a/seamlesscloneoptimization_amd/csrc/sc_u0_bytes.h b/seamlesscloneoptimization_amd/csrc/sc_u0_bytes.h
--- /dev/null
+++ b/seamlesscloneoptimization_amd/csrc/sc_u0_bytes.h
@@ -0,0 +1,55 @@
+#pragma once
+#include <stdint.h>
+#include <hip/hip_runtime.h>
+
+namespace sc {
+
+struct __attribute__((aligned(4))) U0Quad { unsigned d[4]; };
+
+__host__ __device__ __forceinline__ bool u0_dword_in_row(uintptr_t d, uintptr_t row, int W) { return d + 3 >= row && d < row + 3 * (uintptr_t)W; }
+__host__ __device__ __forceinline__ bool u0_wave_unguarded(int xw, int W) { return xw >= 4 && xw + 255 <= W - 2; }
+__host__ __device__ __forceinline__ int u0_clamp_x(int x, int W) { return x < 0 ? 0 : x > W ? W : x; }
+__host__ __device__ __forceinline__ int u0_first_dword(const uint8_t *row, int xc, int &shift)
+{
+    shift = (int)(((uintptr_t)row + 3 * (uintptr_t)xc) & 3);
+    return 3 * xc - shift;
+}
+__host__ __device__ __forceinline__ unsigned u0_alignbyte(unsigned hi, unsigned lo, int shift)
+{
+#if defined(__HIP_DEVICE_COMPILE__)
+    return __builtin_amdgcn_alignbyte(hi, lo, (unsigned)shift);
+#else
+    return (unsigned)(((((unsigned long long)hi) << 32) | lo) >> (8 * shift));
+#endif
+}
+__host__ __device__ __forceinline__ U0Quad u0_fetch_guarded(const uint8_t *__restrict__ row, int W, int q, unsigned &fetched)
+{
+    U0Quad v;
+    fetched = 0u;
+    const int first = -(int)((uintptr_t)row & 3);
+#pragma unroll
+    for (int k = 0; k < 4; ++k) {
+        const bool ok = u0_dword_in_row((uintptr_t)row + (intptr_t)(q + 4 * k), (uintptr_t)row, W);
+        const unsigned w = *reinterpret_cast<const unsigned *>(row + (ok ? q + 4 * k : first));
+        v.d[k] = ok ? w : 0u;
+        fetched |= ok ? 1u << k : 0u;
+    }
+    return v;
+}
+__host__ __device__ __forceinline__ U0Quad u0_fetch_unguarded(const uint8_t *__restrict__ row, int q) { return *reinterpret_cast<const U0Quad *>(row + q); }
+__host__ __device__ __forceinline__ void u0_channels(const U0Quad &v, int shift, unsigned (&ch)[3])
+{
+    const unsigned w0 = u0_alignbyte(v.d[1], v.d[0], shift), w1 = u0_alignbyte(v.d[2], v.d[1], shift), w2 = u0_alignbyte(v.d[3], v.d[2], shift);
+    ch[0] = (w0 & 0xffu) | ((w0 >> 24) << 8) | (((w1 >> 16) & 0xffu) << 16) | (((w2 >> 8) & 0xffu) << 24);
+    ch[1] = ((w0 >> 8) & 0xffu) | ((w1 & 0xffu) << 8) | ((w1 >> 24) << 16) | (((w2 >> 16) & 0xffu) << 24);
+    ch[2] = ((w0 >> 16) & 0xffu) | (((w1 >> 8) & 0xffu) << 8) | ((w2 & 0xffu) << 16) | ((w2 >> 24) << 24);
+}
+__host__ __device__ __forceinline__ void u0_values(unsigned word, int xc, int W, float (&out)[4])
+{
+    out[0] = xc + 0 < W ? (float)(word & 0xffu) : 0.f;
+    out[1] = xc + 1 < W ? (float)((word >> 8) & 0xffu) : 0.f;
+    out[2] = xc + 2 < W ? (float)((word >> 16) & 0xffu) : 0.f;
+    out[3] = xc + 3 < W ? (float)(word >> 24) : 0.f;
+}
+
+}
```
